# sanweiliti/EgoHMR

Measured on AMD Instinct MI355X. Metric: sampled bodies/sec (100-step DDPM, batch 256), higher is better.
Workload: dtype f32 results: denoiser GEMMs as 3x f16 MFMA on hi/lo-split operands (f32 accumulate) on the last 100 of 100 steps, plain f16 operands on the first 0; k = 100 is~; 1 GPU; B256 S1 DDPM-100 N4096 ResNet50+PointNet cond, diffuse_fuse(2 GCN passes), LBS every step, unguided; items_per_gpu=256, samples_per_item=1, denoising_steps=100, scene_points=4096, lbs_every_step=True, collision_guided=False, gcn_precision=f16x3, f16x3_last_steps=100, parallelism=items sharded x1, one RCCL all-gather of [B,226] at the end

## Files before the change

### egohmr_amd/_lib.py

```python
from __future__ import annotations

import ctypes as C
import glob
import itertools
import os
import subprocess
import sys
from types import SimpleNamespace

import torch

_HERE = os.path.dirname(os.path.abspath(__file__))
LIB_PATH = os.environ.get("EHM_LIB_PATH") or os.path.join(_HERE, "libegohmr_hip.so")
CSRC = os.path.join(_HERE, "csrc")
INCLUDE = os.path.join(os.path.dirname(_HERE), "include")
SOURCES = ["gcn.hip", "gcn_tile.hip", "linear.hip", "conv.hip", "stem.hip", "metrics.hip", "smpl.hip", "sampler.hip", "guidance.hip", "prep.hip", "step.hip", "eval.hip", "stage1.hip", "scene.hip", "loss.hip", "gcn_bwd.hip"]


class EgoHMRHipError(RuntimeError):
    def __init__(self, msg="", rc=None, function=None):
        super().__init__(msg)
        self.rc, self.function = rc, function


class EgoHMRRangeError(EgoHMRHipError):
    """rc = -34: an activation of the denoiser reached the f16 range and was clamped in its X2 / f16 store (ehm_gcn_stack_status).  The results are finite
    but not parity grade; the remedy is float32 activations for that checkpoint: EgoHMR.gcn_precision = 'f32' (EgoHMR.on_saturation = 'f32' does it
    and re-runs the call)."""


def build(verbose: bool = False, force: bool = False) -> str:
    import hashlib
    from concurrent.futures import ThreadPoolExecutor
    hipcc = os.environ.get("HIPCC", "/opt/rocm/bin/hipcc")
    extra = os.environ.get("EHM_HIPCC_FLAGS", "").split()
    flags = ["--offload-arch=gfx950", "-O3", "-std=c++17", "-fPIC", f"-I{INCLUDE}", f"-I{CSRC}", *extra]
    hdrs = glob.glob(os.path.join(CSRC, "*.h")) + [os.path.join(INCLUDE, "egohmr_hip.h")]
    hdr_time = max(os.path.getmtime(h) for h in hdrs)
    tag = hashlib.sha1(" ".join([hipcc] + flags).encode()).hexdigest()[:10]
    objdir = os.path.join(_HERE, "build", os.path.basename(LIB_PATH) + "." + tag)
    os.makedirs(objdir, exist_ok=True)
    jobs = []
    sources = SOURCES
    for s in sources:
        src, obj = os.path.join(CSRC, s), os.path.join(objdir, s.replace(".hip", ".o"))
        if force or not os.path.exists(obj) or os.path.getmtime(obj) < max(os.path.getmtime(src), hdr_time):
            jobs.append((src, obj))
    objs = [os.path.join(objdir, s.replace(".hip", ".o")) for s in sources]
    tag_path = LIB_PATH + ".tag"
    linked_tag = open(tag_path).read().strip() if os.path.exists(tag_path) else None
    if not jobs and os.path.exists(LIB_PATH) and linked_tag == tag and all(os.path.getmtime(LIB_PATH) >= os.path.getmtime(o) for o in objs):
        return LIB_PATH

    def compile_one(job):
        cmd = [hipcc, *flags, "-c", job[0], "-o", job[1]]
        if verbose:
            print(" ".join(cmd), file=sys.stderr)
        return subprocess.run(cmd, capture_output=True, text=True)

    with ThreadPoolExecutor(max_workers=int(os.environ.get("EHM_BUILD_JOBS", min(len(jobs) or 1, os.cpu_count() or 1)))) as ex:
        for (src, _), r in zip(jobs, ex.map(compile_one, jobs)):
            if r.returncode != 0:
                raise EgoHMRHipError(f"hipcc failed on {src}:\n{r.stdout}\n{r.stderr}")
            if "failed to meet occupancy target" in r.stderr:
                os.remove(os.path.join(objdir, os.path.basename(src).replace(".hip", ".o")))
                raise EgoHMRHipError(f"hipcc: a kernel of {src} missed its occupancy target:\n{r.stderr}")
    cmd = [hipcc, "--offload-arch=gfx950", "-fPIC", "-shared", *objs, "-o", LIB_PATH]
    if verbose:
        print(" ".join(cmd), file=sys.stderr)
    r = subprocess.run(cmd, capture_output=True, text=True)
    if r.returncode != 0:
        raise EgoHMRHipError(f"hipcc (link) failed:\n{r.stdout}\n{r.stderr}")
    with open(tag_path, "w") as f:
        f.write(tag + "\n")
    return LIB_PATH


def build_features() -> set:
    return set(lib().ehm_build_features().decode().split())


class GConvParams(C.Structure):
    _fields_ = [("W", C.c_void_p), ("M", C.c_void_p), ("adj2", C.c_void_p), ("bias", C.c_void_p),
                ("bn_weight", C.c_void_p), ("bn_bias", C.c_void_p), ("bn_mean", C.c_void_p), ("bn_var", C.c_void_p),
                ("in_dim", C.c_int), ("out_dim", C.c_int)]


class LinearDesc(C.Structure):
    _fields_ = [("A0", C.c_void_p), ("A1", C.c_void_p), ("W", C.c_void_p), ("bias", C.c_void_p), ("group_bias", C.c_void_p),
                ("Y", C.c_void_p), ("colmax", C.c_void_p), ("M", C.c_int64), ("N", C.c_int), ("K0", C.c_int), ("K1", C.c_int),
                ("rows_per_group", C.c_int), ("valid_rows_per_group", C.c_int), ("relu_in0", C.c_int), ("relu_out", C.c_int),
                ("w_scale", C.c_float), ("lift_points", C.c_void_p), ("lift_W4", C.c_void_p), ("hi_only", C.c_int), ("group_bias_stride", C.c_int)]


class ConvDesc(C.Structure):
    _fields_ = [("x", C.c_void_p), ("W", C.c_void_p), ("bias", C.c_void_p), ("residual", C.c_void_p), ("y", C.c_void_p),
                ("N", C.c_int), ("H", C.c_int), ("Wd", C.c_int), ("Ci", C.c_int), ("Co", C.c_int),
                ("KH", C.c_int), ("KW", C.c_int), ("stride", C.c_int), ("pad", C.c_int), ("relu", C.c_int),
                ("w_scale", C.c_float)]


class ConvX2Desc(C.Structure):
    _fields_ = [("x", C.c_void_p), ("x_rows", C.c_int64), ("W", C.c_void_p), ("bias", C.c_void_p), ("residual", C.c_void_p), ("y", C.c_void_p),
                ("N", C.c_int), ("H", C.c_int), ("Wd", C.c_int), ("Ci", C.c_int), ("Co", C.c_int),
                ("KH", C.c_int), ("KW", C.c_int), ("stride", C.c_int), ("pad", C.c_int), ("relu", C.c_int),
                ("w_scale", C.c_float), ("workspace", C.c_void_p), ("workspace_bytes", C.c_int64),
                ("x2", C.c_void_p), ("x2_rows", C.c_int64), ("H2", C.c_int), ("W2", C.c_int), ("Ci2", C.c_int), ("stride2", C.c_int), ("hi_only", C.c_int),
                ("workspace_clean", C.c_int)]


class EvalPointsDesc(C.Structure):
    _fields_ = [("pred", C.c_void_p), ("gt", C.c_void_p), ("pred_origin", C.c_void_p), ("gt_origin", C.c_void_p), ("mask", C.c_void_p),
                ("per_point", C.c_void_p), ("mean", C.c_void_p), ("vis_sum", C.c_void_p), ("invis_sum", C.c_void_p),
                ("B", C.c_int), ("S", C.c_int), ("P", C.c_int), ("pred_points", C.c_int), ("gt_points", C.c_int), ("origin_point", C.c_int)]


class ItemPrepDesc(C.Structure):
    _fields_ = [("keypoints_2d", C.c_void_p), ("joint_map", C.c_void_p), ("NK", C.c_int), ("force_visible", C.c_int),
                ("fx", C.c_void_p), ("cx", C.c_void_p), ("cy", C.c_void_p), ("box_center", C.c_void_p), ("box_size", C.c_void_p), ("transl", C.c_void_p),
                ("fx_norm", C.c_float), ("with_bbox", C.c_int), ("with_cam_center", C.c_int),
                ("tW1", C.c_void_p), ("tb1", C.c_void_p), ("tW2", C.c_void_p), ("tb2", C.c_void_p), ("t_hidden", C.c_int), ("t_out", C.c_int),
                ("img_rowsum", C.c_void_p), ("scene_rowsum", C.c_void_p), ("other", C.c_void_p), ("other_ld", C.c_int), ("other_col0", C.c_int),
                ("vis", C.c_void_p), ("mask_slot", C.c_void_p), ("mask_items", C.c_void_p), ("count", C.c_void_p), ("finite", C.c_void_p),
                ("need_scratch", C.c_void_p), ("pass_group", C.c_int), ("B", C.c_int)]


class PackDesc(C.Structure):
    _fields_ = [("B", C.c_int), ("J", C.c_int), ("V", C.c_int), ("finite", C.c_void_p), ("chk", C.c_void_p), ("chk_rows", C.c_int),
                ("last_noise", C.c_void_p), ("x_final", C.c_void_p), ("x0", C.c_void_p), ("pose6d", C.c_void_p), ("R", C.c_void_p),
                ("verts", C.c_void_p), ("joints", C.c_void_p), ("betas_in", C.c_void_p), ("betas_out", C.c_void_p),
                ("transl", C.c_void_p), ("fx", C.c_void_p), ("cx", C.c_void_p), ("cy", C.c_void_p), ("fx_norm", C.c_float),
                ("global_orient", C.c_void_p), ("body_pose", C.c_void_p), ("kp3d_full", C.c_void_p), ("kp2d_full", C.c_void_p),
                ("focal", C.c_void_p), ("center", C.c_void_p), ("finite_out", C.c_void_p)]


class ValLossesDesc(C.Structure):
    _fields_ = ([(n, C.c_int) for n in ("B", "V", "pred_joints", "gt_joints", "kp3d_points", "kp3d_full_points", "kp2d_points")] +
                [(n, C.c_void_p) for n in ("pred_vertices", "pred_keypoints_3d", "pred_keypoints_3d_full", "pred_keypoints_2d_full",
                                           "pred_global_orient", "pred_body_pose", "pred_betas", "pred_pose_6d",
                                           "keypoints_2d", "keypoints_3d", "keypoints_3d_full",
                                           "gt_vertices_male", "gt_vertices_female", "gt_joints_male", "gt_joints_female", "gender",
                                           "gt_global_orient", "gt_body_pose", "gt_betas", "focal", "center", "penetration")] +
                [("weights", C.c_double * 9), ("workspace", C.c_void_p), ("workspace_bytes", C.c_int64)] +
                [(n, C.c_void_p) for n in ("losses", "joint_vis_num", "per_item", "per_item_vis", "vis_mask")])


LOSS_KEYS = ("loss", "loss_v2v", "loss_keypoints_3d", "loss_keypoints_3d_full", "loss_keypoints_2d_full", "loss_betas", "loss_body_pose",
             "loss_global_orient", "loss_pose_6d_ortho", "loss_coap_penetration", "loss_keypoints_3d_vis_batch_sum")


GCN_CONV_INPUT, GCN_CONV_OUTPUT = -1, -2


class StepCoefs(C.Structure):
    _fields_ = [(n, C.c_float) for n in ("coef1", "coef2", "log_variance", "variance", "sqrt_recip_ac", "sqrt_recipm1_ac",
                                         "sqrt_ac_prev", "dir_coef", "sigma", "nonzero", "grad_scale")]


class NonlocalParams(C.Structure):
    _fields_ = [("Wqkv", C.c_void_p), ("bqkv", C.c_void_p), ("qkv_scale", C.c_float), ("Wo", C.c_void_p), ("bo", C.c_void_p), ("o_scale", C.c_float),
                ("Ci", C.c_int)]


class SampleDesc(C.Structure):
    _fields_ = [("B", C.c_int), ("passes", C.c_int), ("num_steps", C.c_int), ("ddim", C.c_int), ("lbs_every_step", C.c_int),
                ("num_scene_points", C.c_int), ("guide_denom", C.c_float), ("tau", C.c_float), ("num_masked", C.c_int), ("guide_all_points", C.c_int), ("lowprec_steps", C.c_int), ("nonlocal_ci", C.c_int), ("per_step_launches", C.c_int)]


class Stage1Desc(C.Structure):
    _fields_ = [("img_feats", C.c_void_p), ("scene_feats", C.c_void_p), ("fx", C.c_void_p), ("cam_cx", C.c_void_p), ("cam_cy", C.c_void_p),
                ("box_center", C.c_void_p), ("box_size", C.c_void_p), ("W1t", C.c_void_p), ("b1", C.c_void_p), ("W2", C.c_void_p), ("b2", C.c_void_p),
                ("init_cam", C.c_void_p), ("init_betas", C.c_void_p), ("pred_cam", C.c_void_p), ("pred_cam_full", C.c_void_p), ("pred_betas", C.c_void_p),
                ("fx_norm", C.c_float), ("crop_res", C.c_float), ("with_cam_center", C.c_int), ("with_bbox_info", C.c_int), ("with_focal_length", C.c_int),
                ("img_dim", C.c_int), ("scene_dim", C.c_int), ("hidden", C.c_int), ("B", C.c_int)]


class SceneDesc(C.Structure):
    _fields_ = [("verts", C.c_void_p), ("total_verts", C.c_int64), ("mesh_offsets", C.c_void_p), ("num_meshes", C.c_int), ("max_mesh_verts", C.c_int64),
                ("groups", C.c_void_p), ("num_groups", C.c_int), ("params", C.c_void_p), ("mode", C.c_int), ("chain_len", C.c_int), ("B", C.c_int),
                ("target", C.c_int), ("stride", C.c_int), ("points", C.c_void_p), ("index", C.c_void_p), ("n_selected", C.c_void_p),
                ("status", C.c_void_p), ("workspace", C.c_void_p), ("workspace_bytes", C.c_int64)]


_P, _I, _L, _F = C.c_void_p, C.c_int, C.c_int64, C.c_float

PROTOTYPES = {
    "ehm_last_error": (C.c_char_p, []),
    "ehm_target_arch": (C.c_char_p, []),
    "ehm_build_features": (C.c_char_p, []),
    "ehm_rot6d_to_rotmat": (_I, [_P, _P, _L, _I, _P]),
    "ehm_rot6d_to_rotmat_bwd": (_I, [_P, _P, _P, _L, _I, _P]),
    "ehm_rotmat_to_angle_axis": (_I, [_P, _P, _L, _P]),
    "ehm_rotmat_to_angle_axis_bwd": (_I, [_P, _P, _P, _L, _P]),
    "ehm_smpl_create": (_I, [C.POINTER(_P), _P, _P, _P, _P, _P, C.POINTER(C.c_int32), C.POINTER(C.c_int32), _I, _I, _P]),
    "ehm_smpl_destroy": (None, [_P]),
    "ehm_smpl_forward": (_I, [_P, _P, _P, _P, _P, _P, _I, _P]),
    "ehm_smpl_forward_rot6d": (_I, [_P, _P, _P, _P, _P, _P, _P, _P, _P, _P, _I, _P]),
    "ehm_gcn_create": (_I, [C.POINTER(_P), _P, C.POINTER(GConvParams), C.POINTER(GConvParams), _I, C.POINTER(GConvParams), _I, _P]),
    "ehm_gcn_destroy": (None, [_P]),
    "ehm_gcn_row_tile": (_I, []),
    "ehm_gcn_set_precision": (_I, [_P, _I]),
    "ehm_gcn_get_precision": (_I, [_P]),
    "ehm_gcn_set_uncond_mode": (_I, [_P, _I]),
    "ehm_gcn_set_pass_map": (_I, [_P, _P, _P, _I]),
    "ehm_gcn_set_nonlocal": (_I, [_P, C.POINTER(NonlocalParams)]),
    "ehm_gcn_reserve": (_I, [_P, _I, _I]),
    "ehm_gcn_activation_group": (_I, [_P]),
    "ehm_gcn_pack_activations": (_I, [_P, _P, _L, _I, _I, _P]),
    "ehm_gcn_unpack_activations": (_I, [_P, _P, _L, _I, _I, _P]),
    "ehm_gcn_pack_activations_checked": (_I, [_P, _P, _P, _L, _P]),
    "ehm_gcn_input_layer": (_I, [_P, _P, _P, _P, _P, _P, _P, _P, _I, _I, _P]),
    "ehm_gcn_input_layer_rows": (_I, [_P, _P, _P, _I, _P]),
    "ehm_gcn_hidden_layer": (_I, [_P, _I, _P, _P, _P, _L, _P]),
    "ehm_gcn_hidden_stack": (_I, [_P, C.POINTER(C.c_void_p), _L, C.POINTER(C.c_int), _P]),
    "ehm_gcn_stack_status": (_I, [_P, _P]),
    "ehm_gcn_stack_status_async": (_I, [_P, _P, _P]),
    "ehm_gcn_output_layer": (_I, [_P, _P, _P, _P, _I, _I, _P]),
    "ehm_gcn_bwd_epilogue": (_I, [_P, _I, _P, _P, _P, _I, _I, _P]),
    "ehm_gcn_bwd_params_workspace_bytes": (_I, [_P, _I, _I, C.POINTER(C.c_int64)]),
    "ehm_gcn_bwd_params": (_I, [_P, _I, _P, _P, _P, _I, _I, _P, _P, _P, _P, _P, _P, _L, _P]),
    "ehm_linear_split": (_I, [C.POINTER(LinearDesc), _P]),
    "ehm_split_pack": (_I, [_P, _P, _L, _I, _I, _F, _P]),
    "ehm_skinny_gemm_f32": (_I, [_P, _P, _P, _P, _I, _I, _I, _I, _P]),
    "ehm_resnet_stem_scratch_bytes": (C.c_size_t, [_I, _I, _I]),
    "ehm_resnet_stem": (_I, [_P, _P, _P, _P, _P, _I, _I, _I, _I, _P]),
    "ehm_conv_x2_rows": (C.c_int64, [C.c_int64]),
    "ehm_conv_x2": (_I, [C.POINTER(ConvX2Desc), _P]),
    "ehm_conv_x2_workspace_bytes": (C.c_int64, [C.POINTER(ConvX2Desc)]),
    "ehm_conv_x2_workspace_status": (_I, [_P, _P, _P]),
    "ehm_x2_group_mean": (_I, [_P, _P, _I, _I, _I, _I, _P]),
    "ehm_conv_nhwc_split": (_I, [C.POINTER(ConvDesc), _P]),
    "ehm_nonlocal_attention": (_I, [_P, _P, _L, _I, _P]),
    "ehm_pointnet_lift": (_I, [_P, _P, _P, _P, _P, _I, _I, _I, _I, _P]),
    "ehm_ddpm_step": (_I, [_P, _P, _P, _P, _P, _F, _F, _F, _F, _F, _L, _P]),
    "ehm_ddim_step": (_I, [_P, _P, _P, _P, _F, _F, _F, _F, _F, _F, _L, _P]),
    "ehm_collision_proxy": (_I, [_P, _P, _P, _P, _I, _I, _I, _F, _P]),
    "ehm_collision_query": (_I, [_P, _P, _P, _P, _P, _I, _I, _I, _F, _I, _P]),
    "ehm_smpl_backward_rot6d": (_I, [_P, _P, _P, _P, _P, _P, _P, _I, _P]),
    "ehm_guidance_grad_finish": (_I, [_P, _P, _P, _I, _F, _P]),
    "ehm_smpl_backward": (_I, [_P, _P, _P, _P, _P, _P, _P, _I, _P, _L, _P]),
    "ehm_smpl_backward_workspace_bytes": (_I, [_P, _I, C.POINTER(C.c_int64)]),
    "ehm_nn_dist2": (_I, [_P, _P, _P, _P, _I, _I, _I, _P]),
    "ehm_eval_point_errors": (_I, [C.POINTER(EvalPointsDesc), _P]),
    "ehm_eval_procrustes": (_I, [_P, _P, _P, _P, _P, _P, _P, _P, _I, _I, _I, _P]),
    "ehm_eval_procrustes_vis": (_I, [_P, _P, _P, _P, _P, _P, _P, _P, _I, _I, _I, _P]),
    "ehm_eval_diversity": (_I, [_P, _P, _I, _P, _P, _I, _I, _I, _P]),
    "ehm_stage1_head": (_I, [C.POINTER(Stage1Desc), _P]),
    "ehm_scene_workspace_bytes": (_I, [C.POINTER(SceneDesc), C.POINTER(C.c_int64)]),
    "ehm_scene_select": (_I, [C.POINTER(SceneDesc), _P]),
    "ehm_sample_workspace_bytes": (_L, [C.POINTER(SampleDesc), _I, _I]),
    "ehm_sample_loop": (_I, [_P, _P, C.POINTER(SampleDesc), C.POINTER(StepCoefs)] + [_P] * 18 + [_L, _P]),
    "ehm_item_prep": (_I, [C.POINTER(ItemPrepDesc), _P]),
    "ehm_pack_outputs": (_I, [C.POINTER(PackDesc), _P]),
    "ehm_val_losses_workspace_bytes": (_I, [_I, _I, C.POINTER(C.c_int64)]),
    "ehm_val_losses": (_I, [C.POINTER(ValLossesDesc), _P]),
    "ehm_scene_cap_points": (_I, [_P, _P, _P, _P, _I, _I, _I, _I, _P]),
    "ehm_profile_begin": (_I, []),
    "ehm_profile_end": (_I, [C.POINTER(C.c_double), C.POINTER(C.c_int64), _I]),
}
PROF_CLASSES = ("input", "chain_f16x3", "chain_f16", "hidden_f32", "out_dot", "step_body", "skin_input", "guidance", "reserved_8", "reserved_9",
                "guid_nearest", "guid_skin_bwd", "guid_posefeat_bwd", "step_fused", "guid_nearest_evals")
VALUE_FUNCTIONS = frozenset({"ehm_gcn_row_tile", "ehm_gcn_get_precision", "ehm_gcn_activation_group", "ehm_conv_x2_rows", "ehm_conv_x2_workspace_bytes",
                             "ehm_sample_workspace_bytes", "ehm_resnet_stem_scratch_bytes"})

_lib = None
_api = None


def lib() -> C.CDLL:
    global _lib, _api
    if _lib is None:
        if not os.path.exists(LIB_PATH):
            raise EgoHMRHipError(
                f"{LIB_PATH} is missing: build it with `python -c 'import __graft_entry__ as g; g.build()'` "
                "(hipcc --offload-arch=gfx950).  egohmr_amd has no CPU/eager fallback.")
        try:
            handle = C.CDLL(LIB_PATH)
        except OSError as e:
            raise EgoHMRHipError(f"cannot load {LIB_PATH}: {e}") from e
        for name, (res, args) in PROTOTYPES.items():
            try:
                fn = getattr(handle, name)
            except AttributeError as e:
                raise EgoHMRHipError(f"{LIB_PATH} does not export {name}; rebuild it") from e
            fn.restype = res
            fn.argtypes = args
        if handle.ehm_target_arch() != b"gfx950":
            raise EgoHMRHipError("libegohmr_hip.so was not built for gfx950")
        _api = SimpleNamespace(**{name: _checked(name, getattr(handle, name)) for name in PROTOTYPES})
        _lib = handle
    return _lib


def api() -> SimpleNamespace:
    lib()
    return _api


def _error(rc: int, function: str) -> EgoHMRHipError:
    msg = lib().ehm_last_error()
    cls = EgoHMRRangeError if rc == -34 else EgoHMRHipError
    return cls(f"{function} failed (rc={rc}): {msg.decode() if msg else ''}", rc=rc, function=function)


def _checked(name, fn):
    unchecked, value = PROTOTYPES[name][0] in (None, C.c_char_p), name in VALUE_FUNCTIONS

    def call(*args):
        rc = fn(*[ptr(a) if isinstance(a, torch.Tensor) else a for a in args])
        if not unchecked and (rc < 0 if value else rc != 0):
            raise _error(rc, name)
        return rc
    call.__name__ = name
    return call


def check(rc: int, what: str = "") -> None:
    if rc != 0:
        raise _error(rc, what or "libegohmr_hip")


class Handle:
    _serials = itertools.count(1)

    def __init__(self, ptr, destroy, keep=()):
        self.ptr, self._destroy, self.keep = ptr, destroy, list(keep)
        self.serial = next(Handle._serials)

    @property
    def _as_parameter_(self):
        return self.ptr

    def close(self):
        p, self.ptr = self.ptr, None
        if p is not None:
            self._destroy(p)
        self.keep = []

    def __del__(self):
        try:
            self.close()
        except Exception:
            pass


def ptr(t) -> int:
    if t is None:
        return None
    if not t.is_cuda:
        raise EgoHMRHipError("egohmr_amd kernels need tensors on a HIP device (got a CPU tensor); there is no CPU path")
    if not t.is_contiguous():
        raise EgoHMRHipError("tensor handed to the C ABI must be contiguous")
    return t.data_ptr()


class TensorKey:

    def __init__(self, *modules):
        self.modules = modules
        self.refresh()

    def refresh(self):
        self.slots = []
        seen = set()
        for mod in self.modules:
            for m in mod.modules():
                if id(m) in seen:
                    continue
                seen.add(id(m))
                self.slots += [(m._parameters, n) for n in m._parameters] + [(m._buffers, n) for n in m._buffers]

    def __call__(self):
        out = []
        for d, n in self.slots:
            t = d.get(n)
            if t is not None:
                out.append((t.data_ptr(), t._version))
        return tuple(out)


def f32(t, device=None):
    t = t.detach()
    if device is not None and t.device != device:
        t = t.to(device)
    if t.dtype != torch.float32:
        t = t.float()
    return t.contiguous()


def stream_ptr() -> int:
    try:
        return torch.cuda.current_stream().cuda_stream
    except RuntimeError as e:
        raise EgoHMRHipError(f"egohmr_amd kernels need a HIP device; there is no CPU path ({e})") from e


def on_device(dev):
    import contextlib
    dev = torch.device(dev) if not isinstance(dev, torch.device) else dev
    return torch.cuda.device(dev) if dev.type == "cuda" else contextlib.nullcontext()
```

### egohmr_amd/csrc/gcn.hip

```cpp
#include <stdlib.h>

#include "common.h"
#include "egohmr_hip.h"
#include "gcn_dev.h"
#include "internal.h"

namespace {

__global__ void pack_w_kernel(const float* __restrict__ W, float* __restrict__ Wp, int K, int N) {
  __shared__ float tile[32][33];
  int u = blockIdx.z;
  int k0 = blockIdx.y * 32, n0 = blockIdx.x * 32;
  int tx = threadIdx.x & 31, ty = threadIdx.x >> 5;
  for (int r = ty; r < 32; r += 8) {
    int k = k0 + r, n = n0 + tx;
    tile[r][tx] = (k < K && n < N) ? W[((size_t)u * K + k) * N + n] : 0.f;
  }
  __syncthreads();
  for (int r = ty; r < 32; r += 8) {
    int n = n0 + r, k = k0 + tx;
    if (n < N && k < K) {
      int nt = n >> 6, c = n & 63;
      Wp[((size_t)nt * 128 + u * 64 + c) * K + k] = tile[tx][r];
    }
  }
}

__global__ void pack_epilogue_kernel(const float* __restrict__ adj, ehm_gconv_params p, float* D, float* M1, float* shift,
                                     float* Aoff) {
  int N = p.out_dim;
  int n = blockIdx.x * blockDim.x + threadIdx.x;
  if (blockIdx.x == 0 && threadIdx.x < kJ * kJ) {
    int i = threadIdx.x / kJ, j = threadIdx.x % kJ;
    float aij = adj[i * kJ + j] + p.adj2[i * kJ + j];
    float aji = adj[j * kJ + i] + p.adj2[j * kJ + i];
    Aoff[i * kJ + j] = (i == j) ? 0.f : (aji + aij) / 2;
  }
  if (n >= N) return;
  float scale = 1.f, sh = p.bias ? p.bias[n] : 0.f;
  if (p.bn_weight) {
    scale = p.bn_weight[n] / sqrtf(p.bn_var[n] + 1e-5f);
    sh = (sh - p.bn_mean[n]) * scale + p.bn_bias[n];
  }
  shift[n] = sh;
  for (int j = 0; j < kJ; ++j) {
    const float ajj = adj[j * kJ + j] + p.adj2[j * kJ + j];
    float m = p.M[j * N + n];
    D[j * N + n] = ajj * m * scale;
    M1[j * N + n] = m * scale;
  }
}

__global__ void pack_out_kernel(const float* __restrict__ adj, ehm_gconv_params p, float* Wt, float* M, float* A, float* bias) {
  int K = p.in_dim;
  int t = blockIdx.x * blockDim.x + threadIdx.x;
  if (t < 12 * K) {
    int r = t / K, k = t % K;
    int u = r / 6, c = r % 6;
    Wt[t] = p.W[((size_t)u * K + k) * 6 + c];
  }
  if (t < kJ * kJ) {
    int i = t / kJ, j = t % kJ;
    A[t] = ((adj[j * kJ + i] + p.adj2[j * kJ + i]) + (adj[i * kJ + j] + p.adj2[i * kJ + j])) / 2;
  }
  if (t < kJ * 6) M[t] = p.M[t];
  if (t < 6) bias[t] = p.bias ? p.bias[t] : 0.f;
}

__global__ void absmax_kernel(const float* __restrict__ w, size_t n, unsigned int* __restrict__ out) {
  float m = 0.f;
  for (size_t i = (size_t)blockIdx.x * blockDim.x + threadIdx.x; i < n; i += (size_t)gridDim.x * blockDim.x) m = fmaxf(m, fabsf(w[i]));
#pragma unroll
  for (int o = 32; o >= 1; o >>= 1) m = fmaxf(m, __shfl_xor(m, o));
  if ((threadIdx.x & 63) == 0) atomicMax(out, __float_as_uint(m));
}

template <int G>
__global__ void pack_ws_kernel(const float* __restrict__ Wp, half_t* __restrict__ Ws, size_t rows, int K, float scale) {
  size_t i = (size_t)blockIdx.x * blockDim.x + threadIdx.x;
  if (i >= rows * K) return;
  split_store<G>(Ws, i / K, (int)(i % K), K, Wp[i] * scale);
}
__global__ void scale_epilogue_kernel(const float* __restrict__ D, const float* __restrict__ M1, float* __restrict__ Ds,
                                      float* __restrict__ M1s, int N, float inv_scale) {
  int i = blockIdx.x * blockDim.x + threadIdx.x;
  if (i >= kJ * N) return;
  const int j = i / N, n = i % N;
  Ds[n * kJ + j] = D[i] * inv_scale;
  M1s[n * kJ + j] = M1[i] * inv_scale;
}

#define AS1 __attribute__((address_space(1)))
#define AS3 __attribute__((address_space(3)))

template <bool RES>
__global__ __launch_bounds__(256, 2) void gcn_hidden_kernel(const float* __restrict__ X, LayerDev L,
                                                             const float* __restrict__ Res, float* __restrict__ Y,
                                                             int m_tiles) {
  __shared__ __attribute__((aligned(16))) float lds[2 * STAGE];

  const int K = L.K, N = L.N;
  const int n_tiles = N / BNH;
  int bid = blockIdx.x;
  const int total = m_tiles * n_tiles;
  int lin = ((total & 7) == 0) ? (bid & 7) * (total >> 3) + (bid >> 3) : bid;
  const int m_tile = lin / n_tiles, n_tile = lin % n_tiles;
  const size_t m0 = (size_t)m_tile * BM;

  const int tid = threadIdx.x;
  const int lane = tid & 63;
  const int wave = __builtin_amdgcn_readfirstlane(tid >> 6);
  const int wm = wave >> 1, wn = wave & 1;

  const int ld_r = lane >> 3, ld_c = lane & 7;
  const float* gA[6];
  const float* gB[4];
#pragma unroll
  for (int i = 0; i < 6; ++i) {
    int r = 8 * (wave + 4 * i) + ld_r;
    gA[i] = X + (m0 + r) * K + ((ld_c ^ ((r >> 1) & 7)) << 2);
  }
#pragma unroll
  for (int i = 0; i < 4; ++i) {
    int r = 8 * (wave + 4 * i) + ld_r;
    gB[i] = L.Wp + ((size_t)n_tile * 128 + r) * K + ((ld_c ^ ((r >> 1) & 7)) << 2);
  }
  auto stage = [&](int buf, int kt) {
    float* base = lds + buf * STAGE;
#pragma unroll
    for (int i = 0; i < 6; ++i)
      __builtin_amdgcn_global_load_lds((const AS1 void*)(gA[i] + kt * BK), (AS3 void*)(base + (wave + 4 * i) * 256), 16, 0, 0);
#pragma unroll
    for (int i = 0; i < 4; ++i)
      __builtin_amdgcn_global_load_lds((const AS1 void*)(gB[i] + kt * BK),
                                       (AS3 void*)(base + A_TILE + (wave + 4 * i) * 256), 16, 0, 0);
  };

  const int mi = lane & 31, h = lane >> 5;
  const int rA = 96 * wm + 48 * ((mi >> 2) & 1) + (mi & 3) + 4 * (mi >> 3);
  const int rB = 32 * wn + mi;
  const int keyA = (rA >> 1) & 7, keyB = (rB >> 1) & 7;

  f32x16 acc0[3], acc1[3];
#pragma unroll
  for (int t = 0; t < 3; ++t) {
#pragma unroll
    for (int r = 0; r < 16; ++r) { acc0[t][r] = 0.f; acc1[t][r] = 0.f; }
  }

  const int KT = K / BK;
  stage(0, 0);
  for (int kt = 0; kt < KT; ++kt) {
    asm volatile("s_waitcnt vmcnt(0)" ::: "memory");
    __syncthreads();
    if (kt + 1 < KT) stage((kt + 1) & 1, kt + 1);
    const float* As = lds + (kt & 1) * STAGE;
    const float* Bs = As + A_TILE;
#pragma unroll
    for (int kk = 0; kk < 4; ++kk) {
      const int cA = ((2 * kk + h) ^ keyA) << 2, cB = ((2 * kk + h) ^ keyB) << 2;
      f32x4 a[3], b[2];
#pragma unroll
      for (int t = 0; t < 3; ++t) a[t] = *(const f32x4*)(As + (rA + 16 * t) * BK + cA);
#pragma unroll
      for (int u = 0; u < 2; ++u) b[u] = *(const f32x4*)(Bs + (rB + 64 * u) * BK + cB);
#pragma unroll
      for (int s = 0; s < 4; ++s) {
#pragma unroll
        for (int t = 0; t < 3; ++t) {
          acc0[t] = __builtin_amdgcn_mfma_f32_32x32x2f32(a[t][s], b[0][s], acc0[t], 0, 0, 0);
          acc1[t] = __builtin_amdgcn_mfma_f32_32x32x2f32(a[t][s], b[1][s], acc1[t], 0, 0, 0);
        }
      }
    }
  }

  const int n = n_tile * BNH + 32 * wn + mi;
  const size_t rowb = m0 + 96 * wm + 48 * h;
  float res0[kJ], res1[kJ];
#pragma unroll
  for (int j = 0; j < kJ; ++j) res0[j] = RES ? Res[(rowb + j) * (size_t)N + n] : 0.f;
  {
    float dj[kJ], mj[kJ];
    const float sh = L.shift[n];
#pragma unroll
    for (int j = 0; j < kJ; ++j) { dj[j] = L.D[j * N + n]; mj[j] = L.M1[j * N + n]; }
    __builtin_amdgcn_sched_barrier(0);
#pragma unroll
    for (int j = 0; j < kJ; ++j) {
#pragma unroll
      for (int beta = 0; beta < 2; ++beta) {
        const int q = 24 * beta + j;
        acc0[q >> 4][q & 15] = fmaf(dj[j], acc0[q >> 4][q & 15], sh);
        acc1[q >> 4][q & 15] *= mj[j];
      }
    }
  }
  __builtin_amdgcn_sched_barrier(0);
#pragma unroll
  for (int j = 0; j < kJ; ++j) res1[j] = RES ? Res[(rowb + 24 + j) * (size_t)N + n] : 0.f;
  __builtin_amdgcn_sched_barrier(0);
  {
    float d0[kJ], g1[kJ];
#pragma unroll
    for (int j = 0; j < kJ; ++j) { d0[j] = acc0[j >> 4][j & 15]; g1[j] = acc1[j >> 4][j & 15]; }
    gcn_mix_store<false>(d0, g1, res0, n, N, rowb, L.Aoff, Y, L.relu != 0);
  }
  __builtin_amdgcn_sched_barrier(0);
  {
    float d0[kJ], g1[kJ];
#pragma unroll
    for (int j = 0; j < kJ; ++j) { d0[j] = acc0[(24 + j) >> 4][(24 + j) & 15]; g1[j] = acc1[(24 + j) >> 4][(24 + j) & 15]; }
    gcn_mix_store<false>(d0, g1, res1, n, N, rowb + 24, L.Aoff, Y, L.relu != 0);
  }
}

template <int OUT>
__global__ __launch_bounds__(256) void gcn_input_kernel(GcnInputArgs a) {
  __shared__ __attribute__((aligned(16))) float T[kJ * 256];
  gcn_input_body<OUT>(T, blockIdx.x, blockIdx.y, a);
}

template <int OUT>
__global__ __launch_bounds__(256) void gcn_input_rows_kernel(GcnInputArgs a) {
  __shared__ __attribute__((aligned(16))) float T[kJ * 256];
  gcn_input_body<OUT, false, true>(T, (int)threadIdx.x, blockIdx.x, blockIdx.y, a, nullptr);
}


template <bool HALF_IN>
__global__ __launch_bounds__(256) void gcn_out_dot_kernel(const float* __restrict__ X, OutDev O, float* __restrict__ hs, int64_t rows) {
  __shared__ float part[4][16][16];
  gcn_out_dot_rows16<HALF_IN, 0>(X, O, hs, (int64_t)blockIdx.x * OUT_ROWS_PER_BLOCK, rows, part, (int)threadIdx.x);
}

__global__ __launch_bounds__(192) void gcn_out_mix_kernel(const float* __restrict__ hs, OutDev O, const uint8_t* __restrict__ vis,
                                                          float* __restrict__ x0, int B, int passes, const int32_t* __restrict__ mask_slot) {
  __shared__ float sh[2][kJ][12];
  __shared__ float outs[2][kJ][6];
  const int b = blockIdx.x, tid = threadIdx.x;
  const int slot = mask_slot ? mask_slot[b] : b;
  for (int i = tid; i < passes * kJ * 12; i += 192) {
    const int p = i / (kJ * 12), rem = i % (kJ * 12);
    sh[p][rem / 12][rem % 12] = (p == 1 && slot < 0) ? 0.f : hs[((size_t)(p ? B + slot : b) * kJ) * 12 + rem];
  }
  __syncthreads();
  for (int e = tid; e < passes * kJ * 6; e += 192) {
    const int p = e / (kJ * 6), j = (e / 6) % kJ, c = e % 6;
    const float s = O.A[j * kJ + j] * (O.M[j * 6 + c] * sh[p][j][c]);
    float t = 0.f;
    for (int jp = 0; jp < kJ; ++jp)
      if (jp != j) t = fmaf(O.A[j * kJ + jp], O.M[jp * 6 + c] * sh[p][jp][6 + c], t);
    outs[p][j][c] = s + t + O.bias[c];
  }
  __syncthreads();
  if (tid < kPoseDim) {
    const int j = tid / 6, c = tid % 6;
    float v = outs[0][j][c];
    if (passes == 2 && !vis[(size_t)b * kJ + j]) v = outs[1][j][c];
    x0[(size_t)b * kPoseDim + tid] = v;
  }
}

}

__global__ void pack_aoff_half_kernel(const float* __restrict__ Aoff, half8* __restrict__ out) {
  const int lane = threadIdx.x, i = lane & 31;
#pragma unroll
  for (int s = 0; s < 3; ++s) {
    half8 v;
#pragma unroll
    for (int c = 0; c < 8; ++c) {
      const int kk = 16 * s + 8 * (lane >> 5) + c;
      float x = 0.f;
      if (i < kJ) x = kk < kJ ? Aoff[i * kJ + kk] : (kk - kJ == i ? 1.f : 0.f);
      v[c] = (half_t)x;
    }
    out[s * 64 + lane] = v;
  }
}

static int pack_layer(const float* adj, const ehm_gconv_params& p, LayerDev& L, float*& cursor, bool with_w, hipStream_t st) {
  const int N = p.out_dim, K = p.in_dim;
  L.K = K;
  L.N = N;
  L.relu = p.bn_weight != nullptr;
  if (with_w) {
    L.Wp = cursor;
    cursor += (size_t)2 * K * N;
    L.Ws = (half_t*)cursor;
    cursor += (size_t)2 * K * N;
    L.Wh = (half_t*)cursor;
    cursor += (size_t)K * N;
    L.Ds = cursor;   cursor += (size_t)kJ * N;
    L.M1s = cursor;  cursor += (size_t)kJ * N;
  }
  if (!with_w) {
    L.Ds = cursor;   cursor += (size_t)kJ * N;
    L.M1s = cursor;  cursor += (size_t)kJ * N;
    L.w_scale = 1.f;
  }
  L.D = cursor;      cursor += (size_t)kJ * N;
  L.M1 = cursor;     cursor += (size_t)kJ * N;
  L.shift = cursor;  cursor += N;
  L.Aoff = cursor;   cursor += kJ * kJ;
  L.AoffH = (const half_t*)cursor;  cursor += 768;
  if (with_w) {
    dim3 grid((unsigned)ceil_div(N, 32), (unsigned)ceil_div(K, 32), 2);
    hipLaunchKernelGGL(pack_w_kernel, grid, dim3(256), 0, st, p.W, L.Wp, K, N);
  }
  const int threads = 1024;
  hipLaunchKernelGGL(pack_epilogue_kernel, dim3((unsigned)ceil_div(N, threads)), dim3(threads), 0, st, adj, p, L.D, L.M1,
                     L.shift, L.Aoff);
  hipLaunchKernelGGL(pack_aoff_half_kernel, dim3(1), dim3(64), 0, st, L.Aoff, (half8*)L.AoffH);
  if (!with_w) hipLaunchKernelGGL(scale_epilogue_kernel, dim3((unsigned)ceil_div(kJ * N, 256)), dim3(256), 0, st, L.D, L.M1, L.Ds, L.M1s, N, 1.f);
  EHM_LAUNCH_CHECK();
  if (with_w) {
    unsigned int* d_max = (unsigned int*)cursor;
    EHM_HIP(hipMemsetAsync(d_max, 0, sizeof(unsigned int), st));
    hipLaunchKernelGGL(absmax_kernel, dim3(256), dim3(256), 0, st, p.W, (size_t)2 * K * N, d_max);
    unsigned int bits = 0;
    EHM_HIP(hipMemcpyAsync(&bits, d_max, sizeof(bits), hipMemcpyDeviceToHost, st));
    EHM_HIP(hipStreamSynchronize(st));
    float wmax;
    memcpy(&wmax, &bits, sizeof(wmax));
    int e = 0;
    if (wmax > 0.f && wmax < 3.0e38f) {
      (void)frexpf(wmax, &e);
      e = 12 - e;
      if (e > 24) e = 24;
      if (e < -24) e = -24;
    }
    L.w_scale = ldexpf(1.f, e);
    hipLaunchKernelGGL(pack_ws_kernel<32>, dim3((unsigned)ceil_div((int64_t)2 * K * N, 256)), dim3(256), 0, st, L.Wp, L.Ws, (size_t)2 * N, K,
                       L.w_scale);
    ehm_pack_half(L.Wp, L.Wh, (size_t)2 * K * N, L.w_scale, st);
    hipLaunchKernelGGL(scale_epilogue_kernel, dim3((unsigned)ceil_div(kJ * N, 256)), dim3(256), 0, st, L.D, L.M1, L.Ds, L.M1s, N,
                       1.f / L.w_scale);
    EHM_LAUNCH_CHECK();
  }
  return 0;
}

extern "C" int ehm_gcn_row_tile(void) { return BM; }

extern "C" int ehm_gcn_create(ehm_gcn** out, const float* adj, const ehm_gconv_params* input_conv,
                              const ehm_gconv_params* hidden, int num_hidden, const ehm_gconv_params* output_conv,
                              int hid_dim, void* stream) {
  EHM_CHECK_ARG(out && adj && input_conv && hidden && output_conv);
  EHM_CHECK_ARG(num_hidden >= 0 && num_hidden <= 16);
  EHM_CHECK_ARG(hid_dim > 0 && hid_dim % 64 == 0 && hid_dim % BK == 0);
  EHM_CHECK_ARG(input_conv->out_dim == hid_dim && output_conv->in_dim == hid_dim && output_conv->out_dim == 6);
  for (int i = 0; i < num_hidden; ++i) EHM_CHECK_ARG(hidden[i].in_dim == hid_dim && hidden[i].out_dim == hid_dim && hidden[i].W);
  hipStream_t st = (hipStream_t)stream;
  auto* g = new ehm_gcn();
  if (const char* e = getenv("EHM_F16_CHAIN")) g->chain = atoi(e);
  g->hid = hid_dim;
  g->num_hidden = num_hidden;
  g->adj = adj;
  g->raw_input = *input_conv;
  for (int i = 0; i < num_hidden; ++i) g->raw_hidden[i] = hidden[i];
  g->raw_out = *output_conv;
  const size_t epi = (size_t)2 * kJ * hid_dim + hid_dim + kJ * kJ + 768;
  size_t floats = epi * (1 + num_hidden) + (size_t)num_hidden * (5 * (size_t)hid_dim * hid_dim + 2 * kJ * hid_dim) + 2 * (size_t)kJ * hid_dim +
                  12 * (size_t)hid_dim + kJ * 6 + kJ * kJ + 8 + 64;
  if (hipMalloc(&g->arena, floats * sizeof(float)) != hipSuccess) {
    delete g;
    ehm_set_error("ehm_gcn_create: hipMalloc of %zu bytes failed", floats * sizeof(float));
    return EHM_ENOMEM;
  }
  float* cur = g->arena;
  int rc = pack_layer(adj, *input_conv, g->input, cur, false, st);
  for (int i = 0; i < num_hidden && rc == 0; ++i) rc = pack_layer(adj, hidden[i], g->hidden[i], cur, true, st);
  if (rc == 0) {
    g->out.K = hid_dim;
    g->out.Wt = cur;   cur += 12 * (size_t)hid_dim;
    g->out.M = cur;    cur += kJ * 6;
    g->out.A = cur;    cur += kJ * kJ;
    g->out.bias = cur; cur += 8;
    hipLaunchKernelGGL(pack_out_kernel, dim3((unsigned)ceil_div(12 * hid_dim, 256)), dim3(256), 0, st, adj, *output_conv,
                       g->out.Wt, g->out.M, g->out.A, g->out.bias);
    if (hipGetLastError() != hipSuccess) rc = EHM_EIO;
  }
  if (rc == 0 && num_hidden > 0) {
    if (hipMalloc(&g->hidden_dev, sizeof(LayerDev) * num_hidden) != hipSuccess ||
        hipMemcpyAsync(g->hidden_dev, g->hidden, sizeof(LayerDev) * num_hidden, hipMemcpyHostToDevice, st) != hipSuccess)
      rc = EHM_ENOMEM;
  }
  if (rc == 0 && (hipMalloc(&g->chain_sticky, 64) != hipSuccess || hipMemsetAsync(g->chain_sticky, 0, 64, st) != hipSuccess)) rc = EHM_ENOMEM;
  if (rc == 0 && hipStreamSynchronize(st) != hipSuccess) rc = EHM_EIO;
  if (rc == 0) rc = ehm_gcn_reserve_rows(g, 2 * 256 * kJ);
  if (rc != 0) {
    if (g->hidden_dev) (void)hipFree(g->hidden_dev);
    if (g->chain_sticky) (void)hipFree(g->chain_sticky);
    if (g->chain_sync) (void)hipFree(g->chain_sync);
    if (g->hs) (void)hipFree(g->hs);
    (void)hipFree(g->arena);
    delete g;
    ehm_set_error("ehm_gcn_create: packing kernels failed");
    return rc;
  }
  *out = g;
  return 0;
}

extern "C" void ehm_gcn_destroy(ehm_gcn* h) {
  if (!h) return;
  (void)hipFree(h->arena);
  if (h->hs) (void)hipFree(h->hs);
  if (h->hidden_dev) (void)hipFree(h->hidden_dev);
  if (h->chain_sync) (void)hipFree(h->chain_sync);
  if (h->chain_sticky) (void)hipFree(h->chain_sticky);
  delete h;
}

int ehm_gcn_input_args(const ehm_gcn* h, const GcnRun& r, const float* h_img, const float* h_oth, const uint8_t* vis, const float* x, const float* Wx,
                       const float* tvec, float* out, int B, int passes, GcnInputArgs* a) {
  EHM_CHECK_ARG(h && h_img && h_oth && vis && x && Wx && tvec && out && a);
  EHM_CHECK_ARG(B > 0 && (passes == 1 || passes == 2));
  a->h_img = h_img; a->h_oth = h_oth; a->vis = vis; a->x = x; a->Wx = Wx; a->tvec = tvec;
  a->L = h->input;
  a->Y = out;
  a->B = B; a->passes = passes; a->mask_all = r.uncond_masks_all;
  a->mask_items = r.items(passes);
  a->sticky = h->chain_sticky;
  a->total_vb = r.virtual_bodies(B, passes);
  a->ny = (int)ceil_div(h->hid, 256);
  return 0;
}

template <bool PRE, int OUT>
static void launch_input_conv(const GcnInputArgs& a, hipStream_t st) {
  const dim3 grid((unsigned)a.total_vb, (unsigned)a.ny);
  if constexpr (PRE) hipLaunchKernelGGL(gcn_input_rows_kernel<OUT>, grid, dim3(256), 0, st, a);
  else hipLaunchKernelGGL(gcn_input_kernel<OUT>, grid, dim3(256), 0, st, a);
}
template <bool PRE>
static int input_conv(const GcnInputArgs& a, int fmt, hipStream_t st) {
  if (fmt == EHM_PREC_F32) launch_input_conv<PRE, 0>(a, st);
  else if (fmt == EHM_PREC_F16X3) launch_input_conv<PRE, 1>(a, st);
  else launch_input_conv<PRE, 2>(a, st);
  EHM_LAUNCH_CHECK();
  return 0;
}

int ehm_gcn_input_impl(const ehm_gcn* h, const GcnRun& r, const float* h_img, const float* h_oth, const uint8_t* vis, const float* x,
                       const float* Wx, const float* tvec, float* out, int B, int passes, hipStream_t st) {
  GcnInputArgs a;
  const int rc = ehm_gcn_input_args(h, r, h_img, h_oth, vis, x, Wx, tvec, out, B, passes, &a);
  return rc != 0 ? rc : input_conv<false>(a, gcn_input_format(h, r.precision), st);
}

extern "C" int ehm_gcn_input_layer(ehm_gcn* h, const float* h_img, const float* h_oth, const uint8_t* vis, const float* x,
                                   const float* Wx, const float* tvec, float* out, int B, int passes, void* stream) {
  EHM_CHECK_ARG(h);
  const int rc = ehm_gcn_input_impl(h, h->run, h_img, h_oth, vis, x, Wx, tvec, out, B, passes, (hipStream_t)stream);
  if (rc == 0) h->run.valid_rows = (int64_t)h->run.virtual_bodies(B, passes) * kJ;
  return rc;
}

extern "C" int ehm_gcn_input_layer_rows(ehm_gcn* h, const float* pre, float* out, int bodies, void* stream) {
  EHM_CHECK_ARG(h && pre && out && bodies > 0);
  GcnInputArgs a{};
  a.L = h->input;
  a.Y = out;
  a.B = bodies; a.passes = 1; a.mask_all = 0;
  a.mask_items = nullptr;
  a.total_vb = bodies;
  a.ny = (int)ceil_div(h->hid, 256);
  a.sticky = h->chain_sticky;
  h->run.valid_rows = (int64_t)bodies * kJ;
  a.pre = pre;
  return input_conv<true>(a, gcn_input_format(h, h->run.precision), (hipStream_t)stream);
}

static int hidden_layer(const ehm_gcn* h, const GcnRun& r, int layer, const float* X, const float* residual, float* out, int64_t rows_pad,
                        hipStream_t st) {
  EHM_CHECK_ARG(X && out);
  EHM_CHECK_ARG(layer >= 0 && layer < h->num_hidden);
  EHM_CHECK_ARG(rows_pad > 0 && rows_pad % BM == 0);
  EHM_CHECK_ARG(X != out);
  if (r.precision != EHM_PREC_F32)
    return ehm_gcn_tile_layer_impl(h, r, layer, X, residual, out, rows_pad, layer == h->num_hidden - 1, st);
  const int m_tiles = (int)(rows_pad / BM);
  const int blocks = m_tiles * (h->hid / BNH);
  if (residual)
    hipLaunchKernelGGL(gcn_hidden_kernel<true>, dim3(blocks), dim3(256), 0, st, X, h->hidden[layer], residual, out, m_tiles);
  else
    hipLaunchKernelGGL(gcn_hidden_kernel<false>, dim3(blocks), dim3(256), 0, st, X, h->hidden[layer], (const float*)nullptr, out, m_tiles);
  EHM_LAUNCH_CHECK();
  return 0;
}

extern "C" int ehm_gcn_hidden_layer(ehm_gcn* h, int layer, const float* X, const float* residual, float* out,
                                    int64_t rows_pad, void* stream) {
  EHM_CHECK_ARG(h);
  return hidden_layer(h, h->run, layer, X, residual, out, rows_pad, (hipStream_t)stream);
}

int ehm_gcn_hidden_stack_impl(ehm_gcn* h, const GcnRun& r, float* const bufs[3], int64_t rows_pad, int* result_index, hipStream_t st) {
  EHM_CHECK_ARG(h && bufs && bufs[0] && bufs[1] && bufs[2] && result_index && rows_pad > 0 && rows_pad % BM == 0);
  EHM_CHECK_ARG(h->num_hidden % 2 == 0);
  const int nblk = h->num_hidden / 2;
  *result_index = (nblk & 1) ? 2 : 0;
  if (nblk == 0) return 0;
  if (h->chain && r.precision != EHM_PREC_F32) return ehm_gcn_tile_chain_impl(h, r, (void* const*)bufs, rows_pad, st);
  int in = 0;
  for (int blk = 0; blk < nblk; ++blk) {
    const int y2 = in == 0 ? 2 : 0;
    int rc = hidden_layer(h, r, 2 * blk, bufs[in], nullptr, bufs[1], rows_pad, st);
    if (rc == 0) rc = hidden_layer(h, r, 2 * blk + 1, bufs[1], bufs[in], bufs[y2], rows_pad, st);
    if (rc != 0) return rc;
    in = y2;
  }
  return 0;
}

extern "C" int ehm_gcn_hidden_stack(ehm_gcn* h, float* const bufs[3], int64_t rows_pad, int* result_index, void* stream) {
  EHM_CHECK_ARG(h);
  return ehm_gcn_hidden_stack_impl(h, h->run, bufs, rows_pad, result_index, (hipStream_t)stream);
}

extern "C" int ehm_gcn_stack_status(ehm_gcn* h, void* stream) {
  EHM_CHECK_ARG(h);
  unsigned int flag = 0;
  if (h->chain_sticky) {
    EHM_HIP(hipMemcpyAsync(&flag, h->chain_sticky, sizeof(flag), hipMemcpyDeviceToHost, (hipStream_t)stream));
    EHM_HIP(hipStreamSynchronize((hipStream_t)stream));
    if (flag) {
      EHM_HIP(hipMemsetAsync(h->chain_sticky, 0, sizeof(flag), (hipStream_t)stream));
      h->chain_sync_clean = 0;
    }
  }
  if (flag & ~kStickySaturated) {
    ehm_set_error("ehm_gcn_hidden_stack: a chained launch since the last status call timed out waiting for a producer tile, or left tiles "
                  "unproduced (GPU shared / preempted / CU-masked?); the results of that sampling loop are invalid - re-run, or set EHM_F16_CHAIN=0");
    return EHM_EIO;
  }
  if (flag & kStickySaturated) {
    ehm_set_error("ehm_gcn: an activation of the denoiser reached the f16 range (|x| >= 65504) since the last status call and was CLAMPED in its X2 / f16 "
                  "store - the split format holds |x| <= 131008 and is f32-grade only below 65504 (nothing became inf / NaN, the results are finite but not "
                  "parity grade).  This checkpoint needs ehm_gcn_set_precision(h, 0) (EgoHMR.gcn_precision = 'f32': float32 activations, exact-f32 MFMA)");
    return EHM_ERANGE;
  }
  return 0;
}

extern "C" int ehm_gcn_stack_status_async(ehm_gcn* h, uint32_t* host_flag, void* stream) {
  EHM_CHECK_ARG(h && host_flag);
  if (h->chain_sticky) EHM_HIP(hipMemcpyAsync(host_flag, h->chain_sticky, sizeof(unsigned int), hipMemcpyDeviceToHost, (hipStream_t)stream));
  else *host_flag = 0u;
  return 0;
}

int ehm_gcn_reserve_rows(ehm_gcn* h, int64_t rows_pad) {
  if (rows_pad <= h->reserved_rows) return 0;
  const size_t need = 8 + (size_t)((h->num_hidden > 0 ? h->num_hidden : 1) + 3) * (size_t)ceil_div(rows_pad, BM) + 32;
  if (h->chain_sync) EHM_HIP(hipFree(h->chain_sync));
  h->chain_sync = nullptr;
  h->chain_sync_words = 0;
  EHM_HIP(hipMalloc(&h->chain_sync, need * sizeof(unsigned int)));
  h->chain_sync_words = need;
  h->chain_sync_clean = 0;
  if (h->hs) EHM_HIP(hipFree(h->hs));
  h->hs = nullptr;
  h->hs_rows = 0;
  EHM_HIP(hipMalloc(&h->hs, (size_t)round_up(rows_pad, 4096) * 12 * sizeof(float)));
  h->hs_rows = round_up(rows_pad, 4096);
  h->reserved_rows = rows_pad;
  return 0;
}

extern "C" int ehm_gcn_reserve(ehm_gcn* h, int max_bodies, int passes) {
  EHM_CHECK_ARG(h && max_bodies > 0 && (passes == 1 || passes == 2));
  return ehm_gcn_reserve_rows(h, round_up((int64_t)max_bodies * passes * kJ, BM));
}

int ehm_gcn_output_dot_impl(ehm_gcn* h, const GcnRun& r, const float* X, int B, int passes, const float** hs, hipStream_t st) {
  const int64_t rows = (int64_t)r.virtual_bodies(B, passes) * kJ;
  if (rows > h->hs_rows) {
    const int rc = ehm_gcn_reserve_rows(h, round_up(rows, BM));
    if (rc != 0) return rc;
  }
  if (r.precision == EHM_PREC_F16)
    hipLaunchKernelGGL(gcn_out_dot_kernel<true>, dim3((unsigned)ceil_div(rows, OUT_ROWS_PER_BLOCK)), dim3(256), 0, st, X, h->out, h->hs, rows);
  else
    hipLaunchKernelGGL(gcn_out_dot_kernel<false>, dim3((unsigned)ceil_div(rows, OUT_ROWS_PER_BLOCK)), dim3(256), 0, st, X, h->out, h->hs, rows);
  EHM_LAUNCH_CHECK();
  *hs = h->hs;
  return 0;
}

extern "C" int ehm_gcn_output_layer(ehm_gcn* h, const float* X, const uint8_t* vis, float* x0, int B, int passes,
                                    void* stream) {
  EHM_CHECK_ARG(h && X && x0);
  EHM_CHECK_ARG(B > 0 && (passes == 1 || (passes == 2 && vis)));
  const float* hs;
  const int rc = ehm_gcn_output_dot_impl(h, h->run, X, B, passes, &hs, (hipStream_t)stream);
  if (rc != 0) return rc;
  hipLaunchKernelGGL(gcn_out_mix_kernel, dim3(B), dim3(192), 0, (hipStream_t)stream, hs, h->out, vis, x0, B, passes, h->run.slots(passes));
  EHM_LAUNCH_CHECK();
  return 0;
}

extern "C" int ehm_gcn_set_pass_map(ehm_gcn* h, const int32_t* mask_items, const int32_t* mask_slot, int num_masked) {
  EHM_CHECK_ARG(h && (num_masked < 0 || (mask_slot && (num_masked == 0 || mask_items))));
  h->run.mask_items = num_masked >= 0 ? mask_items : nullptr;
  h->run.mask_slot = num_masked >= 0 ? mask_slot : nullptr;
  h->run.num_masked = num_masked < 0 ? -1 : num_masked;
  return 0;
}

extern "C" int ehm_gcn_set_nonlocal(ehm_gcn* h, const ehm_nonlocal_params* p) {
  EHM_CHECK_ARG(h);
  if (!p) { h->nonlocal = ehm_nonlocal_params{}; return 0; }
  EHM_CHECK_ARG(p->Wqkv && p->bqkv && p->Wo && p->bo && p->Ci > 0 && p->Ci % 8 == 0 && p->qkv_scale > 0.f && p->o_scale > 0.f);
  h->nonlocal = *p;
  return 0;
}

extern "C" int ehm_gcn_set_precision(ehm_gcn* h, int mode) {
  EHM_CHECK_ARG(h && (mode == EHM_PREC_F32 || mode == EHM_PREC_F16X3 || mode == EHM_PREC_F16));
  h->run.precision = mode;
  return 0;
}
extern "C" int ehm_gcn_get_precision(const ehm_gcn* h) { return h ? h->run.precision : EHM_EINVAL; }
extern "C" int ehm_gcn_set_uncond_mode(ehm_gcn* h, int masks_whole_condition) {
  EHM_CHECK_ARG(h && (masks_whole_condition == 0 || masks_whole_condition == 1));
  h->run.uncond_masks_all = masks_whole_condition;
  return 0;
}
extern "C" int ehm_gcn_activation_group(const ehm_gcn* h) { return h ? (h->run.precision == EHM_PREC_F16 ? 0 : 32) : EHM_EINVAL; }
```

### egohmr_amd/csrc/gcn_dev.h

```cpp
#pragma once
#include "common.h"
#include "egohmr_hip.h"

typedef _Float16 half_t;
typedef _Float16 half8 __attribute__((ext_vector_type(8)));

constexpr int BM = 192;
constexpr int BNH = 64;
constexpr int BK = 32;
constexpr int A_TILE = BM * BK;
constexpr int B_TILE = 2 * BNH * BK;
constexpr int STAGE = A_TILE + B_TILE;

struct LayerDev {
  float* Wp;
  half_t* Ws;
  half_t* Wh;
  float* Ds;
  float* M1s;
  float w_scale;
  float* D;
  float* M1;
  float* shift;
  float* Aoff;
  const half_t* AoffH;
  int K, N;
  int relu;
};

struct OutDev {
  float* Wt;
  float* M;
  float* A;
  float* bias;
  int K;
};


enum { EHM_PREC_F32 = 0, EHM_PREC_F16X3 = 1, EHM_PREC_F16 = 2 };

struct GcnRun {
  int precision = EHM_PREC_F32;
  const int32_t* mask_items = nullptr;
  const int32_t* mask_slot = nullptr;
  int num_masked = -1;
  int uncond_masks_all = 0;
  int64_t valid_rows = 0;
  int virtual_bodies(int B, int passes) const { return passes == 2 ? B + (num_masked >= 0 ? num_masked : B) : B; }
  const int32_t* items(int passes) const { return (passes == 2 && num_masked >= 0) ? mask_items : nullptr; }
  const int32_t* slots(int passes) const { return (passes == 2 && num_masked >= 0) ? mask_slot : nullptr; }
  unsigned int guarded_rows(int64_t rows_pad) const { return (unsigned int)(valid_rows > 0 && valid_rows < rows_pad ? valid_rows : rows_pad); }
};

struct ehm_gcn {
  int hid = 0;
  int num_hidden = 0;
  GcnRun run{};
  LayerDev input{};
  LayerDev hidden[16]{};
  LayerDev* hidden_dev = nullptr;
  unsigned int* chain_sync = nullptr;
  unsigned int* chain_sticky = nullptr;
  size_t chain_sync_words = 0;
  int chain_sync_clean = 0;
  int64_t chain_sync_shape = 0;
  size_t chain_err_off = 0;
  int chain = 1;
  OutDev out{};
  float* arena = nullptr;
  float* hs = nullptr;
  int64_t hs_rows = 0;
  int64_t reserved_rows = 0;
  ehm_nonlocal_params nonlocal{};
  const float* adj = nullptr;
  ehm_gconv_params raw_input{}, raw_hidden[16]{}, raw_out{};
};

static inline int gcn_input_format(const ehm_gcn* h, int prec) {
  return (prec == EHM_PREC_F16X3 && h->num_hidden == 0) ? (int)EHM_PREC_F32 : prec;
}

template <int G = 32>
static __device__ __forceinline__ size_t split_off(size_t row, int n, int N) {
  return row * (size_t)N * 2 + (size_t)(n / G) * (2 * G) + (n % G);
}
template <int G = 32>
static __device__ __forceinline__ void split_store(half_t* base, size_t row, int n, int N, float v) {
  const float c = fminf(fmaxf(v, -65504.f), 65504.f);
  const half_t hi = (half_t)c;
  const half_t lo = (half_t)fminf(fmaxf(v - (float)hi, -65504.f), 65504.f);
  half_t* p = base + split_off<G>(row, n, N);
  p[0] = hi;
  p[G] = lo;
}
template <int G = 32>
static __device__ __forceinline__ float split_load(const half_t* base, size_t row, int n, int N) {
  const half_t* p = base + split_off<G>(row, n, N);
  return (float)p[0] + (float)p[G];
}

static __device__ __forceinline__ unsigned int split_pack_bits(float v) {
  const float c = fminf(fmaxf(v, -65504.f), 65504.f);
  const half_t hi = (half_t)c;
  const half_t lo = (half_t)fminf(fmaxf(v - (float)hi, -65504.f), 65504.f);
  return (unsigned int)__builtin_bit_cast(unsigned short, hi) | ((unsigned int)__builtin_bit_cast(unsigned short, lo) << 16);
}
static __device__ __forceinline__ unsigned int split_pair_word(float v, bool odd) {
  const unsigned int own = split_pack_bits(v);
  const unsigned int nbr = dpp_xor1_u32(own);
  return odd ? ((nbr >> 16) | (own & 0xffff0000u)) : ((own & 0xffffu) | (nbr << 16));
}
template <int G = 32>
static __device__ __forceinline__ void split_store_pair(half_t* base, size_t row, int n, int N, float v) {
  const unsigned int own = split_pack_bits(v);
  const unsigned int nbr = dpp_xor1_u32(own);
  const bool odd = n & 1;
  const unsigned int word = odd ? ((nbr >> 16) | (own & 0xffff0000u)) : ((own & 0xffffu) | (nbr << 16));
  half_t* p = base + split_off<G>(row, n & ~1, N) + (odd ? G : 0);
  *(unsigned int*)p = word;
}
template <int G = 32>
static __device__ __forceinline__ unsigned int split_load_pair_raw(const half_t* base, size_t row, int n, int N) {
  const half_t* p = base + split_off<G>(row, n & ~1, N) + ((n & 1) ? G : 0);
  return *(const unsigned int*)p;
}
static __device__ __forceinline__ float split_pair_decode(unsigned int own, int n) {
  const bool odd = n & 1;
  const unsigned int nbr = dpp_xor1_u32(own);
  const unsigned short hb = odd ? (unsigned short)(nbr >> 16) : (unsigned short)(own & 0xffffu);
  const unsigned short lb = odd ? (unsigned short)(own >> 16) : (unsigned short)(nbr & 0xffffu);
  return (float)__builtin_bit_cast(half_t, hb) + (float)__builtin_bit_cast(half_t, lb);
}
template <int G = 32>
static __device__ __forceinline__ float split_load_pair(const half_t* base, size_t row, int n, int N) {
  const bool odd = n & 1;
  const half_t* p = base + split_off<G>(row, n & ~1, N) + (odd ? G : 0);
  const unsigned int own = *(const unsigned int*)p;
  const unsigned int nbr = dpp_xor1_u32(own);
  const unsigned short hb = odd ? (unsigned short)(nbr >> 16) : (unsigned short)(own & 0xffffu);
  const unsigned short lb = odd ? (unsigned short)(own >> 16) : (unsigned short)(nbr & 0xffffu);
  return (float)__builtin_bit_cast(half_t, hb) + (float)__builtin_bit_cast(half_t, lb);
}

template <bool SPLIT_OUT, int G = 32>
static __device__ __forceinline__ void gcn_mix_store(const float (&d0)[kJ], const float (&g1)[kJ], const float (&res)[kJ], int n, int N,
                                              size_t row0, const float* __restrict__ Aoff, float* __restrict__ Y, bool relu) {
  typedef const float __attribute__((address_space(4))) cfloat;
  const cfloat* Ac = (const cfloat*)(uintptr_t)Aoff;
#pragma unroll
  for (int j = 0; j < kJ; ++j) {
    float s = d0[j];
#pragma unroll
    for (int jp = 0; jp < kJ; ++jp) s = fmaf(Ac[j * kJ + jp], g1[jp], s);
    if (relu) s = fmaxf(s, 0.f);
    if (SPLIT_OUT) split_store_pair<G>((half_t*)Y, row0 + j, n, N, s + res[j]);
    else Y[(row0 + j) * (size_t)N + n] = s + res[j];
  }
}

typedef float f32x2 __attribute__((ext_vector_type(2)));
template <class Store>
static __device__ __forceinline__ void gcn_mix2(const f32x2 (&dp)[kJ], const f32x2 (&gp)[kJ], const float* __restrict__ Aoff, bool relu,
                                                Store store) {
  typedef const float __attribute__((address_space(4))) cfloat;
  const cfloat* Ac = (const cfloat*)(uintptr_t)Aoff;
#pragma unroll
  for (int j0 = 0; j0 < kJ; j0 += 4) {
    __builtin_amdgcn_sched_barrier(0);
#pragma unroll
    for (int i = 0; i < 4; ++i) {
      const int j = j0 + i;
      float s0 = dp[j][0], s1 = dp[j][1];
#pragma unroll
      for (int jp = 0; jp < kJ; ++jp) {
        const float a = Ac[j * kJ + jp];
        s0 = fmaf(a, gp[jp][0], s0);
        s1 = fmaf(a, gp[jp][1], s1);
      }
      if (relu) { s0 = fmaxf(s0, 0.f); s1 = fmaxf(s1, 0.f); }
      store(j, s0, s1);
    }
  }
}

constexpr unsigned int kStickySaturated = 4u;

struct GcnInputArgs {
  const float* h_img; const float* h_oth; const uint8_t* vis; const float* x; const float* Wx; const float* tvec;
  LayerDev L;
  float* Y;
  int B, passes, mask_all;
  const int32_t* mask_items;
  int total_vb, ny;
  unsigned int* sticky = nullptr;
  const float* pre = nullptr;
};

template <int OUT, bool X_LDS = false, bool PRE = false>
__device__ __forceinline__ void gcn_input_body(float* T, int tid, int bx, int by, const GcnInputArgs& a, const float* xb_in) {
  const float* __restrict__ h_img = a.h_img; const float* __restrict__ h_oth = a.h_oth; const uint8_t* __restrict__ vis = a.vis;
  const float* __restrict__ x = a.x; const float* __restrict__ Wx = a.Wx; const float* __restrict__ tvec = a.tvec;
  const LayerDev& L = a.L;
  float* __restrict__ Y = a.Y;
  const int B = a.B, passes = a.passes, mask_all = a.mask_all;
  const int32_t* __restrict__ mask_items = a.mask_items;
  (void)passes;
  const int N = L.N;
  const int vb = bx;
  const int p = vb >= B ? 1 : 0, b = p ? (mask_items ? mask_items[vb - B] : vb - B) : vb;
  const int n_raw = by * 256 + tid;
  const int n = n_raw < N ? n_raw : N - 1;
  float base[2] = {0.f, 0.f}, img[2] = {0.f, 0.f}, wx[2][6] = {{0.f, 0.f, 0.f, 0.f, 0.f, 0.f}, {0.f, 0.f, 0.f, 0.f, 0.f, 0.f}};
  if constexpr (!PRE)
#pragma unroll
  for (int k = 0; k < 2; ++k) {
    base[k] = ((p == 1 && mask_all) ? 0.f : h_oth[((size_t)b * 2 + k) * N + n]) + tvec[k * N + n];
    img[k] = (p == 0) ? h_img[((size_t)b * 2 + k) * N + n] : 0.f;
#pragma unroll
    for (int c = 0; c < 6; ++c) wx[k][c] = Wx[(k * 6 + c) * N + n];
  }
  const float* xb = xb_in ? xb_in : (PRE ? nullptr : x + (size_t)b * kPoseDim);
  float xr[X_LDS ? kPoseDim : 1];
  if constexpr (X_LDS) {
    typedef const f32x4 __attribute__((address_space(3))) lf32x4;
    lf32x4* xl = (lf32x4*)xb_in;
#pragma unroll
    for (int i = 0; i < kPoseDim / 4; ++i) {
      const f32x4 v = xl[i];
      xr[4 * i] = v[0]; xr[4 * i + 1] = v[1]; xr[4 * i + 2] = v[2]; xr[4 * i + 3] = v[3];
    }
  }
  const uint8_t* vb_ = PRE ? nullptr : vis + (size_t)b * kJ;
  float h0[kJ], h1[kJ];
  const float sh = L.shift[n];
  float dj[kJ], mj[kJ];
  {
    typedef unsigned int u32x4_tb __attribute__((ext_vector_type(4)));
    const __amdgpu_buffer_rsrc_t dsB = ehm_buffer_rsrc(L.Ds), m1B = ehm_buffer_rsrc(L.M1s);
    const unsigned int nrow = (unsigned int)n * (unsigned int)(kJ * 4);
#pragma unroll
    for (int q4 = 0; q4 < kJ / 4; ++q4) {
      const u32x4_tb d4 = __builtin_amdgcn_raw_buffer_load_b128(dsB, nrow, 16 * q4, 0);
      const u32x4_tb m4 = __builtin_amdgcn_raw_buffer_load_b128(m1B, nrow, 16 * q4, 0);
#pragma unroll
      for (int i = 0; i < 4; ++i) {
        const unsigned int du = d4[i], mu = m4[i];
        dj[4 * q4 + i] = __builtin_bit_cast(float, du);
        mj[4 * q4 + i] = __builtin_bit_cast(float, mu);
      }
    }
  }
  const f32x2 img2 = {img[0], img[1]}, base2 = {base[0], base[1]};
  f32x2 wx2[6];
#pragma unroll
  for (int c = 0; c < 6; ++c) wx2[c] = f32x2{wx[0][c], wx[1][c]};
#pragma unroll
  for (int j = 0; j < kJ; ++j) {
    f32x2 s;
    if constexpr (PRE) {
      const float* pr = a.pre + ((size_t)vb * kJ + j) * 2 * (size_t)N + n;
      s = f32x2{pr[0], pr[N]};
    } else {
    const float v = vb_[j] ? 1.f : 0.f;
    s = __builtin_elementwise_fma(f32x2{v, v}, img2, base2);
#pragma unroll
    for (int c = 0; c < 6; ++c) {
      const float xv = X_LDS ? xr[X_LDS ? j * 6 + c : 0] : xb[j * 6 + c];
      s = __builtin_elementwise_fma(f32x2{xv, xv}, wx2[c], s);
    }
    }
    h0[j] = fmaf(dj[j], s[0], sh);
    h1[j] = mj[j] * s[1];
  }
  if constexpr (OUT == 2) {
    typedef unsigned int u32x4_t __attribute__((ext_vector_type(4)));
    typedef _Float16 half2_t __attribute__((ext_vector_type(2)));
    const int lane = tid & 63, wv = tid >> 6;
    f32x16 DA, DB;
#pragma unroll
    for (int r = 0; r < 16; ++r) { DA[r] = 0.f; DB[r] = 0.f; }
#pragma unroll
    for (int s3 = 0; s3 < 3; ++s3) {
      const half8 af = ((const half8*)L.AoffH)[s3 * 64 + lane];
      u32x4_t Pw, Qw;
#pragma unroll
      for (int e = 0; e < 4; ++e) {
        const int kp = 16 * s3 + 2 * e, kq = kp + 8;
        const float p0 = kp < kJ ? h1[kp] : h0[kp - kJ], p1 = kp + 1 < kJ ? h1[kp + 1] : h0[kp + 1 - kJ];
        const float q0 = kq < kJ ? h1[kq] : h0[kq - kJ], q1 = kq + 1 < kJ ? h1[kq + 1] : h0[kq + 1 - kJ];
        const half2_t hp = {(half_t)fmaf(p0, 0.f, fminf(fmaxf(p0, -65504.f), 65504.f)), (half_t)fmaf(p1, 0.f, fminf(fmaxf(p1, -65504.f), 65504.f))};
        const half2_t hq = {(half_t)fmaf(q0, 0.f, fminf(fmaxf(q0, -65504.f), 65504.f)), (half_t)fmaf(q1, 0.f, fminf(fmaxf(q1, -65504.f), 65504.f))};
        const auto sw = __builtin_amdgcn_permlane32_swap(__builtin_bit_cast(unsigned int, hp), __builtin_bit_cast(unsigned int, hq), false, false);
        Pw[e] = sw[0];
        Qw[e] = sw[1];
      }
      DA = __builtin_amdgcn_mfma_f32_32x32x16_f16(af, __builtin_bit_cast(half8, Pw), DA, 0, 0, 0);
      DB = __builtin_amdgcn_mfma_f32_32x32x16_f16(af, __builtin_bit_cast(half8, Qw), DB, 0, 0, 0);
    }
    const bool relu = L.relu != 0;
    const int cA = 64 * wv + (lane & 31), half = lane >> 5;
#pragma unroll
    for (int r = 0; r < 12; ++r) {
      const int j = (r & 3) + 8 * (r >> 2) + 4 * half;
      const float va = relu ? fmaxf(DA[r], 0.f) : DA[r], vb = relu ? fmaxf(DB[r], 0.f) : DB[r];
      T[j * 256 + cA] = fmaf(DA[r], 0.f, va);
      T[j * 256 + cA + 32] = fmaf(DB[r], 0.f, vb);
    }
  } else {
    typedef const float __attribute__((address_space(4))) cfloat;
    const cfloat* Ac = (const cfloat*)(uintptr_t)L.Aoff;
    const bool relu = L.relu != 0;
    f32x2 sacc[kJ / 2];
#pragma unroll
    for (int jj = 0; jj < kJ / 2; ++jj) sacc[jj] = f32x2{h0[2 * jj], h0[2 * jj + 1]};
#pragma unroll
    for (int jp = 0; jp < kJ; ++jp) {
      const f32x2 hh = {h1[jp], h1[jp]};
#pragma unroll
      for (int jj = 0; jj < kJ / 2; ++jj) sacc[jj] = __builtin_elementwise_fma(f32x2{Ac[jp * kJ + 2 * jj], Ac[jp * kJ + 2 * jj + 1]}, hh, sacc[jj]);
    }
#pragma unroll
    for (int jj = 0; jj < kJ / 2; ++jj) {
      f32x2 o = sacc[jj];
      if (relu) { o[0] = fmaxf(o[0], 0.f); o[1] = fmaxf(o[1], 0.f); }
      if constexpr (OUT != 0) o = __builtin_elementwise_fma(sacc[jj], f32x2{0.f, 0.f}, o);
      T[(2 * jj) * 256 + tid] = o[0];
      T[(2 * jj + 1) * 256 + tid] = o[1];
    }
  }
  __syncthreads();
  typedef unsigned int u32x4 __attribute__((ext_vector_type(4)));
  const int nb = by * 256;
#pragma unroll
  for (int i = 0; i < 3; ++i) {
    const int u = tid + 256 * i, j = u >> 5, c8 = (u & 31) * 8;
    if (nb + c8 >= N) continue;

    const f32x4 v0 = *(const f32x4*)(T + j * 256 + c8), v1 = *(const f32x4*)(T + j * 256 + c8 + 4);
    const float v[8] = {v0[0], v0[1], v0[2], v0[3], v1[0], v1[1], v1[2], v1[3]};
    const size_t row = (size_t)vb * kJ + j;
    if (OUT != 0) {
      if (a.sticky) {
        float vm = 0.f;
#pragma unroll
        for (int k = 0; k < 8; k += 2) vm = fmaxf(vm, fmaxf(fabsf(v[k]), fabsf(v[k + 1])));
        if (vm >= 65504.f && vm <= 3.0e38f) __hip_atomic_fetch_or(a.sticky, kStickySaturated, __ATOMIC_RELAXED, __HIP_MEMORY_SCOPE_AGENT);
      }
      half8 hh, ll;
#pragma unroll
      for (int k = 0; k < 8; ++k) {
        const float c = fmaf(v[k], 0.f, fminf(fmaxf(v[k], -65504.f), 65504.f));
        hh[k] = (half_t)c;
        ll[k] = (half_t)fminf(fmaxf(v[k] - (float)hh[k], -65504.f), 65504.f);
      }
      if (OUT == 1) {
        half_t* p = (half_t*)Y + split_off<32>(row, nb + c8, N);
        *(u32x4*)p = __builtin_bit_cast(u32x4, hh);
        *(u32x4*)(p + 32) = __builtin_bit_cast(u32x4, ll);
      } else {
        *(u32x4*)((half_t*)Y + row * (size_t)N + nb + c8) = __builtin_bit_cast(u32x4, hh);
      }
    } else {
      float* p = Y + row * (size_t)N + nb + c8;
      *(f32x4*)p = v0;
      *(f32x4*)(p + 4) = v1;
    }
  }
}
template <int OUT>
__device__ __forceinline__ void gcn_input_body(float* T, int bx, int by, const GcnInputArgs& a) {
  gcn_input_body<OUT>(T, (int)threadIdx.x, bx, by, a, nullptr);
}

constexpr int OUT_ROWS_PER_BLOCK = 16;
template <bool HALF_IN, int AUX>
__device__ __forceinline__ f32x4 gcn_out_dot_quarter(const float* __restrict__ X, const OutDev& O, int64_t r, int wave, int lane) {
  const int K = O.K;
  const int row = lane & 15, q = lane >> 4;
  const int kq = K / 4;
  typedef unsigned int u32x4_od __attribute__((ext_vector_type(4)));
  typedef unsigned int u32x2_od __attribute__((ext_vector_type(2)));
  const __amdgpu_buffer_rsrc_t rsX = ehm_buffer_rsrc_4g(X), rsW = ehm_buffer_rsrc(O.Wt);
  const unsigned int vox = (unsigned int)((r * K + (size_t)wave * kq + 8 * q) * (HALF_IN ? 2 : 4));
  const unsigned int vow = (unsigned int)(((size_t)(row < 12 ? row : 0) * K + (size_t)wave * kq + 8 * q) * 4);
  f32x4 acc = {0.f, 0.f, 0.f, 0.f}, acc2 = {0.f, 0.f, 0.f, 0.f};
#pragma unroll 4
  for (int k = 0; k + 32 <= kq; k += 32) {
    float xv[8];
    if (HALF_IN) {
      const half8 hv = __builtin_bit_cast(half8, (u32x4_od)__builtin_amdgcn_raw_buffer_load_b128(rsX, vox, k * 2, AUX));
#pragma unroll
      for (int c = 0; c < 8; ++c) xv[c] = (float)hv[c];
    } else {
      const f32x4 x0 = __builtin_bit_cast(f32x4, (u32x4_od)__builtin_amdgcn_raw_buffer_load_b128(rsX, vox, k * 4, AUX));
      const f32x4 x1 = __builtin_bit_cast(f32x4, (u32x4_od)__builtin_amdgcn_raw_buffer_load_b128(rsX, vox, k * 4 + 16, AUX));
#pragma unroll
      for (int c = 0; c < 4; ++c) { xv[c] = x0[c]; xv[4 + c] = x1[c]; }
    }
    f32x4 w0 = __builtin_bit_cast(f32x4, (u32x4_od)__builtin_amdgcn_raw_buffer_load_b128(rsW, vow, k * 4, 0));
    f32x4 w1 = __builtin_bit_cast(f32x4, (u32x4_od)__builtin_amdgcn_raw_buffer_load_b128(rsW, vow, k * 4 + 16, 0));
    if (row >= 12) { w0 = f32x4{0.f, 0.f, 0.f, 0.f}; w1 = w0; }
#pragma unroll
    for (int c = 0; c < 4; c += 2) {
      acc = __builtin_amdgcn_mfma_f32_16x16x4f32(xv[c], w0[c], acc, 0, 0, 0);
      acc2 = __builtin_amdgcn_mfma_f32_16x16x4f32(xv[c + 1], w0[c + 1], acc2, 0, 0, 0);
    }
#pragma unroll
    for (int c = 0; c < 4; c += 2) {
      acc = __builtin_amdgcn_mfma_f32_16x16x4f32(xv[4 + c], w1[c], acc, 0, 0, 0);
      acc2 = __builtin_amdgcn_mfma_f32_16x16x4f32(xv[5 + c], w1[c + 1], acc2, 0, 0, 0);
    }
  }
  if (kq & 16) {
    const int k = kq - 16 - 4 * q;
    f32x4 xv;
    if (HALF_IN) {
      typedef _Float16 half4_t __attribute__((ext_vector_type(4)));
      const half4_t hv = __builtin_bit_cast(half4_t, (u32x2_od)__builtin_amdgcn_raw_buffer_load_b64(rsX, vox + (unsigned int)(k * 2), 0, AUX));
      xv = f32x4{(float)hv[0], (float)hv[1], (float)hv[2], (float)hv[3]};
    } else {
      xv = __builtin_bit_cast(f32x4, (u32x4_od)__builtin_amdgcn_raw_buffer_load_b128(rsX, vox + (unsigned int)(k * 4), 0, AUX));
    }
    f32x4 wv = __builtin_bit_cast(f32x4, (u32x4_od)__builtin_amdgcn_raw_buffer_load_b128(rsW, vow + (unsigned int)(k * 4), 0, 0));
    if (row >= 12) wv = f32x4{0.f, 0.f, 0.f, 0.f};
#pragma unroll
    for (int c = 0; c < 4; c += 2) {
      acc = __builtin_amdgcn_mfma_f32_16x16x4f32(xv[c], wv[c], acc, 0, 0, 0);
      acc2 = __builtin_amdgcn_mfma_f32_16x16x4f32(xv[c + 1], wv[c + 1], acc2, 0, 0, 0);
    }
  }
  acc += acc2;
  return acc;
}

template <bool HALF_IN, int AUX>
__device__ __forceinline__ void gcn_out_dot_rows16(const float* __restrict__ X, const OutDev& O, float* __restrict__ hs, int64_t r0, int64_t rows,
                                                   float (*part)[16][16], int tid) {
  const int lane = tid & 63, wave = tid >> 6;
  const int row = lane & 15, q = lane >> 4;
  const int64_t r = r0 + row < rows ? r0 + row : rows - 1;
  const float* Xb = (const float*)((const char*)X + (size_t)r0 * O.K * (HALF_IN ? 2 : 4));
  const f32x4 acc = gcn_out_dot_quarter<HALF_IN, AUX>(Xb, O, r - r0, wave, lane);
#pragma unroll
  for (int c = 0; c < 4; ++c) part[wave][4 * q + c][row] = acc[c];
  __syncthreads();
  if (tid < 16 * 12) {
    const int rr = tid / 12, cc = tid % 12;
    if (r0 + rr < rows) hs[(r0 + rr) * 12 + cc] = (part[0][rr][cc] + part[1][rr][cc]) + (part[2][rr][cc] + part[3][rr][cc]);
  }
}
```

### egohmr_amd/csrc/internal.h

```cpp
#pragma once
#include "common.h"
#include "egohmr_hip.h"

int ehm_smpl_forward_impl(ehm_smpl* h, const float* betas, const float* rot_or_x, bool from_rot6d, const float* mean,
                          const float* std_, float* verts, float* joints, float* Rws, float* Aws, float* pose6d_out, int B,
                          hipStream_t st, float* vposed = nullptr);
int ehm_smpl_writes_vposed(const ehm_smpl* h, int B);
int ehm_smpl_pose_impl(ehm_smpl* h, const float* betas, const float* x, const float* mean, const float* std_, float* Rws, float* Aws,
                       float* jws, int B, hipStream_t st);
int ehm_smpl_pose_rotmat_impl(ehm_smpl* h, const float* betas, const float* rotmats, float* Rws, float* Aws, float* jws, int B, hipStream_t st);
int ehm_step_body_impl(ehm_smpl* h, const float* hs, const void* out_dev, const uint8_t* vis, const float* x, const float* noise,
                       const float* grad, float* x_next, float* x0, const ehm_step_coefs* c, int ddim, int passes, const int32_t* mask_slot, int do_pose,
                       const float* betas, const float* mean, const float* std_, float* verts, float* joints, float* Rws, float* Aws,
                       float* pose6d, int B, hipStream_t st, const struct GcnInputArgs* next_input = nullptr, int next_prec = 0,
                       int* fused = nullptr, void* defer_pf = nullptr);
int ehm_skin_steps_impl(ehm_smpl* h, const float* A_steps, const void* pf_steps, int nsteps, int final_step, int B, float* verts, float* joints,
                        float* scratch_verts, float* scratch_joints, hipStream_t st);
int ehm_step_fused_impl(const void* out_dev, const float* X, int prec, const uint8_t* vis, const float* x, const float* noise, const float* grad,
                        float* x_next, float* x0, const ehm_step_coefs* c, int ddim, int passes, const int32_t* mask_slot, int B,
                        const struct GcnInputArgs* next_input, int next_prec, hipStream_t st);
int ehm_pose_steps_impl(ehm_smpl* smpl, const float* x0_steps, int nsteps, int final_step, int B, const float* betas, const float* mean,
                        const float* std_, float* A_steps, void* pf_steps, float* R, float* joints, float* pose6d, float* x0_final,
                        float* scratch_joints, hipStream_t st);
int ehm_skin_min_bodies();
int ehm_smpl_has_mfma_skin(const ehm_smpl* h);
int64_t ehm_skin_pf_bytes_per_step(int B);
void ehm_smpl_dev(const ehm_smpl* h, void* out);
size_t ehm_smpl_dev_size();
int ehm_smpl_num_verts(const ehm_smpl* h);
int ehm_smpl_num_extra(const ehm_smpl* h);
struct GcnInputArgs;
struct GcnRun;
int ehm_gcn_input_args(const ehm_gcn* h, const GcnRun& r, const float* h_img, const float* h_oth, const uint8_t* vis, const float* x, const float* Wx,
                       const float* tvec, float* out, int B, int passes, GcnInputArgs* a);
int ehm_gcn_input_impl(const ehm_gcn* h, const GcnRun& r, const float* h_img, const float* h_oth, const uint8_t* vis, const float* x,
                       const float* Wx, const float* tvec, float* out, int B, int passes, hipStream_t st);
int ehm_gcn_hidden_stack_impl(ehm_gcn* h, const GcnRun& r, float* const bufs[3], int64_t rows_pad, int* result_index, hipStream_t st);
int ehm_gcn_output_dot_impl(ehm_gcn* h, const GcnRun& r, const float* X, int B, int passes, const float** hs, hipStream_t st);
int ehm_num_cus();
int ehm_gcn_tile_layer_impl(const ehm_gcn* h, const GcnRun& r, int layer, const void* X, const void* residual, void* out, int64_t rows_pad,
                            bool out_f32, hipStream_t st);
int ehm_gcn_tile_chain_impl(ehm_gcn* h, const GcnRun& r, void* const bufs[3], int64_t rows_pad, hipStream_t st);
void ehm_pack_half(const float* X, void* Y, size_t n, float scale, hipStream_t st);
int ehm_gcn_reserve_rows(ehm_gcn* h, int64_t rows_pad);
int64_t ehm_guidance_scratch_bytes(int B, int N);
int ehm_guidance_impl(ehm_smpl* smpl, const float* betas, const float* x, const float* mean, const float* std_,
                      const float* scene, int B, int N, float tau, float denom, float margin, float* verts_ws, float* joints_ws, float* R_ws,
                      float* A_ws, float* gverts, float* loss, float* gpose, float* grad, void* scratch, hipStream_t st,
                      float* vposed_ws = nullptr);
unsigned long long* ehm_prof_evals_ptr();
struct EhmProfScope {
  int cls;
  hipStream_t st;
  void* rec;
  EhmProfScope(int cls_, hipStream_t st_);
  ~EhmProfScope();
};
```

### egohmr_amd/csrc/sampler.hip

```cpp
#include <stdarg.h>

#include "common.h"
#include "egohmr_hip.h"
#include "gcn_dev.h"
#include "internal.h"
#include "smpl_dev.h"
#include "step_dev.h"

static thread_local char g_err[512] = "";
void ehm_set_error(const char* fmt, ...) {
  va_list ap;
  va_start(ap, fmt);
  vsnprintf(g_err, sizeof(g_err), fmt, ap);
  va_end(ap);
}
extern "C" const char* ehm_last_error(void) { return g_err; }
extern "C" const char* ehm_target_arch(void) { return "gfx950"; }
extern "C" const char* ehm_build_features(void) {
  return ""
#ifdef EHM_STAMPS
         "stamps "
#endif
      ;
}

int ehm_num_cus() {
  static int n[16] = {};
  int dev = 0;
  if (hipGetDevice(&dev) != hipSuccess || dev < 0 || dev >= 16) return 256;
  if (n[dev] == 0) {
    hipDeviceProp_t prop;
    n[dev] = (hipGetDeviceProperties(&prop, dev) == hipSuccess && prop.multiProcessorCount > 0) ? prop.multiProcessorCount : 256;
  }
  return n[dev];
}

#include <vector>
namespace {
struct ProfRec { int cls; hipEvent_t a, b; };
bool g_prof_on = false;
std::vector<ProfRec*> g_prof;
unsigned long long* g_prof_evals = nullptr;
}
unsigned long long* ehm_prof_evals_ptr() { return g_prof_on ? g_prof_evals : nullptr; }
EhmProfScope::EhmProfScope(int cls_, hipStream_t st_) : cls(cls_), st(st_), rec(nullptr) {
  if (!g_prof_on) return;
  ProfRec* r = new ProfRec{cls, nullptr, nullptr};
  if (hipEventCreate(&r->a) != hipSuccess || hipEventCreate(&r->b) != hipSuccess || hipEventRecord(r->a, st) != hipSuccess) {
    delete r;
    return;
  }
  rec = r;
}
EhmProfScope::~EhmProfScope() {
  if (!rec) return;
  ProfRec* r = (ProfRec*)rec;
  (void)hipEventRecord(r->b, st);
  g_prof.push_back(r);
}
extern "C" int ehm_profile_begin(void) {
  for (ProfRec* r : g_prof) { (void)hipEventDestroy(r->a); (void)hipEventDestroy(r->b); delete r; }
  g_prof.clear();
  if (!g_prof_evals && hipMalloc(&g_prof_evals, sizeof(unsigned long long)) != hipSuccess) g_prof_evals = nullptr;
  if (g_prof_evals) (void)hipMemset(g_prof_evals, 0, sizeof(unsigned long long));
  g_prof_on = true;
  return 0;
}
extern "C" int ehm_profile_end(double* ms, int64_t* launches, int n) {
  EHM_CHECK_ARG(ms && launches && n > 0 && n <= EHM_PROF_N);
  g_prof_on = false;
  for (int i = 0; i < n; ++i) { ms[i] = 0.0; launches[i] = 0; }
  int rc = 0;
  for (ProfRec* r : g_prof) {
    float t = 0.f;
    if (hipEventSynchronize(r->b) != hipSuccess || hipEventElapsedTime(&t, r->a, r->b) != hipSuccess) rc = EHM_EIO;
    else if (r->cls >= 0 && r->cls < n) { ms[r->cls] += t; launches[r->cls] += 1; }
    (void)hipEventDestroy(r->a);
    (void)hipEventDestroy(r->b);
    delete r;
  }
  g_prof.clear();
  if (n > EHM_PROF_G_NEAREST_EVALS && g_prof_evals) {
    unsigned long long ev = 0;
    if (hipMemcpy(&ev, g_prof_evals, sizeof(ev), hipMemcpyDeviceToHost) == hipSuccess) launches[EHM_PROF_G_NEAREST_EVALS] = (int64_t)ev;
  }
  if (rc) ehm_set_error("ehm_profile_end: an event of the profile could not be read");
  return rc;
}

namespace {

__global__ void ddpm_step_kernel(const float* __restrict__ x, const float* __restrict__ x0, const float* __restrict__ noise,
                                 const float* __restrict__ grad, float* __restrict__ out, float c1, float c2, float logvar,
                                 float nz, float gscale, int64_t n) {
  int64_t i = (int64_t)blockIdx.x * blockDim.x + threadIdx.x;
  if (i >= n) return;
  float mean = __fadd_rn(__fmul_rn(c1, x0[i]), __fmul_rn(c2, x[i]));
  if (grad) mean = __fadd_rn(mean, __fmul_rn(gscale, grad[i]));
  const float sd = expf(__fmul_rn(0.5f, logvar));
  out[i] = __fadd_rn(mean, __fmul_rn(__fmul_rn(nz, sd), noise[i]));
}

__global__ void ddim_step_kernel(const float* __restrict__ x, const float* __restrict__ x0, const float* __restrict__ noise,
                                 float* __restrict__ out, float sr, float srm1, float sap, float dir, float sigma, float nz,
                                 int64_t n) {
  int64_t i = (int64_t)blockIdx.x * blockDim.x + threadIdx.x;
  if (i >= n) return;
  const float eps = __fdiv_rn(__fsub_rn(__fmul_rn(sr, x[i]), x0[i]), srm1);
  const float mean = __fadd_rn(__fmul_rn(x0[i], sap), __fmul_rn(dir, eps));
  out[i] = __fadd_rn(mean, __fmul_rn(__fmul_rn(nz, sigma), noise[i]));
}

}

extern "C" int ehm_ddpm_step(const float* x, const float* x0, const float* noise, const float* grad, float* x_next, float coef1,
                             float coef2, float log_variance, float nonzero, float grad_scale, int64_t n, void* stream) {
  EHM_CHECK_ARG(x && x0 && noise && x_next && n >= 0);
  if (n == 0) return 0;
  hipLaunchKernelGGL(ddpm_step_kernel, dim3((unsigned)ceil_div(n, 256)), dim3(256), 0, (hipStream_t)stream, x, x0, noise, grad,
                     x_next, coef1, coef2, log_variance, nonzero, grad_scale, n);
  EHM_LAUNCH_CHECK();
  return 0;
}

extern "C" int ehm_ddim_step(const float* x, const float* x0, const float* noise, float* x_next, float sqrt_recip_ac,
                             float sqrt_recipm1_ac, float sqrt_ac_prev, float dir_coef, float sigma, float nonzero, int64_t n,
                             void* stream) {
  EHM_CHECK_ARG(x && x0 && noise && x_next && n >= 0);
  if (n == 0) return 0;
  hipLaunchKernelGGL(ddim_step_kernel, dim3((unsigned)ceil_div(n, 256)), dim3(256), 0, (hipStream_t)stream, x, x0, noise, x_next,
                     sqrt_recip_ac, sqrt_recipm1_ac, sqrt_ac_prev, dir_coef, sigma, nonzero, n);
  EHM_LAUNCH_CHECK();
  return 0;
}

namespace {
constexpr int kSkinSegment = 128;
struct Workspace {
  float* X[3];
  float* x_cur;
  float* A;
  float* g_verts_in;
  float* g_joints;
  float* g_R;
  float* g_A;
  float* g_gverts;
  float* g_vposed;
  float* g_loss;
  float* g_gpose;
  float* g_grad;
  void* g_scratch;
  float* nl_qkv;
  float* nl_y;
  float* loop_A;
  void* loop_pf;
  float* loop_verts;
  float* loop_joints;
  float* loop_x0;
  int skin_seg;
  int64_t rows, rows_pad;
  int64_t total_bytes;
};

Workspace carve(const ehm_sample_desc* d, int hid, int V, int n_joints, char* base) {
  Workspace w{};
  w.rows = (int64_t)(d->B + (d->passes == 2 ? (d->num_masked >= 0 ? d->num_masked : d->B) : 0)) * kJ;
  w.rows_pad = round_up(w.rows, ehm_gcn_row_tile());
  int64_t off = 0;
  auto take = [&](int64_t floats) {
    float* p = base ? (float*)(base + off) : nullptr;
    off += round_up(floats * 4, 256);
    return p;
  };
  for (int i = 0; i < 3; ++i) w.X[i] = take(w.rows_pad * hid);
  w.x_cur = take((int64_t)d->B * kPoseDim);
  w.A = take((int64_t)d->B * kJ * 12);
  const bool guided = d->num_scene_points > 0;
  if (guided) {
    w.g_verts_in = take((int64_t)d->B * V * 3);
    w.g_joints = take((int64_t)d->B * n_joints * 3);
    w.g_R = take((int64_t)d->B * kJ * 9);
    w.g_A = take((int64_t)d->B * kJ * 12);
    w.g_gverts = take((int64_t)d->B * V * 3);
    w.g_vposed = take((int64_t)d->B * V * 3);
    w.g_loss = take(d->B);
    w.g_gpose = take((int64_t)d->B * kPoseDim);
    w.g_grad = take((int64_t)d->B * kPoseDim);
    w.g_scratch = take(ehm_guidance_scratch_bytes(d->B, d->num_scene_points) / 4 + 64);
  }
  if (d->nonlocal_ci > 0) {
    w.nl_qkv = take(w.rows * 3 * d->nonlocal_ci);
    w.nl_y = take(w.rows * d->nonlocal_ci);
  }
  if (d->B >= ehm_skin_min_bodies() && d->lbs_every_step) {
    w.skin_seg = d->num_steps < kSkinSegment ? d->num_steps : kSkinSegment;
    w.loop_A = take((int64_t)w.skin_seg * d->B * kJ * 12);
    w.loop_pf = take((int64_t)w.skin_seg * (ehm_skin_pf_bytes_per_step(d->B) / 4));
    w.loop_verts = take((int64_t)d->B * V * 3);
    w.loop_joints = take((int64_t)d->B * n_joints * 3);
    w.loop_x0 = take((int64_t)w.skin_seg * d->B * kPoseDim);
  }
  w.total_bytes = off;
  return w;
}
}

extern "C" int64_t ehm_sample_workspace_bytes(const ehm_sample_desc* d, int hid_dim, int num_verts) {
  EHM_CHECK_ARG(d && d->B > 0 && (d->passes == 1 || d->passes == 2) && hid_dim > 0 && num_verts > 0);
  return carve(d, hid_dim, num_verts, 64 + kJ, nullptr).total_bytes;
}

extern "C" int ehm_sample_loop(ehm_gcn* gcn, ehm_smpl* smpl, const ehm_sample_desc* d, const ehm_step_coefs* steps,
                               const float* h_img, const float* h_oth, const uint8_t* vis, const float* Wx, const float* tvecs,
                               const float* noise, const float* scene, const float* betas, const float* mean, const float* std_,
                               float* x_final, float* x0_final, float* verts, float* joints, float* R, float* pose6d,
                               float* trace, void* workspace, int64_t workspace_bytes, void* stream) {
  EHM_CHECK_ARG(gcn && smpl && d && steps && h_img && h_oth && vis && Wx && tvecs && noise && betas && mean && std_);
  EHM_CHECK_ARG(x_final && x0_final && verts && joints && R && pose6d && workspace);
  EHM_CHECK_ARG(d->B > 0 && d->num_steps > 0 && (d->passes == 1 || d->passes == 2));
  GcnRun base = gcn->run;
  EHM_CHECK_ARG(d->passes == 1 || base.virtual_bodies(d->B, 2) == d->B + (d->num_masked >= 0 ? d->num_masked : d->B));
  const int hid = gcn->hid, nh = gcn->num_hidden, V = ehm_smpl_num_verts(smpl);
  EHM_CHECK_ARG(nh % 2 == 0);
  bool any_guided = false;
  for (int k = 0; k < d->num_steps; ++k) any_guided |= steps[k].grad_scale != 0.f;
  EHM_CHECK_ARG(!any_guided || (scene && d->num_scene_points > 0));
  const ehm_nonlocal_params* nlp = &gcn->nonlocal;
  EHM_CHECK_ARG(d->nonlocal_ci == nlp->Ci);
  EHM_CHECK_ARG(nlp->Ci == 0 || (base.precision != EHM_PREC_F16 && d->lowprec_steps == 0));
  Workspace w = carve(d, hid, V, 64 + kJ, (char*)workspace);
  EHM_CHECK_ARG(workspace_bytes >= w.total_bytes);
  hipStream_t st = (hipStream_t)stream;
  const int B = d->B;
  const int64_t n = (int64_t)B * kPoseDim;

  for (int i = 0; i < 3; ++i)
    if (w.rows_pad > w.rows)
      EHM_HIP(hipMemsetAsync(w.X[i] + w.rows * hid, 0, (size_t)(w.rows_pad - w.rows) * hid * sizeof(float), st));
  EHM_HIP(hipMemcpyAsync(w.x_cur, noise, n * sizeof(float), hipMemcpyDeviceToDevice, st));

  int rc = 0;
  base.valid_rows = w.rows;
  const int lowprec = base.precision == EHM_PREC_F16X3 ? d->lowprec_steps : 0;
  auto prec_of = [&](int k) { return (lowprec > 0 && k < lowprec) ? (int)EHM_PREC_F16 : base.precision; };
  const bool defer_skin = w.skin_seg > 0 && d->lbs_every_step && ehm_smpl_has_mfma_skin(smpl);
  const int64_t pf_bytes_step = ehm_skin_pf_bytes_per_step(B);
  int pending = 0;
  bool pending_poses = false;
  const bool fused_steps = !d->per_step_launches && hid % 64 == 0 && (defer_skin || !d->lbs_every_step) &&
                           w.rows_pad * hid * 4 < ((int64_t)1 << 32);
  if (defer_skin && B % 32 != 0) EHM_HIP(hipMemsetAsync(w.loop_pf, 0, (size_t)w.skin_seg * pf_bytes_step, st));
  auto flush_skin = [&](bool final_step_inside) -> int {
    if (pending == 0) return 0;
    int r = 0;
    if (pending_poses)
      r = ehm_pose_steps_impl(smpl, w.loop_x0, pending, final_step_inside ? pending - 1 : -1, B, betas, mean, std_, w.loop_A, w.loop_pf, R, joints, pose6d,
                              x0_final, w.loop_joints, st);
    if (r == 0)
      r = ehm_skin_steps_impl(smpl, w.loop_A, w.loop_pf, pending, final_step_inside ? pending - 1 : -1, B, verts, joints, w.loop_verts, w.loop_joints, st);
    pending = 0;
    pending_poses = false;
    return r;
  };
  bool input_done = false;
  for (int k = 0; k < d->num_steps && rc == 0; ++k) {
    const ehm_step_coefs& c = steps[k];
    GcnRun run = base;
    run.precision = prec_of(k);
    const bool last = k == d->num_steps - 1;
    if (trace) EHM_HIP(hipMemcpyAsync(trace + (int64_t)k * n, w.x_cur, n * sizeof(float), hipMemcpyDeviceToDevice, st));
    const float* grad = nullptr;
    if (c.grad_scale != 0.f) {
      EhmProfScope ps(EHM_PROF_GUIDANCE, st);
      rc = ehm_guidance_impl(smpl, betas, w.x_cur, mean, std_, scene, B, d->num_scene_points, d->tau, d->guide_denom, d->guide_all_points ? d->tau : 0.f,
                             w.g_verts_in, w.g_joints, w.g_R, w.g_A, w.g_gverts, w.g_loss, w.g_gpose, w.g_grad, w.g_scratch, st, w.g_vposed);
      grad = w.g_grad;
    }
    if (rc == 0 && !input_done) {
      EhmProfScope ps(EHM_PROF_INPUT, st);
      rc = ehm_gcn_input_impl(gcn, run, h_img, h_oth, vis, w.x_cur, Wx, tvecs + (int64_t)k * 2 * hid, w.X[0], B, d->passes, st);
    }
    input_done = false;
    int in = 0;
    if (rc == 0) {
      const int p = run.precision;
      EhmProfScope ps(p == EHM_PREC_F16X3 ? EHM_PROF_CHAIN_F16X3 : p == EHM_PREC_F16 ? EHM_PROF_CHAIN_F16 : EHM_PROF_HIDDEN_F32, st);
      rc = ehm_gcn_hidden_stack_impl(gcn, run, w.X, w.rows_pad, &in, st);
    }
    const float* hs = nullptr;
    const void* out_dev = &gcn->out;
    const float* feat = w.X[in];
    if (rc == 0 && nlp->Ci > 0) {
      const int ci = nlp->Ci, nrows = (int)w.rows;
      ehm_conv_desc c1{feat, nlp->Wqkv, nlp->bqkv, nullptr, w.nl_qkv, nrows, 1, 1, hid, 3 * ci, 1, 1, 1, 0, 0, nlp->qkv_scale};
      rc = ehm_conv_nhwc_split(&c1, st);
      if (rc == 0) rc = ehm_nonlocal_attention(w.nl_qkv, w.nl_y, w.rows / kJ, ci, st);
      ehm_conv_desc c2{w.nl_y, nlp->Wo, nlp->bo, feat, w.X[1], nrows, 1, 1, ci, hid, 1, 1, 1, 0, 0, nlp->o_scale};
      if (rc == 0) rc = ehm_conv_nhwc_split(&c2, st);
      feat = w.X[1];
    }
    if (rc == 0 && fused_steps && (last ? defer_skin : run.precision == prec_of(k + 1))) {
      if (defer_skin && pending > 0 && !pending_poses) rc = flush_skin(false);
      const float* eps = noise + (int64_t)(1 + k) * n;
      float* dst = last ? x_final : w.x_cur;
      GcnInputArgs nin;
      if (rc == 0 && !last) rc = ehm_gcn_input_args(gcn, run, h_img, h_oth, vis, dst, Wx, tvecs + (int64_t)(k + 1) * 2 * hid, w.X[0], B, d->passes, &nin);
      if (rc == 0)
        rc = ehm_step_fused_impl(out_dev, feat, run.precision, vis, w.x_cur, eps, grad, dst, defer_skin ? w.loop_x0 + (int64_t)pending * n : x0_final,
                                 &c, d->ddim, d->passes, run.slots(d->passes), B, last ? nullptr : &nin, gcn_input_format(gcn, prec_of(k + 1)), st);
      input_done = !last;
      if (rc == 0 && defer_skin) {
        pending_poses = true;
        ++pending;
        if (pending == w.skin_seg || last) rc = flush_skin(last);
      }
      continue;
    }
    if (rc == 0 && pending_poses) rc = flush_skin(false);
    if (rc == 0) {
      EhmProfScope ps(EHM_PROF_OUT_DOT, st);
      rc = ehm_gcn_output_dot_impl(gcn, run, feat, B, d->passes, &hs, st);
    }
    if (rc == 0) {
      const float* eps = noise + (int64_t)(1 + k) * n;
      float* dst = last ? x_final : w.x_cur;
      GcnInputArgs nin;
      const GcnInputArgs* pnin = nullptr;
      if (!last && d->lbs_every_step && !defer_skin) {
        rc = ehm_gcn_input_args(gcn, run, h_img, h_oth, vis, dst, Wx, tvecs + (int64_t)(k + 1) * 2 * hid, w.X[0], B, d->passes, &nin);
        pnin = &nin;
      }
      int fused = 0;
      if (rc == 0 && defer_skin) {
        rc = ehm_step_body_impl(smpl, hs, out_dev, vis, w.x_cur, eps, grad, dst, x0_final, &c, d->ddim, d->passes, run.slots(d->passes), 1,
                                betas, mean, std_, verts, joints, R, w.loop_A + (int64_t)pending * B * kJ * 12, pose6d, B, st, nullptr, 0, nullptr,
                                (char*)w.loop_pf + (int64_t)pending * pf_bytes_step);
        ++pending;
        if (rc == 0 && (pending == w.skin_seg || last)) rc = flush_skin(last);
      } else if (rc == 0) {
        rc = ehm_step_body_impl(smpl, hs, out_dev, vis, w.x_cur, eps, grad, dst, x0_final, &c, d->ddim, d->passes, run.slots(d->passes),
                                (d->lbs_every_step || last) ? 1 : 0,
                                betas, mean, std_, verts, joints, R, w.A, pose6d, B, st, pnin, gcn_input_format(gcn, prec_of(k + 1)), &fused);
      }
      input_done = fused != 0;
    }
  }
  return rc;
}
```

### egohmr_amd/csrc/step.hip

```cpp
#include "common.h"
#include "egohmr_hip.h"
#include "gcn_dev.h"
#include "internal.h"
#include "smpl_dev.h"
#include "step_dev.h"

namespace {

struct StepFusedArgs {
  const float* X;
  StepBodyArgs sb;
  GcnInputArgs in;
  int do_input;
};

constexpr int kFusedT = kJ * 256;

template <bool HALF_IN, int OUT, int NT>
__global__ __launch_bounds__(NT, 4) void step_fused_kernel(StepFusedArgs a) {
  constexpr int G = NT / 256, NWV = NT / 64;
  __shared__ __attribute__((aligned(16))) float T[G * kFusedT];
  __shared__ __attribute__((aligned(16))) StepBodyLds L;
  const int tid = threadIdx.x, lane = tid & 63, wave = tid >> 6;
  const int b = blockIdx.x, B = a.sb.B;
  const int slot = a.sb.passes == 2 ? (a.sb.mask_slot ? a.sb.mask_slot[b] : b) : -1;
  const int nrows = slot >= 0 ? 2 * kJ : kJ;

  float (*part)[4][16][16] = (float (*)[4][16][16])T;
  for (int task = wave; task < 12; task += NWV) {
    const int tile = task >> 2, wq = task & 3;
    if (16 * tile < nrows) {
      int rr = 16 * tile + (lane & 15);
      if (rr >= nrows) rr = nrows - 1;
      const int64_t r = (int64_t)(rr >= kJ ? B + slot : b) * kJ + (rr % kJ);
      const f32x4 acc = gcn_out_dot_quarter<HALF_IN, 0>(a.X, a.sb.O, r, wq, lane);
#pragma unroll
      for (int c = 0; c < 4; ++c) part[tile][wq][4 * (lane >> 4) + c][lane & 15] = acc[c];
    }
  }
  if (wave == NWV - 1) step_stage_tables<true>(b, lane, a.sb, L);
  __syncthreads();
  for (int i = tid; i < 2 * kJ * 12; i += NT) {
    const int rr = i / 12, cc12 = i % 12, tile = rr >> 4, tr = rr & 15;
    (&L.sh[0][0][0])[i] = rr < nrows ? (part[tile][0][tr][cc12] + part[tile][1][tr][cc12]) + (part[tile][2][tr][cc12] + part[tile][3][tr][cc12]) : 0.f;
  }
  __syncthreads();
  if (wave < 3) {
    SmplDev unused;
    step_body_one<true, false, true>(b, lane, a.sb, unused, L, [] {}, wave, 3);
  }
  if (!a.do_input) return;
  __syncthreads();
  const int ny = a.in.ny, np = slot >= 0 ? 2 : 1, grp = tid >> 8;
  const int rounds = np * ((ny + G - 1) / G);
  for (int k = 0; k < rounds; ++k) {
    const int cb = grp + G * (k / np), p = k % np;
    if (cb < ny) gcn_input_body<OUT, true>(T + grp * kFusedT, tid & 255, p ? B + slot : b, cb, a.in, L.xn);
    else __syncthreads();
    __syncthreads();
  }
}

struct PoseStepsArgs {
  const float* x0_steps;
  const float *betas, *mean, *std_;
  float* A_steps; char* pf_steps; int64_t pf_bytes;
  float *R, *joints, *pose6d, *x0_final, *scratch_joints;
  int B, final_step, jstride;
};

__global__ __launch_bounds__(64) void pose_steps_kernel(PoseStepsArgs p, SmplDev S) {
  __shared__ StepBodyLds L;
  const int b = blockIdx.x, s = blockIdx.y, lane = threadIdx.x;
  const bool fin = s == p.final_step;
  StepBodyArgs a{};
  a.betas = p.betas; a.mean = p.mean; a.std_ = p.std_; a.B = p.B; a.jstride = p.jstride;
  a.Rws = fin ? p.R : nullptr;
  a.joints = fin ? p.joints : p.scratch_joints;
  a.pose6d = fin ? p.pose6d : nullptr;
  a.Aws = p.A_steps + (size_t)s * p.B * kJ * 12;
  a.pf = (sk_half8*)(p.pf_steps + (size_t)s * p.pf_bytes);
  const float* x0row = p.x0_steps + ((size_t)s * p.B + b) * kPoseDim;
  for (int e = lane; e < kPoseDim; e += 64) {
    const float v = x0row[e];
    L.x0s[e] = v;
    if (fin) p.x0_final[(size_t)b * kPoseDim + e] = v;
  }
  __syncthreads();
  step_pose_part(b, lane, a, S, L, [] { __syncthreads(); }, L.x0s);
}

template <bool HALF_IN, int NT>
void launch_fused2(int next_prec, int B, hipStream_t st, const StepFusedArgs& a) {
  const dim3 grid((unsigned)B), blk(NT);
  if (next_prec == EHM_PREC_F32) hipLaunchKernelGGL((step_fused_kernel<HALF_IN, 0, NT>), grid, blk, 0, st, a);
  else if (next_prec == EHM_PREC_F16X3) hipLaunchKernelGGL((step_fused_kernel<HALF_IN, 1, NT>), grid, blk, 0, st, a);
  else hipLaunchKernelGGL((step_fused_kernel<HALF_IN, 2, NT>), grid, blk, 0, st, a);
}
template <bool HALF_IN>
void launch_fused(int next_prec, int B, hipStream_t st, const StepFusedArgs& a) {
  if (B <= ehm_num_cus()) launch_fused2<HALF_IN, 1024>(next_prec, B, st, a);
  else if (B > 2 * ehm_num_cus()) launch_fused2<HALF_IN, 256>(next_prec, B, st, a);
  else launch_fused2<HALF_IN, 512>(next_prec, B, st, a);
}

}

int ehm_step_fused_impl(const void* out_dev, const float* X, int prec, const uint8_t* vis, const float* x, const float* noise, const float* grad,
                        float* x_next, float* x0, const ehm_step_coefs* c, int ddim, int passes, const int32_t* mask_slot, int B,
                        const GcnInputArgs* next_input, int next_prec, hipStream_t st) {
  StepFusedArgs a{};
  a.X = X;
  a.sb.hs = nullptr; a.sb.O = *(const OutDev*)out_dev; a.sb.vis = vis; a.sb.x = x; a.sb.noise = noise; a.sb.grad = grad; a.sb.x_next = x_next;
  a.sb.x0 = x0; a.sb.c = *c; a.sb.ddim = ddim; a.sb.passes = passes; a.sb.B = B; a.sb.do_pose = 0; a.sb.mask_slot = mask_slot;
  a.sb.trace = nullptr; a.sb.pf = nullptr;
  if (a.sb.O.K % 64 != 0) {
    ehm_set_error("ehm_step_fused_impl: hidden width %d is not a multiple of 64", a.sb.O.K);
    return EHM_EINVAL;
  }
  a.do_input = next_input ? 1 : 0;
  if (next_input) a.in = *next_input;
  EhmProfScope ps(EHM_PROF_STEP_FUSED, st);
  if (prec == EHM_PREC_F16) launch_fused<true>(next_prec, B, st, a);
  else launch_fused<false>(next_prec, B, st, a);
  EHM_LAUNCH_CHECK();
  return 0;
}

int ehm_pose_steps_impl(ehm_smpl* smpl, const float* x0_steps, int nsteps, int final_step, int B, const float* betas, const float* mean,
                        const float* std_, float* A_steps, void* pf_steps, float* R, float* joints, float* pose6d, float* x0_final,
                        float* scratch_joints, hipStream_t st) {
  SmplDev sd;
  ehm_smpl_dev(smpl, &sd);
  PoseStepsArgs p{x0_steps, betas, mean, std_, A_steps, (char*)pf_steps, ehm_skin_pf_bytes_per_step(B), R, joints, pose6d, x0_final, scratch_joints,
                  B, final_step, (kJ + ehm_smpl_num_extra(smpl)) * 3};
  EhmProfScope ps(EHM_PROF_STEP_BODY, st);
  hipLaunchKernelGGL(pose_steps_kernel, dim3(B, nsteps), dim3(64), 0, st, p, sd);
  EHM_LAUNCH_CHECK();
  return 0;
}
```

### egohmr_amd/fused.py

```python
from __future__ import annotations

import ctypes as C
import dataclasses
from functools import partial
from types import SimpleNamespace

import torch

from . import _lib
from . import smpl as smpl_mod

PRECISIONS = {"f32": 0, "f16x3": 1, "f16": 2}

def pass_map(need):
    need = need.reshape(-1).bool()
    rank = torch.cumsum(need, 0, dtype=torch.int32) - 1
    mask_slot = torch.where(need, rank, torch.full_like(rank, -1)).contiguous()
    mask_items = torch.nonzero(need).reshape(-1).to(torch.int32).contiguous()
    return mask_items, mask_slot, int(mask_items.numel())


@dataclasses.dataclass
class _Prepared:
    B: int
    h_img: torch.Tensor
    h_oth: torch.Tensor
    vis: torch.Tensor
    vis_bool: torch.Tensor
    betas: torch.Tensor
    scene: torch.Tensor
    transl: torch.Tensor
    fx: torch.Tensor
    cam_cx: torch.Tensor
    cam_cy: torch.Tensor
    img_feats: torch.Tensor
    scene_feats: torch.Tensor
    finite: torch.Tensor
    mask_items: torch.Tensor
    mask_slot: torch.Tensor
    num_masked: int
    inputs: list = None

    PER_ITEM = ("h_img", "h_oth", "vis", "vis_bool", "betas", "scene", "transl", "fx", "cam_cx", "cam_cy", "img_feats", "scene_feats", "finite")

    def take(self, index):
        if isinstance(index, int):
            if index >= self.B:
                return self
            index = torch.arange(index, device=self.vis.device)
        index = index.to(self.vis.device, torch.long)
        picked = {k: getattr(self, k).index_select(0, index).contiguous() for k in self.PER_ITEM}
        mask_items, mask_slot, num_masked = pass_map(~picked["vis_bool"].all(dim=1))
        return dataclasses.replace(self, B=int(index.numel()), mask_items=mask_items, mask_slot=mask_slot, num_masked=num_masked, **picked)

    def tile(self, S):
        B, nm = self.B, max(self.num_masked, 0)
        off = torch.arange(S, device=self.mask_slot.device, dtype=torch.int32).view(-1, 1)
        slot = self.mask_slot.view(1, -1)
        tiled = {k: getattr(self, k).repeat(S, *([1] * (getattr(self, k).dim() - 1))).contiguous() for k in self.PER_ITEM}
        return dataclasses.replace(
            self, B=S * B, mask_items=(self.mask_items.view(1, -1) + off * B).reshape(-1).contiguous(),
            mask_slot=torch.where(slot >= 0, slot + off * nm, torch.full_like(slot, -1)).reshape(-1).contiguous(),
            num_masked=S * self.num_masked if self.num_masked >= 0 else self.num_masked, **tiled)


class FusedSampler:

    def __init__(self, model):
        self._model_ref = [model]
        self._gcn = self._gcn_key = self._folded = None
        self._nl_set = None
        self._pk = self._ck = None
        self._prep = self._prep_key = None
        self._joint_map = self._count_host = None
        self._beta_key = self._beta_w = None
        self._tv_cache = None
        self._ws, self._graphs = None, {}
        self._status_host = self._status_event = None
        self._sched_cache = {}
        self.schedule_info = None
        self.last_lowprec = 0
        self.last_trace = None

    @property
    def model(self):
        return self._model_ref[0]

    def _param_key(self):
        self._pk = self._pk or _lib.TensorKey(self.model.diffusion_model, self.model.input_process)
        return self._pk()

    def gcn(self):
        key = self._param_key()
        if self._gcn is None or key != self._gcn_key:
            if self._gcn is not None:
                self._gcn.close()
            m = self.model
            dm = m.diffusion_model
            gi = dm.gconv_input[0]
            h, keep = dm.create_native_handle(m.device)
            self._gcn, self._gcn_key = _lib.Handle(h, _lib.api().ehm_gcn_destroy, keep), key
            W = gi.gconv.W.detach().double()
            Wp, bp = m.input_process.poseEmbedding.weight.detach().double(), m.input_process.poseEmbedding.bias.detach().double()
            a, b, c, d = m.cond_split
            Wx = torch.einsum("ec,kef->kcf", Wp, W[:, b:c, :])
            bx = torch.einsum("e,kef->kf", bp, W[:, b:c, :])
            hid = dm.hid_dim
            Wd = gi.gconv.W.detach().float()
            k_oth = (b - a + 31) // 32 * 32
            W_img_cat = Wd[:, :a, :].permute(1, 0, 2).reshape(a, 2 * hid).contiguous()
            W_oth_cat = torch.zeros(k_oth, 2 * hid, device=m.device)
            W_oth_cat[:b - a] = Wd[:, a:b, :].permute(1, 0, 2).reshape(b - a, 2 * hid)
            self._folded = SimpleNamespace(Wx=Wx.float().contiguous(), bx=bx, W_t=W[:, c:d, :], W_img_cat=W_img_cat, W_oth_cat=W_oth_cat, k_oth=k_oth)
        A = _lib.api()
        A.ehm_gcn_set_uncond_mode(self._gcn, 0 if self.model.only_mask_img_cond else 1)
        mode = PRECISIONS[self.model.gcn_precision]
        if A.ehm_gcn_get_precision(self._gcn) != mode:
            A.ehm_gcn_set_precision(self._gcn, mode)
        if self.model.diffusion_model.nonlocal_layer:
            ((wq, sq, bq), (wo, so, bo)), nl_key = self.model.diffusion_model.nonlocal_packed()
            if self._nl_set != (nl_key, self._gcn.serial):
                p = _lib.NonlocalParams(_lib.ptr(wq), _lib.ptr(bq), sq, _lib.ptr(wo), _lib.ptr(bo), so, self.model.diffusion_model.non_local.inter_channels)
                A.ehm_gcn_set_nonlocal(self._gcn, C.byref(p))
                self._nl_set = (nl_key, self._gcn.serial)
        return self._gcn

    def _backbone_fn(self):
        return self.model.backbone.current()

    @torch.no_grad()
    def prepare(self, batch) -> _Prepared:
        with _lib.on_device(self.model.device):
            return self._prepare_on_device(batch)

    def _prepare_on_device(self, batch) -> _Prepared:
        m = self.model
        ins = [batch["img"], batch["scene_pcd_verts_full"], batch["orig_keypoints_2d"], batch["fx"], batch["cam_cx"], batch["cam_cy"],
               batch["box_center"], batch["box_size"], batch["smpl_params"]["transl"]]
        if ins[0].shape[0] == 0:
            raise ValueError("empty batch (the reference fails on it too: egohmr.py:233 reshapes x_t [0, 144] to [0, 24, -1])")
        if m.encoder_precision not in ("f16x3", "f16"):
            raise ValueError(f"EgoHMR.encoder_precision must be 'f16x3' or 'f16', not {m.encoder_precision!r}")
        m.backbone.hi_only = m.scene_enc.hi_only = m.encoder_precision == "f16"
        switches = (bool(m.with_bbox_info), bool(m.with_cam_center), bool(m.scene_cano), tuple(m.openpose_to_smpl), m.encoder_precision)
        key = tuple((id(t), t._version, t.data_ptr()) for t in ins) + self._param_key() + self._cond_param_key() + (switches,)
        if self._prep is not None and self._prep_key == key:
            return self._prep
        self.gcn()
        dev = m.device
        g = lambda k: _lib.f32(batch[k], dev)
        transl = _lib.f32(batch["smpl_params"]["transl"], dev)
        scene = g("scene_pcd_verts_full")
        if m.scene_cano:
            scene = scene - transl.unsqueeze(1)
        scene = scene.contiguous()
        img = g("img")
        B, f, st = img.shape[0], self._folded, _lib.stream_ptr()
        kp = g("orig_keypoints_2d")
        fx, cx, cy, bc, bs = g("fx"), g("cam_cx"), g("cam_cy"), g("box_center"), g("box_size")
        te = m.transl_enc.layers
        tw = [_lib.f32(te[0].weight, dev), _lib.f32(te[0].bias, dev), _lib.f32(te[2].weight, dev), _lib.f32(te[2].bias, dev)]
        n_scene, n_tr = m.scene_enc.fc_c.out_features, te[2].out_features
        n_other = n_scene + n_tr + 1 + (3 if m.with_bbox_info else 0) + (2 if m.with_cam_center else 0)
        jm = self._joint_map
        if kp.dim() != 3 or kp.shape[2] != 3 or not all(0 <= int(k) < kp.shape[1] for k in m.openpose_to_smpl):
            raise ValueError(f"orig_keypoints_2d must be [B, NK, 3] with NK > max(openpose_to_smpl) = {max(m.openpose_to_smpl)}; got {tuple(kp.shape)}")
        if jm is None or jm[0] != (tuple(m.openpose_to_smpl), str(dev)):
            jm = self._joint_map = ((tuple(m.openpose_to_smpl), str(dev)), torch.tensor(m.openpose_to_smpl, dtype=torch.int32, device=dev))
        oth = torch.empty(B, f.k_oth, device=dev)
        vis = torch.empty(B, 24, dtype=torch.uint8, device=dev)
        flags = torch.empty(2, B, dtype=torch.uint8, device=dev)
        maps = torch.empty(2 * B + 1, dtype=torch.int32, device=dev)
        sums = (img.reshape(B, -1).sum(dim=1), scene.reshape(B, -1).sum(dim=1))
        P = _lib.ptr
        d = _lib.ItemPrepDesc(keypoints_2d=P(kp), joint_map=P(jm[1]), NK=kp.shape[1], force_visible=8, fx=P(fx), cx=P(cx),
                              cy=P(cy), box_center=P(bc), box_size=P(bs), transl=P(transl), fx_norm=m.cfg.CAM.FX_NORM_COEFF,
                              with_bbox=int(m.with_bbox_info), with_cam_center=int(m.with_cam_center), tW1=P(tw[0]), tb1=P(tw[1]),
                              tW2=P(tw[2]), tb2=P(tw[3]), t_hidden=te[0].out_features, t_out=n_tr, img_rowsum=P(sums[0]),
                              scene_rowsum=P(sums[1]), other=P(oth), other_ld=f.k_oth, other_col0=n_scene, vis=P(vis),
                              mask_slot=P(maps), mask_items=P(maps[B:]), count=P(maps[2 * B:]), finite=P(flags),
                              need_scratch=P(flags[1]), pass_group=1, B=B)
        _lib.api().ehm_item_prep(C.byref(d), st)
        if self._count_host is None:
            self._count_host = torch.zeros(1, dtype=torch.int32).pin_memory()
        self._count_host.copy_(maps[2 * B:], non_blocking=True)
        count_ready = torch.cuda.Event()
        count_ready.record(torch.cuda.current_stream(dev))
        img_feats = self._backbone_fn()(img)
        scene_feats = m.scene_enc(scene)
        oth[:, :n_scene].copy_(scene_feats)
        h_img, h_oth, betas = self._project(img_feats.contiguous(), oth, n_other)
        bad = (flags[0] == 0).view(B, 1, 1)
        h_img.masked_fill_(bad, 0.0)
        h_oth.masked_fill_(bad, 0.0)
        count_ready.synchronize()
        num_masked = int(self._count_host[0])
        self._prep = _Prepared(B=B, h_img=h_img, h_oth=h_oth, vis=vis, vis_bool=vis.view(torch.bool),
                               betas=betas, scene=scene, transl=transl, fx=fx, cam_cx=cx, cam_cy=cy, img_feats=img_feats,
                               scene_feats=scene_feats, finite=flags[0].view(torch.bool), mask_items=maps[B:B + num_masked],
                               mask_slot=maps[:B], num_masked=num_masked, inputs=ins)
        self._prep_key = key
        return self._prep

    def _project(self, img_feats, oth, n_other):
        m, f, A = self.model, self._folded, _lib.api()
        B, dev, hid = img_feats.shape[0], img_feats.device, m.diffusion_model.hid_dim
        st = _lib.stream_ptr()
        a = img_feats.shape[1]
        l1, l2 = m.beta_layer.layers[0], m.beta_layer.layers[2]
        if a % 32 or l1.out_features % 32 or l1.in_features != a + n_other or l2.out_features > 32:
            raise _lib.EgoHMRHipError(f"conditioning widths the projection kernels are not built for: image features {a}, beta head "
                                      f"{l1.in_features} -> {l1.out_features} -> {l2.out_features}, other features {n_other}")
        h_img = torch.empty(B, 2, hid, device=dev)
        h_oth = torch.empty(B, 2, hid, device=dev)
        A.ehm_skinny_gemm_f32(img_feats, f.W_img_cat, None, h_img, B, a, 2 * hid, 0, st)
        A.ehm_skinny_gemm_f32(oth, f.W_oth_cat, None, h_oth, B, f.k_oth, 2 * hid, 0, st)
        ib = m.beta_layer.init_betas
        key = tuple((t.data_ptr(), t._version) for t in (l1.weight, l1.bias, l2.weight, l2.bias, ib)) + (str(dev),)
        if self._beta_key != key:
            Wt = torch.zeros(a + f.k_oth, l1.out_features, device=dev)
            w = l1.weight.detach().float().to(dev)
            Wt[:a] = w[:, :a].t()
            Wt[a:a + n_other] = w[:, a:].t()
            W2 = torch.zeros(l1.out_features, 32, device=dev)
            W2[:, :l2.out_features] = l2.weight.detach().float().to(dev).t()
            b2 = torch.zeros(32, device=dev)
            b2[:l2.out_features] = (l2.bias.detach().float().to(dev) + ib.detach().float().to(dev).reshape(-1))
            self._beta_w = (Wt.contiguous(), l1.bias.detach().float().to(dev).contiguous(), W2.contiguous(), b2)
            self._beta_key = key
        W1, b1, W2, b2 = self._beta_w
        xb = torch.cat([img_feats, oth], dim=1)
        hb = torch.empty(B, l1.out_features, device=dev)
        A.ehm_skinny_gemm_f32(xb, W1, b1, hb, B, xb.shape[1], l1.out_features, 1, st)
        b32 = torch.empty(B, 32, device=dev)
        A.ehm_skinny_gemm_f32(hb, W2, b2, b32, B, l1.out_features, 32, 0, st)
        return h_img, h_oth, b32[:, :l2.out_features].contiguous()

    def _cond_param_key(self):
        m = self.model
        self._ck = self._ck or _lib.TensorKey(m.backbone, m.scene_enc, m.transl_enc, m.beta_layer, m.embed_timestep)
        return self._ck()

    def _apply_pass_map(self, st, passes):
        m, A = self.model, _lib.api()
        h = self.gcn()
        if passes == 2 and m.prune_passes:
            A.ehm_gcn_set_pass_map(h, st.mask_items if st.num_masked else None, st.mask_slot, st.num_masked)
            return st.B + st.num_masked, st.num_masked
        A.ehm_gcn_set_pass_map(h, None, None, -1)
        return passes * st.B, -1

    def invalidate(self, structure: bool = False):
        self._prep, self._prep_key = None, None
        if structure:
            self._pk = self._ck = None

    @torch.no_grad()
    def timestep_vectors(self, t_orig) -> torch.Tensor:
        m = self.model
        self.gcn()
        ckey = None
        if not torch.is_tensor(t_orig):
            ckey = (self._param_key(), self._cond_param_key(), tuple(int(t) for t in t_orig))
            if self._tv_cache is not None and self._tv_cache[0] == ckey:
                return self._tv_cache[1]
            t_orig = torch.tensor(ckey[2], device=m.device, dtype=torch.long)
        temb = m.embed_timestep.time_embed(m.sequence_pos_encoder.pe[t_orig][:, 0])
        tv = torch.einsum("ne,kef->nkf", temb.double(), self._folded.W_t) + self._folded.bx[None]
        tv = tv.float().contiguous()
        if ckey is not None:
            self._tv_cache = (ckey, tv)
        return tv

    @staticmethod
    def step_table(diffusion, ddim, cond_grad_weight, guided):
        cache = diffusion.__dict__.setdefault("_ehm_step_tables", {})
        fp = hash((diffusion.betas.tobytes(), tuple(getattr(diffusion, "timestep_map", ()))))
        key = (bool(ddim), float(cond_grad_weight), bool(guided), fp)
        if key not in cache:
            T = diffusion.num_timesteps
            rows = [diffusion.step_coefs(i, ddim, 0.0, cond_grad_weight, guided) for i in range(T - 1, -1, -1)]
            first_guided = next((i for i, r in enumerate(rows) if r.grad_scale != 0.0), T)
            cache[key] = ((_lib.StepCoefs * T)(*rows), first_guided)
        return cache[key]

    @staticmethod
    def guided_steps(diffusion, ddim, cond_grad_weight, guided) -> int:
        return diffusion.num_timesteps - FusedSampler.step_table(diffusion, ddim, cond_grad_weight, guided)[1]

    def _workspace(self, nbytes, device):
        if self._ws is None or self._ws.numel() < nbytes or self._ws.device != device:
            self._ws = torch.empty(int(nbytes), dtype=torch.uint8, device=device)
        return self._ws

    @torch.no_grad()
    def denoise_once(self, st, x_t, tvec, passes):
        m, A = self.model, _lib.api()
        rows = self._apply_pass_map(st, passes)[0] * 24
        h = self.gcn()
        fill = lambda X0: A.ehm_gcn_input_layer(h, st.h_img, st.h_oth, st.vis, x_t, self._folded.Wx, tvec, X0, st.B, passes, _lib.stream_ptr())
        return m.diffusion_model.denoiser_tail(h, fill, rows=rows, B=st.B, passes=passes, vis=st.vis, precision=m.gcn_precision, device=m.device)

    @torch.no_grad()
    def collision(self, verts, scene, want_grad=True, want_hits=False, all_points=None):
        m = self.model
        verts, scene = _lib.f32(verts, m.device), _lib.f32(scene, m.device)
        B, V, N = verts.shape[0], verts.shape[1], scene.shape[1]
        loss = torch.empty(B, device=m.device)
        gverts = torch.empty_like(verts) if want_grad else None
        hits = torch.empty(B, device=m.device, dtype=torch.int32) if want_hits else None
        allp = m.guide_all_points if all_points is None else all_points
        with torch.cuda.device(m.device):
            _lib.api().ehm_collision_query(verts, scene, loss, gverts, hits, B, V, N, m.collision_tau, int(bool(allp)), _lib.stream_ptr())
        return loss, gverts, hits

    @torch.no_grad()
    def guidance_gradient(self, st, x, betas):
        m, A = self.model, _lib.api()
        B = x.shape[0]
        mean, std = m._std_mean()
        verts = torch.empty(B, m.smpl.num_verts, 3, device=m.device)
        joints = torch.empty(B, m.smpl.num_joints_out, 3, device=m.device)
        s = _lib.stream_ptr()
        A.ehm_smpl_forward_rot6d(m.smpl.handle(), betas, x, mean, std, verts, joints, None, None, None, B, s)
        loss, gverts, _ = self.collision(verts, st.scene)
        gpose = torch.empty(B, 144, device=m.device)
        A.ehm_smpl_backward_rot6d(m.smpl.handle(), betas, x, mean, std, gverts, gpose, B, s)
        grad = torch.empty(B, 144, device=m.device)
        denom = self.guide_denom(B)
        A.ehm_guidance_grad_finish(gpose, loss, grad, B, denom, s)
        return grad

    def guide_denom(self, B: int) -> float:
        m = self.model
        if m.guide_reduction != "mean":
            return 1.0
        return float(m.guide_denom_override) if m.guide_denom_override else float(B)

    def schedule_key(self, diffusion, ddim: bool, n_guided: int, cond_grad_weight: float = 0.0, guide_denom: float = 1.0):
        m = self.model
        return (self._param_key(), self._cond_param_key(), tuple(diffusion.timestep_map), int(getattr(diffusion, "original_num_steps", diffusion.num_timesteps)),
                bool(ddim), int(n_guided), (float(cond_grad_weight), str(m.guide_reduction)) if n_guided else None, bool(m.guide_all_points) if n_guided else False,
                bool(m.diffuse_fuse),
                float(m.schedule_tol))

    def lowprec_steps(self, T: int, guided=False, ddim: bool = True, key=None) -> int:
        k = self.model.f16x3_last_steps
        if k is None or self.model.gcn_precision != "f16x3":
            return 0
        if k == "auto":
            info = self._sched_cache.get(key) if key is not None else None
            if info is None:
                return 0
            k = info["k"]
        return max(0, T - int(k))

    @staticmethod
    def _k_ladder(T: int, floor: int = 2):
        ks, x = [], float(max(floor, 2))
        while x < T:
            if not ks or int(round(x)) > ks[-1]:
                ks.append(int(round(x)))
            x *= 4.0 / 3.0
        return [k for k in ks if k < T] + [T]

    @staticmethod
    def pick_k(ladder, err_a, err_b, bar):
        lo, hi = 0, len(ladder) - 1
        while lo < hi:
            mid = (lo + hi) // 2
            if err_a(ladder[mid]) <= bar:
                hi = mid
            else:
                lo = mid + 1
        idx = lo
        while idx < len(ladder) - 1 and err_b(ladder[idx]) > bar:
            idx += 1
        return idx

    @torch.no_grad()
    def calibrate_schedule(self, diffusion, batch=None, ddim=False, guided=False, cond_grad_weight=1.0, tol=None, bodies=64, prepared=None,
                           seeds=(20260929, 20260930), force=False, denom_items=None, n_guided=None):
        m = self.model
        if m.gcn_precision != "f16x3":
            raise _lib.EgoHMRHipError("calibrate_schedule: the precision schedule only exists for gcn_precision='f16x3'")
        tol = float(m.schedule_tol if tol is None else tol)
        st_full = prepared if prepared is not None else self.prepare(batch)
        T = diffusion.num_timesteps
        if n_guided is None:
            n_guided = self.guided_steps(diffusion, ddim, cond_grad_weight, guided)
        denom_items = int(denom_items or st_full.B)
        old_tol, m.schedule_tol = m.schedule_tol, tol
        try:
            key = self.schedule_key(diffusion, ddim, n_guided, cond_grad_weight, self.guide_denom(denom_items))
        finally:
            m.schedule_tol = old_tol
        if not force and key in self._sched_cache:
            return self._sched_cache[key]
        good = torch.nonzero(st_full.finite).reshape(-1)
        if good.numel() == 0:
            return {"k": int(T), "T": int(T), "f16_steps": 0, "tol_m": tol, "criterion": "no item with finite inputs in the batch: not calibrated, not cached",
                    "bodies": 0, "ddim": bool(ddim), "guided_steps": int(n_guided), "trials": []}
        st = st_full.take(good[torch.arange(int(bodies), device=good.device) % good.numel()])
        nb, dev = st.B, m.device
        sub_batch = dict(batch) if batch is not None else {}

        def loop(noise, lowprec):
            r = self.run(diffusion, sub_batch, noise, ddim=ddim, guided=guided, cond_grad_weight=cond_grad_weight, prepared=st,
                         denom_items=denom_items, lowprec=lowprec)
            o = r["other_outputs"]
            return o["pred_vertices"].clone(), o["pred_keypoints_3d"].clone()

        def dist(a, b):
            return max(float((a[0] - b[0]).norm(dim=-1).max()), float((a[1] - b[1]).norm(dim=-1).max()))

        draws, refs, tried = [], [], {}
        for sd_ in seeds:
            g = torch.Generator(device=dev).manual_seed(int(sd_))
            draws.append(torch.randn(T + 1, nb, 144, device=dev, generator=g))
        refs.append(loop(draws[0], 0))
        ladder = self._k_ladder(T, floor=(n_guided + 8) if n_guided else 2)

        def err(k, d):
            if (k, d) not in tried:
                tried[(k, d)] = 0.0 if k >= T else dist(loop(draws[d], T - k), refs[d])
            return tried[(k, d)]

        def err1(k):
            if ladder[-1] > k and len(refs) < 2:
                refs.append(loop(draws[1], 0))
            return err(k, 1)

        idx = self.pick_k(ladder, lambda k: err(k, 0), err1, 0.5 * tol)
        k = ladder[idx]
        info = {"k": int(k), "T": int(T), "f16_steps": int(T - k), "tol_m": tol, "criterion": "max vertex/joint distance to the all-f16x3 loop <= tol/2 on two noise draws",
                "bodies": int(nb), "ddim": bool(ddim), "guided_steps": int(n_guided),
                "trials": sorted([{"k": kk, "draw": d, "max_dist_m": e} for (kk, d), e in tried.items()], key=lambda r: (r["k"], r["draw"]))}
        self._sched_cache[key] = info
        self.schedule_info = info
        return info

    def install_schedule(self, diffusion, info, ddim=False, guided=False, cond_grad_weight=1.0, denom_items=1):
        T = diffusion.num_timesteps
        n_guided = self.guided_steps(diffusion, ddim, cond_grad_weight, guided)
        assert int(info["T"]) == T, (info["T"], T)
        self._sched_cache[self.schedule_key(diffusion, ddim, n_guided, cond_grad_weight, self.guide_denom(int(denom_items)))] = dict(info)
        self.schedule_info = dict(info)

    @torch.no_grad()
    def measure_gain(self, batch=None, timesteps=(0,), prepared=None, bodies=16, delta=1e-2, seed=7):
        m = self.model
        st = (prepared if prepared is not None else self.prepare(batch)).take(bodies)
        g = torch.Generator(device=m.device).manual_seed(seed)
        x = torch.randn(st.B, 144, device=m.device, generator=g)
        d = torch.randn(st.B, 144, device=m.device, generator=g)
        d = d / d.norm(dim=1, keepdim=True) * delta
        passes = 2 if m.diffuse_fuse else 1
        out = {}
        for t in timesteps:
            tv = self.timestep_vectors(torch.tensor([int(t)], device=m.device))[0]
            a = self.denoise_once(st, x, tv, passes).clone()
            b = self.denoise_once(st, (x + d).contiguous(), tv, passes)
            out[int(t)] = float(((b - a).norm(dim=1) / delta).mean())
        return out

    @torch.no_grad()
    def run_samples(self, diffusion, batch, noise_stacks, ddim=False, guided=False, cond_grad_weight=1.0, defer_status=False):
        S = len(noise_stacks)
        st = self.prepare(batch)
        if S == 1:
            return [self.run(diffusion, batch, noise_stacks[0], ddim=ddim, guided=guided, cond_grad_weight=cond_grad_weight, prepared=st,
                             defer_status=defer_status)]
        B = st.B
        width = int(getattr(self.model, "loop_bodies", 0) or 0)
        g = S if width <= 0 else max(1, min(S, width // max(B, 1)))
        outs = []
        for s0 in range(0, S, g):
            outs += self._run_sample_group(diffusion, batch, st, noise_stacks[s0:s0 + g], ddim, guided, cond_grad_weight, defer_status)
        m = self.model
        m.scene_pcd_verts, m.input_transl = st.scene, st.transl
        m.focal_length, m.camera_center_full = m.focal_length[:B], m.camera_center_full[:B]
        last = outs[-1]["other_outputs"]
        m.smpl_output = smpl_mod.SMPLOutput(vertices=last["pred_vertices"], joints=last["pred_keypoints_3d"],
                                            full_pose=torch.cat([last["pred_smpl_params"]["global_orient"], last["pred_smpl_params"]["body_pose"]], dim=1))
        return outs

    def _run_sample_group(self, diffusion, batch, st, noise_stacks, ddim, guided, cond_grad_weight, defer_status):
        S, B, T = len(noise_stacks), st.B, diffusion.num_timesteps
        run = partial(self.run, diffusion, dict(batch), ddim=ddim, guided=guided, cond_grad_weight=cond_grad_weight, denom_items=B, defer_status=defer_status)
        if S == 1:
            return [run(noise_stack=noise_stacks[0], prepared=st)]
        res = run(noise_stack=torch.cat([_lib.f32(n, self.model.device)[: T + 1] for n in noise_stacks], dim=1), prepared=st.tile(S))

        def split(x):
            if torch.is_tensor(x):
                return list(x.reshape(S, B, *x.shape[1:]).unbind(0)) if x.dim() >= 1 and x.shape[0] == S * B else [x] * S
            if isinstance(x, dict):
                parts = {k: split(v) for k, v in x.items()}
                return [{k: parts[k][i] for k in x} for i in range(S)]
            return [x] * S
        return split(res)

    @torch.no_grad()
    def run(self, diffusion, batch, noise_stack, ddim=False, guided=False, cond_grad_weight=1.0, trace=False, prepared=None, denom_items=None,
            defer_status=False, lowprec=None):
        m = self.model
        if guided and getattr(m, "collision_model", None) is not None:
            raise _lib.EgoHMRHipError("FusedSampler.run(guided=True): the one-call loop cannot call the attached collision_model between steps and will "
                                      "not fall back to the build's proxy; sample through diffusion.p_sample_loop / ddim_sample_loop / val_losses")
        call = dict(diffusion=diffusion, batch=batch, noise_stack=noise_stack, ddim=ddim, guided=guided, cond_grad_weight=cond_grad_weight, trace=trace,
                    prepared=prepared, denom_items=denom_items)
        with _lib.on_device(m.device):
            try:
                return self._run_on_device(**call, defer_status=defer_status, lowprec=lowprec)
            except _lib.EgoHMRRangeError:
                if m.on_saturation != "f32" or m.gcn_precision == "f32":
                    raise
                import warnings
                warnings.warn("egohmr_amd: a denoiser activation reached the f16 range (|x| >= 65504) and was clamped in the split-f16 / f16 path; "
                              "EgoHMR.on_saturation = 'f32': switching this model to gcn_precision = 'f32' and re-running the call", RuntimeWarning)
                m.gcn_precision = "f32"
                return self._run_on_device(**call, defer_status=False, lowprec=None)

    def _run_on_device(self, *, diffusion, batch, noise_stack, ddim, guided, cond_grad_weight, trace, prepared, denom_items, defer_status, lowprec):
        m = self.model
        nonlocal_ci = m.diffusion_model.non_local.inter_channels if m.diffusion_model.nonlocal_layer else 0
        if nonlocal_ci and m.gcn_precision == "f16":
            raise _lib.EgoHMRHipError(m.diffusion_model.NONLOCAL_F16)
        if self._status_event is not None and self._status_event.query():
            self.check_status()
        st = prepared if prepared is not None else self.prepare(batch)
        B, T = st.B, diffusion.num_timesteps
        noise = _lib.f32(noise_stack, m.device)
        assert noise.shape[0] >= T + 1 and noise.shape[1] == B and noise.shape[2] == 144, noise.shape
        steps, first_guided = self.step_table(diffusion, ddim, cond_grad_weight, guided)
        any_guided = first_guided < T
        tvecs = self.timestep_vectors([diffusion.timestep_map[i] for i in range(T - 1, -1, -1)])
        if nonlocal_ci:
            lowprec = 0
        elif lowprec is None:
            lowprec = self._scheduled_lowprec(diffusion=diffusion, batch=batch, st=st, ddim=ddim, guided=guided, cond_grad_weight=cond_grad_weight,
                                              n_guided=T - first_guided, denom_items=denom_items or B)
        self.last_lowprec = int(lowprec)
        desc, nbytes = self._describe(st=st, T=T, ddim=ddim, any_guided=any_guided, denom_items=denom_items or B, lowprec=lowprec, nonlocal_ci=nonlocal_ci)
        gcn, smpl_h = self.gcn(), m.smpl.handle()
        launch = partial(self._launch, gcn=gcn, smpl_h=smpl_h, desc=desc, steps=steps, nbytes=nbytes, any_guided=any_guided)
        ins = dict(h_img=st.h_img, h_oth=st.h_oth, vis=st.vis, tvecs=tvecs, noise=noise[: T + 1].contiguous(), betas=st.betas, scene=st.scene)
        graph = m.use_hip_graph is True or (m.use_hip_graph == "auto" and desc.passes * B <= 64)
        tr = torch.empty(T, B, 144, device=m.device) if trace else None
        with torch.cuda.device(m.device):
            if graph and not any_guided and not trace:
                o = self._replay(launch=launch, gcn=gcn, smpl_h=smpl_h, desc=desc, steps=steps, nbytes=nbytes, st=st, ins=ins)
            else:
                o = SimpleNamespace(**ins, **self._out_bufs(B))
                launch(bufs=o, ws=self._workspace(nbytes, m.device), tr=tr)
        return self._finish(batch=batch, st=st, o=o, tr=tr, noise=noise, T=T, guided_ddim=ddim and any_guided, gcn=gcn, defer_status=defer_status)

    def _scheduled_lowprec(self, *, diffusion, batch, st, ddim, guided, cond_grad_weight, n_guided, denom_items):
        m, skey = self.model, None
        if m.f16x3_last_steps == "auto" and m.gcn_precision == "f16x3":
            skey = self.schedule_key(diffusion, ddim, n_guided, cond_grad_weight, self.guide_denom(denom_items))
            if skey not in self._sched_cache and m.auto_calibrate:
                self.calibrate_schedule(diffusion, batch, ddim=ddim, guided=guided, cond_grad_weight=cond_grad_weight, prepared=st,
                                        denom_items=denom_items, n_guided=n_guided)
            self.schedule_info = self._sched_cache.get(skey)
        return self.lowprec_steps(diffusion.num_timesteps, n_guided, ddim, key=skey)

    def _describe(self, *, st, T, ddim, any_guided, denom_items, lowprec, nonlocal_ci):
        m = self.model
        passes = 2 if m.diffuse_fuse else 1
        _, num_masked = self._apply_pass_map(st, passes)
        desc = _lib.SampleDesc(B=st.B, passes=passes, num_steps=T, ddim=int(ddim), per_step_launches=int(bool(m.per_step_launches)),
                               lbs_every_step=int(m.lbs_every_step), num_scene_points=st.scene.shape[1] if any_guided else 0,
                               guide_denom=self.guide_denom(denom_items), tau=m.collision_tau, num_masked=num_masked,
                               guide_all_points=int(bool(m.guide_all_points)), lowprec_steps=int(lowprec), nonlocal_ci=int(nonlocal_ci))
        return desc, _lib.api().ehm_sample_workspace_bytes(C.byref(desc), m.diffusion_model.hid_dim, m.smpl.num_verts)

    def _out_bufs(self, B):
        smpl = self.model.smpl
        shapes = dict(x_final=(144,), x0=(144,), verts=(smpl.num_verts, 3), joints=(smpl.num_joints_out, 3), R=(24, 3, 3), pose6d=(144,))
        return {k: torch.empty(B, *shape, device=self.model.device) for k, shape in shapes.items()}

    def _launch(self, *, gcn, smpl_h, desc, steps, nbytes, any_guided, bufs, ws, tr):
        mean, std = self.model._std_mean()
        _lib.api().ehm_sample_loop(gcn, smpl_h, C.byref(desc), steps, bufs.h_img, bufs.h_oth, bufs.vis, self._folded.Wx, bufs.tvecs, bufs.noise,
                                   bufs.scene if any_guided else None, bufs.betas, mean, std, bufs.x_final, bufs.x0, bufs.verts, bufs.joints, bufs.R,
                                   bufs.pose6d, tr, ws, nbytes, _lib.stream_ptr())

    def _replay(self, *, launch, gcn, smpl_h, desc, steps, nbytes, st, ins):
        m, dev = self.model, self.model.device
        ins = dict(ins, mask_items=st.mask_items, mask_slot=st.mask_slot)
        mean, std = m._std_mean()
        key = (st.B, desc.num_steps, desc.ddim, desc.passes, desc.lbs_every_step, desc.lowprec_steps, m.gcn_precision, gcn.serial,
               bytes(steps), st.scene.shape[1], desc.num_masked, smpl_h.serial,
               mean.data_ptr(), std.data_ptr(), self._folded.Wx.data_ptr(), self._nl_set)
        ent = self._graphs.get(key)
        if ent is None:
            if len(self._graphs) >= 8:
                self._graphs.clear()
            bufs = SimpleNamespace(**{k: torch.empty_like(v) for k, v in ins.items()}, **self._out_bufs(st.B))
            ws = torch.empty(int(nbytes), dtype=torch.uint8, device=dev)
            for k, v in ins.items():
                getattr(bufs, k).copy_(v)
            if desc.num_masked >= 0:
                _lib.api().ehm_gcn_set_pass_map(gcn, bufs.mask_items if desc.num_masked else None, bufs.mask_slot, desc.num_masked)
            launch(bufs=bufs, ws=ws, tr=None)
            torch.cuda.synchronize(dev)
            g = torch.cuda.CUDAGraph()
            with torch.cuda.graph(g):
                launch(bufs=bufs, ws=ws, tr=None)
            ent = self._graphs[key] = SimpleNamespace(graph=g, bufs=bufs, ws=ws)
        for k, v in ins.items():
            getattr(ent.bufs, k).copy_(v)
        ent.graph.replay()
        return SimpleNamespace(**{k: getattr(ent.bufs, k).clone() for k in ("x_final", "x0", "verts", "joints", "R", "pose6d")})

    def _finish(self, *, batch, st, o, tr, noise, T, guided_ddim, gcn, defer_status):
        m, A = self.model, _lib.api()
        self.last_trace = tr
        if tr is not None:
            batch["x_t"] = tr[-1]
        batch["vis_mask_smpl"] = st.vis_bool
        out = m._pack_output(batch, st, o.x0, o.pose6d, o.R, o.verts, o.joints, chk=noise, chk_rows=T, last_noise=noise[T], x_final=o.x_final)
        with torch.cuda.device(m.device):
            if defer_status:
                if self._status_host is None:
                    self._status_host = torch.zeros(1, dtype=torch.int32).pin_memory()
                A.ehm_gcn_stack_status_async(gcn, self._status_host.data_ptr(), _lib.stream_ptr())
                self._status_event = torch.cuda.Event()
                self._status_event.record()
            else:
                A.ehm_gcn_stack_status(gcn, _lib.stream_ptr())
                m.backbone.check_status()
        return {"sample": o.x_final, "pred_xstart": o.x_final if guided_ddim else o.x0, "other_outputs": out}

    def check_status(self):
        self.model.backbone.check_status()
        if self._status_event is None:
            return
        self._status_event.synchronize()
        self._status_event = None
        if int(self._status_host[0]) != 0:
            self._status_host.zero_()
            with torch.cuda.device(self.model.device):
                _lib.api().ehm_gcn_stack_status(self.gcn(), _lib.stream_ptr())
```

### include/egohmr_hip.h

```cpp
#ifndef EGOHMR_HIP_H
#define EGOHMR_HIP_H

#include <stddef.h>
#include <stdint.h>

#ifdef __cplusplus
extern "C" {
#endif

#define EHM_NUM_JOINTS 24
#define EHM_NUM_BETAS 10
#define EHM_POSE_DIM 144

const char* ehm_last_error(void);
const char* ehm_target_arch(void);
const char* ehm_build_features(void);

int ehm_rot6d_to_rotmat(const float* x6d, float* R, int64_t n, int mode, void* stream);
int ehm_rot6d_to_rotmat_bwd(const float* x6d, const float* gR, float* gx, int64_t n, int mode, void* stream);
int ehm_rotmat_to_angle_axis(const float* R, float* aa, int64_t n, void* stream);
int ehm_rotmat_to_angle_axis_bwd(const float* R, const float* gaa, float* gR, int64_t n, void* stream);

typedef struct ehm_smpl ehm_smpl;

int ehm_smpl_create(ehm_smpl** out, const float* v_template, const float* shapedirs, const float* posedirs,
                    const float* J_regressor, const float* lbs_weights, const int32_t* parents,
                    const int32_t* extra_joint_vertex_ids, int num_verts, int n_extra, void* stream);
void ehm_smpl_destroy(ehm_smpl* h);

int ehm_smpl_forward(ehm_smpl* h, const float* betas, const float* rotmats, float* verts, float* joints,
                     float* A_out, int B, void* stream);

int ehm_smpl_forward_rot6d(ehm_smpl* h, const float* betas, const float* x, const float* mean, const float* std,
                           float* verts, float* joints, float* R_out, float* pose6d_out, float* A_out, int B,
                           void* stream);

typedef struct {
  const float* W;
  const float* M;
  const float* adj2;
  const float* bias;
  const float* bn_weight;
  const float* bn_bias;
  const float* bn_mean;
  const float* bn_var;
  int in_dim;
  int out_dim;
} ehm_gconv_params;

typedef struct ehm_gcn ehm_gcn;

int ehm_gcn_create(ehm_gcn** out, const float* adj, const ehm_gconv_params* input_conv,
                   const ehm_gconv_params* hidden, int num_hidden, const ehm_gconv_params* output_conv,
                   int hid_dim, void* stream);
void ehm_gcn_destroy(ehm_gcn* h);

int ehm_gcn_set_precision(ehm_gcn* h, int mode);
int ehm_gcn_get_precision(const ehm_gcn* h);
int ehm_gcn_activation_group(const ehm_gcn* h);
int ehm_gcn_reserve(ehm_gcn* h, int max_bodies, int passes);
int ehm_gcn_pack_activations(const float* X, void* X2, int64_t rows, int K, int group, void* stream);
int ehm_gcn_unpack_activations(const void* X2, float* X, int64_t rows, int K, int group, void* stream);
int ehm_gcn_pack_activations_checked(ehm_gcn* h, const float* X, void* X2, int64_t rows, void* stream);

int ehm_gcn_row_tile(void);

int ehm_gcn_set_uncond_mode(ehm_gcn* h, int masks_whole_condition);
int ehm_gcn_set_pass_map(ehm_gcn* h, const int32_t* mask_items, const int32_t* mask_slot, int num_masked);
typedef struct {
  const void* Wqkv; const float* bqkv; float qkv_scale;
  const void* Wo; const float* bo; float o_scale;
  int Ci;
} ehm_nonlocal_params;
int ehm_gcn_set_nonlocal(ehm_gcn* h, const ehm_nonlocal_params* p);
int ehm_gcn_input_layer(ehm_gcn* h, const float* h_img, const float* h_oth, const uint8_t* vis, const float* x,
                        const float* Wx, const float* tvec, float* out, int B, int passes, void* stream);
int ehm_gcn_input_layer_rows(ehm_gcn* h, const float* pre, float* out, int bodies, void* stream);

int ehm_gcn_hidden_layer(ehm_gcn* h, int layer, const float* X, const float* residual, float* out,
                         int64_t rows_pad, void* stream);

int ehm_gcn_hidden_stack(ehm_gcn* h, float* const bufs[3], int64_t rows_pad, int* result_index, void* stream);
int ehm_gcn_stack_status(ehm_gcn* h, void* stream);
int ehm_gcn_stack_status_async(ehm_gcn* h, uint32_t* host_flag, void* stream);

int ehm_gcn_output_layer(ehm_gcn* h, const float* X, const uint8_t* vis, float* x0, int B, int passes,
                         void* stream);

#define EHM_GCN_CONV_INPUT (-1)
#define EHM_GCN_CONV_OUTPUT (-2)
int ehm_gcn_bwd_epilogue(const ehm_gcn* h, int conv, const float* gout, const float* gate, float* G, int ldg, int bodies, void* stream);
int ehm_gcn_bwd_params_workspace_bytes(const ehm_gcn* h, int conv, int bodies, int64_t* bytes);
int ehm_gcn_bwd_params(const ehm_gcn* h, int conv, const float* gout, const float* gate, const float* pre, int ld_pre, int bodies,
                       float* gM, float* gadj2, float* gbias, float* gbn_weight, float* gbn_bias, void* workspace, int64_t workspace_bytes,
                       void* stream);

typedef struct {
  const void* A0;
  const void* A1;
  const void* W;
  const float* bias;
  const float* group_bias;
  void* Y;
  float* colmax;
  int64_t M;
  int N, K0, K1;
  int rows_per_group;
  int valid_rows_per_group;
  int relu_in0;
  int relu_out;
  float w_scale;
  const float* lift_points;
  const float* lift_W4;
  int hi_only;
  int group_bias_stride;
} ehm_linear_desc;
int ehm_linear_split(const ehm_linear_desc* d, void* stream);
int ehm_split_pack(const float* X, void* X2, int64_t rows, int K, int K_padded, float scale, void* stream);
int ehm_pointnet_lift(const float* pts, const float* Wpos, const float* bpos, void* R0, void* P32, int B, int N, int N_padded,
                      int C, void* stream);

int ehm_skinny_gemm_f32(const float* X, const float* W, const float* bias, float* Y, int M, int K, int N, int relu, void* stream);


size_t ehm_resnet_stem_scratch_bytes(int N, int H, int W);
int ehm_resnet_stem(const float* img, const float* Wt, const float* bias, float* scratch, float* y, int N, int H, int W,
                    int out_x2, void* stream);

typedef struct ehm_conv_desc {
  const float* x; const void* W; const float* bias; const float* residual; float* y;
  int N, H, Wd, Ci, Co;
  int KH, KW, stride, pad, relu;
  float w_scale;
} ehm_conv_desc;
int ehm_conv_nhwc_split(const ehm_conv_desc* d, void* stream);

typedef struct ehm_conv_x2_desc {
  const void* x; int64_t x_rows; const void* W; const float* bias; const void* residual; void* y;
  int N, H, Wd, Ci, Co;
  int KH, KW, stride, pad, relu;
  float w_scale;
  void* workspace;
  int64_t workspace_bytes;
  const void* x2; int64_t x2_rows;
  int H2, W2, Ci2, stride2;
  int hi_only;
  int workspace_clean;
} ehm_conv_x2_desc;
int64_t ehm_conv_x2_rows(int64_t pixels);
int64_t ehm_conv_x2_workspace_bytes(const ehm_conv_x2_desc* d);
int ehm_conv_x2(const ehm_conv_x2_desc* d, void* stream);
int ehm_conv_x2_workspace_status(void* workspace, uint32_t* host_flag, void* stream);
int ehm_x2_group_mean(const void* X, float* Y, int groups, int rows_per_group, int C, int hi_only , void* stream);

int ehm_nonlocal_attention(const float* qkv, float* y, int64_t bodies, int Ci, void* stream);

int ehm_ddpm_step(const float* x, const float* x0, const float* noise, const float* grad, float* x_next,
                  float coef1, float coef2, float log_variance, float nonzero, float grad_scale, int64_t n,
                  void* stream);
int ehm_ddim_step(const float* x, const float* x0, const float* noise, float* x_next, float sqrt_recip_ac,
                  float sqrt_recipm1_ac, float sqrt_ac_prev, float dir_coef, float sigma, float nonzero,
                  int64_t n, void* stream);

int ehm_collision_proxy(const float* verts, const float* scene, float* loss, float* gverts, int B, int V, int N,
                        float tau, void* stream);

int ehm_collision_query(const float* verts, const float* scene, float* loss, float* gverts, int32_t* hits, int B, int V, int N,
                        float tau, int all_points, void* stream);

int ehm_smpl_backward_rot6d(ehm_smpl* h, const float* betas, const float* x, const float* mean, const float* std,
                            const float* gverts, float* gpose6d, int B, void* stream);

int ehm_smpl_backward(ehm_smpl* h, const float* betas, const float* rotmats, const float* gverts, const float* gjoints, float* gbetas,
                      float* grotmats, int B, void* workspace, int64_t workspace_bytes, void* stream);
int ehm_smpl_backward_workspace_bytes(const ehm_smpl* h, int B, int64_t* bytes);

int ehm_guidance_grad_finish(const float* gpose6d, const float* loss, float* grad, int B, float denom, void* stream);

int ehm_nn_dist2(const float* x, const float* y, float* dist2, int32_t* idx, int B, int P1, int P2, void* stream);

typedef struct ehm_eval_points_desc {
  const float* pred; const float* gt; const float* pred_origin; const float* gt_origin; const uint8_t* mask;
  float* per_point; float* mean; float* vis_sum; float* invis_sum;
  int B, S, P, pred_points, gt_points, origin_point;
} ehm_eval_points_desc;
int ehm_eval_point_errors(const ehm_eval_points_desc* d, void* stream);
int ehm_eval_procrustes(const float* pred, const float* gt, const uint8_t* mask, float* aligned, float* per_joint, float* mean, float* vis_sum,
                        float* invis_sum, int B, int S, int J, void* stream);
int ehm_eval_procrustes_vis(const float* pred, const float* gt, const uint8_t* align_mask, float* aligned, float* per_joint, float* mean, float* vis_sum,
                            float* invis_sum, int B, int S, int J, void* stream);
int ehm_eval_diversity(const float* joints, const uint8_t* mask, int invert, float* std_out, float* apd_out, int B, int S, int J, void* stream);

typedef struct ehm_stage1_desc {
  const float* img_feats;
  const float* scene_feats;
  const float* fx; const float* cam_cx; const float* cam_cy; const float* box_center ; const float* box_size;
  const float* W1t; const float* b1; const float* W2; const float* b2; const float* init_cam; const float* init_betas;
  float* pred_cam;
  float* pred_cam_full;
  float* pred_betas;
  float fx_norm, crop_res;
  int with_cam_center, with_bbox_info, with_focal_length;
  int img_dim, scene_dim, hidden, B;
} ehm_stage1_desc;
int ehm_stage1_head(const ehm_stage1_desc* d, void* stream);

#define EHM_SCENE_GROUP 8
#define EHM_SCENE_PARAMS 64
#define EHM_SCENE_MAX_CHAIN 4
#define EHM_SCENE_P_CHAIN 0
#define EHM_SCENE_P_COS 0
#define EHM_SCENE_P_SIN 1
#define EHM_SCENE_P_CX 2
#define EHM_SCENE_P_CZ 3
#define EHM_SCENE_P_XMIN 4
#define EHM_SCENE_P_XMAX 5
#define EHM_SCENE_P_ZMIN 6
#define EHM_SCENE_P_ZMAX 7
#define EHM_SCENE_P_CUBE 8
#define EHM_SCENE_P_OUT 48
enum { EHM_SCENE_WHOLE = 0, EHM_SCENE_CUBE = 1 };
enum { EHM_SCENE_OK = 0, EHM_SCENE_TOO_FEW = 1, EHM_SCENE_EMPTY_CROP = 2 };
typedef struct ehm_scene_desc {
  const double* verts;
  int64_t total_verts;
  const int64_t* mesh_offsets;
  int num_meshes;
  int64_t max_mesh_verts;
  const int32_t* groups;
  int num_groups;
  const double* params;
  int mode, chain_len, B, target, stride;
  float* points;
  int64_t* index;
  int64_t* n_selected;
  int32_t* status;
  void* workspace;
  int64_t workspace_bytes;
} ehm_scene_desc;
int ehm_scene_workspace_bytes(const ehm_scene_desc* d, int64_t* bytes);
int ehm_scene_select(const ehm_scene_desc* d, void* stream);

typedef struct ehm_item_prep_desc {
  const float* keypoints_2d;
  const int32_t* joint_map;
  int NK, force_visible;
  const float *fx, *cx, *cy, *box_center, *box_size, *transl;
  float fx_norm;
  int with_bbox, with_cam_center;
  const float *tW1, *tb1, *tW2, *tb2;
  int t_hidden, t_out;
  const float *img_rowsum, *scene_rowsum;
  float* other;
  int other_ld, other_col0;
  uint8_t* vis;
  int32_t *mask_slot, *mask_items, *count;
  uint8_t* finite;
  uint8_t* need_scratch;
  int pass_group;
  int B;
} ehm_item_prep_desc;
int ehm_item_prep(const ehm_item_prep_desc* d, void* stream);

typedef struct ehm_pack_desc {
  int B, J, V;
  const uint8_t* finite;
  const float* chk;
  int chk_rows;
  const float* last_noise;
  float* x_final;
  float *x0, *pose6d, *R, *verts, *joints;
  const float* betas_in;
  float* betas_out;
  const float *transl, *fx, *cx, *cy;
  float fx_norm;
  float *global_orient, *body_pose, *kp3d_full, *kp2d_full, *focal, *center;
  uint8_t* finite_out;
} ehm_pack_desc;
int ehm_pack_outputs(const ehm_pack_desc* d, void* stream);

enum {
  EHM_LOSS_TOTAL = 0, EHM_LOSS_V2V = 1, EHM_LOSS_KP3D = 2, EHM_LOSS_KP3D_FULL = 3, EHM_LOSS_KP2D_FULL = 4, EHM_LOSS_BETAS = 5, EHM_LOSS_BODY_POSE = 6,
  EHM_LOSS_GLOBAL_ORIENT = 7, EHM_LOSS_POSE_6D_ORTHO = 8, EHM_LOSS_PENETRATION = 9, EHM_LOSS_KP3D_VIS_SUM = 10, EHM_LOSS_TERMS = 11
};
typedef struct ehm_val_losses_desc {
  int B, V, pred_joints, gt_joints, kp3d_points, kp3d_full_points, kp2d_points;
  const float *pred_vertices, *pred_keypoints_3d, *pred_keypoints_3d_full, *pred_keypoints_2d_full;
  const float *pred_global_orient, *pred_body_pose, *pred_betas, *pred_pose_6d;
  const float *keypoints_2d, *keypoints_3d, *keypoints_3d_full;
  const float *gt_vertices_male, *gt_vertices_female, *gt_joints_male, *gt_joints_female;
  const int64_t* gender;
  const float *gt_global_orient, *gt_body_pose, *gt_betas;
  const float *focal, *center;
  const float* penetration;
  double weights[9];
  void* workspace;
  int64_t workspace_bytes;
  float* losses;
  int64_t* joint_vis_num;
  float* per_item;
  int64_t* per_item_vis;
  uint8_t* vis_mask;
} ehm_val_losses_desc;
int ehm_val_losses_workspace_bytes(int B, int V, int64_t* bytes);
int ehm_val_losses(const ehm_val_losses_desc* d, void* stream);

int ehm_scene_cap_points(const float* verts, const float* scene, float* scene_out, int32_t* count, int B, int V, int N, int cap, void* stream);

typedef struct {
  float coef1, coef2, log_variance, variance;
  float sqrt_recip_ac, sqrt_recipm1_ac, sqrt_ac_prev, dir_coef, sigma;
  float nonzero;
  float grad_scale;
} ehm_step_coefs;

typedef struct {
  int B;
  int passes;
  int num_steps;
  int ddim;
  int lbs_every_step;
  int num_scene_points;
  float guide_denom;
  float tau;
  int num_masked;
  int guide_all_points;
  int lowprec_steps;
  int nonlocal_ci;
  int per_step_launches;
} ehm_sample_desc;

int64_t ehm_sample_workspace_bytes(const ehm_sample_desc* d, int hid_dim, int num_verts);
int ehm_sample_loop(ehm_gcn* gcn, ehm_smpl* smpl, const ehm_sample_desc* d, const ehm_step_coefs* steps,
                    const float* h_img, const float* h_oth, const uint8_t* vis, const float* Wx, const float* tvecs,
                    const float* noise, const float* scene, const float* betas, const float* mean, const float* std,
                    float* x_final, float* x0_final, float* verts, float* joints, float* R, float* pose6d,
                    float* trace, void* workspace, int64_t workspace_bytes, void* stream);

enum {
  EHM_PROF_INPUT = 0,
  EHM_PROF_CHAIN_F16X3 = 1,
  EHM_PROF_CHAIN_F16 = 2,
  EHM_PROF_HIDDEN_F32 = 3,
  EHM_PROF_OUT_DOT = 4,
  EHM_PROF_STEP_BODY = 5,
  EHM_PROF_SKIN_INPUT = 6,
  EHM_PROF_GUIDANCE = 7,
  EHM_PROF_RESERVED_8 = 8,
  EHM_PROF_RESERVED_9 = 9,
  EHM_PROF_G_NEAREST = 10,
  EHM_PROF_G_SKIN_BWD = 11,
  EHM_PROF_G_POSEFEAT_BWD = 12,
  EHM_PROF_STEP_FUSED = 13,
  EHM_PROF_G_NEAREST_EVALS = 14,
  EHM_PROF_N = 15
};
int ehm_profile_begin(void);
int ehm_profile_end(double* ms, int64_t* launches, int n);

#ifdef __cplusplus
}
#endif
#endif
```

Before: 2278 bodies/s.

## Precompute step-invariant condition contribution table for GCN input layer

Splits the GCN input-layer graph convolution by linearity. The image and other-condition terms, which do not change across denoising steps, are precomputed once per sampling run into a [B,24,hid] table E. Each step then convolves only the x/time part and adds E for the conditioned pass. The fused step kernel now emits both the conditioned and masked virtual bodies from one convolution instead of two, halving input-conv rounds per body. The cost is reading a sizeable table every step, plus extra memory and a cache key in the Python path, and relu is applied after the sum, which may slightly change rounding.

```diff
diff --git a/egohmr_amd/_lib.py b/egohmr_amd/_lib.py
--- a/egohmr_amd/_lib.py
+++ b/egohmr_amd/_lib.py
@@ -210,6 +210,8 @@
     "ehm_gcn_unpack_activations": (_I, [_P, _P, _L, _I, _I, _P]),
     "ehm_gcn_pack_activations_checked": (_I, [_P, _P, _P, _L, _P]),
     "ehm_gcn_input_layer": (_I, [_P, _P, _P, _P, _P, _P, _P, _P, _I, _I, _P]),
+    "ehm_gcn_cond_table": (_I, [_P, _P, _P, _P, _I, _P, _P]),
+    "ehm_gcn_input_layer_cond": (_I, [_P, _P, _P, _P, _P, _P, _P, _P, _P, _I, _I, _P]),
     "ehm_gcn_input_layer_rows": (_I, [_P, _P, _P, _I, _P]),
     "ehm_gcn_hidden_layer": (_I, [_P, _I, _P, _P, _P, _L, _P]),
     "ehm_gcn_hidden_stack": (_I, [_P, C.POINTER(C.c_void_p), _L, C.POINTER(C.c_int), _P]),
diff --git a/egohmr_amd/csrc/gcn.hip b/egohmr_amd/csrc/gcn.hip
--- a/egohmr_amd/csrc/gcn.hip
+++ b/egohmr_amd/csrc/gcn.hip
@@ -224,7 +224,13 @@
 template <int OUT>
 __global__ __launch_bounds__(256) void gcn_input_rows_kernel(GcnInputArgs a) {
   __shared__ __attribute__((aligned(16))) float T[kJ * 256];
-  gcn_input_body<OUT, false, true>(T, (int)threadIdx.x, blockIdx.x, blockIdx.y, a, nullptr);
+  gcn_input_body<OUT, false, true>(T, (int)threadIdx.x, (int)blockIdx.x, -1, (int)blockIdx.x, (int)blockIdx.y, a, nullptr);
+}
+
+__global__ __launch_bounds__(256) void gcn_cond_table_kernel(const float* __restrict__ h_img, const float* __restrict__ h_oth, const uint8_t* __restrict__ vis,
+                                                             LayerDev L, int mask_all, float* __restrict__ E) {
+  const int n = blockIdx.x * 256 + threadIdx.x;
+  if (n < L.N) gcn_cond_table_body(h_img, h_oth, vis, L, mask_all, (int)blockIdx.y, n, E);
 }
 
 
@@ -407,6 +413,7 @@
 extern "C" void ehm_gcn_destroy(ehm_gcn* h) {
   if (!h) return;
   (void)hipFree(h->arena);
+  if (h->cond_E) (void)hipFree(h->cond_E);
   if (h->hs) (void)hipFree(h->hs);
   if (h->hidden_dev) (void)hipFree(h->hidden_dev);
   if (h->chain_sync) (void)hipFree(h->chain_sync);
@@ -414,11 +421,11 @@
   delete h;
 }
 
-int ehm_gcn_input_args(const ehm_gcn* h, const GcnRun& r, const float* h_img, const float* h_oth, const uint8_t* vis, const float* x, const float* Wx,
-                       const float* tvec, float* out, int B, int passes, GcnInputArgs* a) {
-  EHM_CHECK_ARG(h && h_img && h_oth && vis && x && Wx && tvec && out && a);
+int ehm_gcn_input_args(const ehm_gcn* h, const GcnRun& r, const float* h_img, const float* h_oth, const uint8_t* vis, const float* E, const float* x,
+                       const float* Wx, const float* tvec, float* out, int B, int passes, GcnInputArgs* a) {
+  EHM_CHECK_ARG(h && h_img && h_oth && vis && E && x && Wx && tvec && out && a);
   EHM_CHECK_ARG(B > 0 && (passes == 1 || passes == 2));
-  a->h_img = h_img; a->h_oth = h_oth; a->vis = vis; a->x = x; a->Wx = Wx; a->tvec = tvec;
+  a->h_img = h_img; a->h_oth = h_oth; a->vis = vis; a->E = E; a->x = x; a->Wx = Wx; a->tvec = tvec;
   a->L = h->input;
   a->Y = out;
   a->B = B; a->passes = passes; a->mask_all = r.uncond_masks_all;
@@ -444,19 +451,54 @@
   return 0;
 }
 
-int ehm_gcn_input_impl(const ehm_gcn* h, const GcnRun& r, const float* h_img, const float* h_oth, const uint8_t* vis, const float* x,
+int ehm_gcn_input_impl(const ehm_gcn* h, const GcnRun& r, const float* h_img, const float* h_oth, const uint8_t* vis, const float* E, const float* x,
                        const float* Wx, const float* tvec, float* out, int B, int passes, hipStream_t st) {
   GcnInputArgs a;
-  const int rc = ehm_gcn_input_args(h, r, h_img, h_oth, vis, x, Wx, tvec, out, B, passes, &a);
+  const int rc = ehm_gcn_input_args(h, r, h_img, h_oth, vis, E, x, Wx, tvec, out, B, passes, &a);
   return rc != 0 ? rc : input_conv<false>(a, gcn_input_format(h, r.precision), st);
+}
+
+int ehm_gcn_cond_table_impl(const ehm_gcn* h, const GcnRun& r, const float* h_img, const float* h_oth, const uint8_t* vis, int B, float* E, hipStream_t st) {
+  EHM_CHECK_ARG(h && h_img && h_oth && vis && E && B > 0);
+  hipLaunchKernelGGL(gcn_cond_table_kernel, dim3((unsigned)ceil_div(h->hid, 256), (unsigned)B), dim3(256), 0, st, h_img, h_oth, vis, h->input,
+                     r.uncond_masks_all, E);
+  EHM_LAUNCH_CHECK();
+  return 0;
+}
+
+extern "C" int ehm_gcn_cond_table(ehm_gcn* h, const float* h_img, const float* h_oth, const uint8_t* vis, int B, float* E, void* stream) {
+  EHM_CHECK_ARG(h);
+  return ehm_gcn_cond_table_impl(h, h->run, h_img, h_oth, vis, B, E, (hipStream_t)stream);
+}
+
+extern "C" int ehm_gcn_input_layer_cond(ehm_gcn* h, const float* h_img, const float* h_oth, const uint8_t* vis, const float* E, const float* x,
+                                        const float* Wx, const float* tvec, float* out, int B, int passes, void* stream) {
+  EHM_CHECK_ARG(h);
+  const int rc = ehm_gcn_input_impl(h, h->run, h_img, h_oth, vis, E, x, Wx, tvec, out, B, passes, (hipStream_t)stream);
+  if (rc == 0) h->run.valid_rows = (int64_t)h->run.virtual_bodies(B, passes) * kJ;
+  return rc;
 }
 
 extern "C" int ehm_gcn_input_layer(ehm_gcn* h, const float* h_img, const float* h_oth, const uint8_t* vis, const float* x,
                                    const float* Wx, const float* tvec, float* out, int B, int passes, void* stream) {
-  EHM_CHECK_ARG(h);
-  const int rc = ehm_gcn_input_impl(h, h->run, h_img, h_oth, vis, x, Wx, tvec, out, B, passes, (hipStream_t)stream);
-  if (rc == 0) h->run.valid_rows = (int64_t)h->run.virtual_bodies(B, passes) * kJ;
-  return rc;
+  EHM_CHECK_ARG(h && B > 0);
+  const size_t need = (size_t)B * h->hid * kJ;
+  if (h->cond_E_floats < need) {
+    if (h->cond_E) {
+      EHM_HIP(hipDeviceSynchronize());
+      (void)hipFree(h->cond_E);
+      h->cond_E = nullptr;
+      h->cond_E_floats = 0;
+    }
+    if (hipMalloc(&h->cond_E, need * sizeof(float)) != hipSuccess) {
+      h->cond_E = nullptr;
+      ehm_set_error("ehm_gcn_input_layer: hipMalloc of %zu bytes failed", need * sizeof(float));
+      return EHM_ENOMEM;
+    }
+    h->cond_E_floats = need;
+  }
+  const int rc = ehm_gcn_cond_table(h, h_img, h_oth, vis, B, h->cond_E, stream);
+  return rc != 0 ? rc : ehm_gcn_input_layer_cond(h, h_img, h_oth, vis, h->cond_E, x, Wx, tvec, out, B, passes, stream);
 }
 
 extern "C" int ehm_gcn_input_layer_rows(ehm_gcn* h, const float* pre, float* out, int bodies, void* stream) {
diff --git a/egohmr_amd/csrc/gcn_dev.h b/egohmr_amd/csrc/gcn_dev.h
--- a/egohmr_amd/csrc/gcn_dev.h
+++ b/egohmr_amd/csrc/gcn_dev.h
@@ -67,6 +67,8 @@
   size_t chain_err_off = 0;
   int chain = 1;
   OutDev out{};
+  float* cond_E = nullptr;
+  size_t cond_E_floats = 0;
   float* arena = nullptr;
   float* hs = nullptr;
   int64_t hs_rows = 0;
@@ -194,28 +196,60 @@
   int total_vb, ny;
   unsigned int* sticky = nullptr;
   const float* pre = nullptr;
+  const float* E = nullptr;
 };
 
+__device__ __forceinline__ void gcn_cond_table_body(const float* __restrict__ h_img, const float* __restrict__ h_oth, const uint8_t* __restrict__ vis,
+                                                    const LayerDev& L, int mask_all, int b, int n, float* __restrict__ E) {
+  typedef const float __attribute__((address_space(4))) cfloat;
+  const cfloat* Ac = (const cfloat*)(uintptr_t)L.Aoff;
+  const int N = L.N;
+  const float img0 = h_img[((size_t)b * 2) * N + n], img1 = h_img[((size_t)b * 2 + 1) * N + n];
+  const float dl0 = mask_all ? h_oth[((size_t)b * 2) * N + n] : 0.f, dl1 = mask_all ? h_oth[((size_t)b * 2 + 1) * N + n] : 0.f;
+  const f32x4* d4 = (const f32x4*)(L.Ds + (size_t)n * kJ);
+  const f32x4* m4 = (const f32x4*)(L.M1s + (size_t)n * kJ);
+  float v[kJ], mv[kJ], mj[kJ], dj[kJ];
+#pragma unroll
+  for (int q = 0; q < kJ / 4; ++q) {
+    const f32x4 d = d4[q], m = m4[q];
+#pragma unroll
+    for (int i = 0; i < 4; ++i) {
+      const int j = 4 * q + i;
+      v[j] = vis[(size_t)b * kJ + j] ? 1.f : 0.f;
+      dj[j] = d[i];
+      mj[j] = m[i];
+      mv[j] = m[i] * v[j];
+    }
+  }
+#pragma unroll
+  for (int j = 0; j < kJ; ++j) {
+    float S = 0.f, R = 0.f;
+#pragma unroll
+    for (int k = 0; k < kJ; ++k) {
+      const float a = Ac[j * kJ + k];
+      S = fmaf(a, mv[k], S);
+      R = fmaf(a, mj[k], R);
+    }
+    E[((size_t)b * kJ + j) * N + n] = fmaf(dl1, R, fmaf(img1, S, dj[j] * fmaf(v[j], img0, dl0)));
+  }
+}
+
 template <int OUT, bool X_LDS = false, bool PRE = false>
-__device__ __forceinline__ void gcn_input_body(float* T, int tid, int bx, int by, const GcnInputArgs& a, const float* xb_in) {
-  const float* __restrict__ h_img = a.h_img; const float* __restrict__ h_oth = a.h_oth; const uint8_t* __restrict__ vis = a.vis;
+__device__ __forceinline__ void gcn_input_body(float* T, int tid, int b, int vb_c, int vb_m, int by, const GcnInputArgs& a, const float* xb_in) {
+  const float* __restrict__ h_oth = a.h_oth;
   const float* __restrict__ x = a.x; const float* __restrict__ Wx = a.Wx; const float* __restrict__ tvec = a.tvec;
   const LayerDev& L = a.L;
   float* __restrict__ Y = a.Y;
-  const int B = a.B, passes = a.passes, mask_all = a.mask_all;
-  const int32_t* __restrict__ mask_items = a.mask_items;
-  (void)passes;
+  const int mask_all = a.mask_all;
   const int N = L.N;
-  const int vb = bx;
-  const int p = vb >= B ? 1 : 0, b = p ? (mask_items ? mask_items[vb - B] : vb - B) : vb;
+  const bool cond = !PRE && vb_c >= 0;
   const int n_raw = by * 256 + tid;
   const int n = n_raw < N ? n_raw : N - 1;
-  float base[2] = {0.f, 0.f}, img[2] = {0.f, 0.f}, wx[2][6] = {{0.f, 0.f, 0.f, 0.f, 0.f, 0.f}, {0.f, 0.f, 0.f, 0.f, 0.f, 0.f}};
+  float base[2] = {0.f, 0.f}, wx[2][6] = {{0.f, 0.f, 0.f, 0.f, 0.f, 0.f}, {0.f, 0.f, 0.f, 0.f, 0.f, 0.f}};
   if constexpr (!PRE)
 #pragma unroll
   for (int k = 0; k < 2; ++k) {
-    base[k] = ((p == 1 && mask_all) ? 0.f : h_oth[((size_t)b * 2 + k) * N + n]) + tvec[k * N + n];
-    img[k] = (p == 0) ? h_img[((size_t)b * 2 + k) * N + n] : 0.f;
+    base[k] = (mask_all ? 0.f : h_oth[((size_t)b * 2 + k) * N + n]) + tvec[k * N + n];
 #pragma unroll
     for (int c = 0; c < 6; ++c) wx[k][c] = Wx[(k * 6 + c) * N + n];
   }
@@ -230,7 +264,6 @@
       xr[4 * i] = v[0]; xr[4 * i + 1] = v[1]; xr[4 * i + 2] = v[2]; xr[4 * i + 3] = v[3];
     }
   }
-  const uint8_t* vb_ = PRE ? nullptr : vis + (size_t)b * kJ;
   float h0[kJ], h1[kJ];
   const float sh = L.shift[n];
   float dj[kJ], mj[kJ];
@@ -250,7 +283,7 @@
       }
     }
   }
-  const f32x2 img2 = {img[0], img[1]}, base2 = {base[0], base[1]};
+  const f32x2 base2 = {base[0], base[1]};
   f32x2 wx2[6];
 #pragma unroll
   for (int c = 0; c < 6; ++c) wx2[c] = f32x2{wx[0][c], wx[1][c]};
@@ -258,11 +291,10 @@
   for (int j = 0; j < kJ; ++j) {
     f32x2 s;
     if constexpr (PRE) {
-      const float* pr = a.pre + ((size_t)vb * kJ + j) * 2 * (size_t)N + n;
+      const float* pr = a.pre + ((size_t)vb_m * kJ + j) * 2 * (size_t)N + n;
       s = f32x2{pr[0], pr[N]};
     } else {
-    const float v = vb_[j] ? 1.f : 0.f;
-    s = __builtin_elementwise_fma(f32x2{v, v}, img2, base2);
+    s = base2;
 #pragma unroll
     for (int c = 0; c < 6; ++c) {
       const float xv = X_LDS ? xr[X_LDS ? j * 6 + c : 0] : xb[j * 6 + c];
@@ -297,19 +329,16 @@
       DA = __builtin_amdgcn_mfma_f32_32x32x16_f16(af, __builtin_bit_cast(half8, Pw), DA, 0, 0, 0);
       DB = __builtin_amdgcn_mfma_f32_32x32x16_f16(af, __builtin_bit_cast(half8, Qw), DB, 0, 0, 0);
     }
-    const bool relu = L.relu != 0;
     const int cA = 64 * wv + (lane & 31), half = lane >> 5;
 #pragma unroll
     for (int r = 0; r < 12; ++r) {
       const int j = (r & 3) + 8 * (r >> 2) + 4 * half;
-      const float va = relu ? fmaxf(DA[r], 0.f) : DA[r], vb = relu ? fmaxf(DB[r], 0.f) : DB[r];
-      T[j * 256 + cA] = fmaf(DA[r], 0.f, va);
-      T[j * 256 + cA + 32] = fmaf(DB[r], 0.f, vb);
+      T[j * 256 + cA] = DA[r];
+      T[j * 256 + cA + 32] = DB[r];
     }
   } else {
     typedef const float __attribute__((address_space(4))) cfloat;
     const cfloat* Ac = (const cfloat*)(uintptr_t)L.Aoff;
-    const bool relu = L.relu != 0;
     f32x2 sacc[kJ / 2];
 #pragma unroll
     for (int jj = 0; jj < kJ / 2; ++jj) sacc[jj] = f32x2{h0[2 * jj], h0[2 * jj + 1]};
@@ -321,24 +350,34 @@
     }
 #pragma unroll
     for (int jj = 0; jj < kJ / 2; ++jj) {
-      f32x2 o = sacc[jj];
-      if (relu) { o[0] = fmaxf(o[0], 0.f); o[1] = fmaxf(o[1], 0.f); }
-      if constexpr (OUT != 0) o = __builtin_elementwise_fma(sacc[jj], f32x2{0.f, 0.f}, o);
-      T[(2 * jj) * 256 + tid] = o[0];
-      T[(2 * jj + 1) * 256 + tid] = o[1];
-    }
-  }
-  __syncthreads();
+      T[(2 * jj) * 256 + tid] = sacc[jj][0];
+      T[(2 * jj + 1) * 256 + tid] = sacc[jj][1];
+    }
+  }
   typedef unsigned int u32x4 __attribute__((ext_vector_type(4)));
+  const bool relu = L.relu != 0;
   const int nb = by * 256;
+  f32x4 e0[3], e1[3];
 #pragma unroll
   for (int i = 0; i < 3; ++i) {
     const int u = tid + 256 * i, j = u >> 5, c8 = (u & 31) * 8;
-    if (nb + c8 >= N) continue;
-
-    const f32x4 v0 = *(const f32x4*)(T + j * 256 + c8), v1 = *(const f32x4*)(T + j * 256 + c8 + 4);
-    const float v[8] = {v0[0], v0[1], v0[2], v0[3], v1[0], v1[1], v1[2], v1[3]};
-    const size_t row = (size_t)vb * kJ + j;
+    e0[i] = f32x4{0.f, 0.f, 0.f, 0.f};
+    e1[i] = e0[i];
+    if (cond && nb + c8 < N) {
+      const float* ep = a.E + (size_t)b * kJ * N + (unsigned int)(j * N + nb + c8);
+      e0[i] = *(const f32x4*)ep;
+      e1[i] = *(const f32x4*)(ep + 4);
+    }
+  }
+  __syncthreads();
+  auto store_row = [&](int vbr, int j, int c8, const float (&pre)[8]) {
+    float v[8];
+#pragma unroll
+    for (int k = 0; k < 8; ++k) {
+      v[k] = relu ? fmaxf(pre[k], 0.f) : pre[k];
+      if (OUT != 0) v[k] = fmaf(pre[k], 0.f, v[k]);
+    }
+    const unsigned int off = (unsigned int)(j * N + nb + c8);
     if (OUT != 0) {
       if (a.sticky) {
         float vm = 0.f;
@@ -354,22 +393,40 @@
         ll[k] = (half_t)fminf(fmaxf(v[k] - (float)hh[k], -65504.f), 65504.f);
       }
       if (OUT == 1) {
-        half_t* p = (half_t*)Y + split_off<32>(row, nb + c8, N);
+        half_t* p = (half_t*)Y + (size_t)vbr * kJ * N * 2 + (unsigned int)split_off<32>(j, nb + c8, N);
         *(u32x4*)p = __builtin_bit_cast(u32x4, hh);
         *(u32x4*)(p + 32) = __builtin_bit_cast(u32x4, ll);
       } else {
-        *(u32x4*)((half_t*)Y + row * (size_t)N + nb + c8) = __builtin_bit_cast(u32x4, hh);
+        *(u32x4*)((half_t*)Y + (size_t)vbr * kJ * N + off) = __builtin_bit_cast(u32x4, hh);
       }
     } else {
-      float* p = Y + row * (size_t)N + nb + c8;
-      *(f32x4*)p = v0;
-      *(f32x4*)(p + 4) = v1;
+      float* p = Y + (size_t)vbr * kJ * N + off;
+      *(f32x4*)p = f32x4{v[0], v[1], v[2], v[3]};
+      *(f32x4*)(p + 4) = f32x4{v[4], v[5], v[6], v[7]};
+    }
+  };
+#pragma unroll
+  for (int i = 0; i < 3; ++i) {
+    const int u = tid + 256 * i, j = u >> 5, c8 = (u & 31) * 8;
+    if (nb + c8 >= N) continue;
+
+    const f32x4 v0 = *(const f32x4*)(T + j * 256 + c8), v1 = *(const f32x4*)(T + j * 256 + c8 + 4);
+    if (cond) {
+      const f32x4 c0 = v0 + e0[i], c1 = v1 + e1[i];
+      const float pre[8] = {c0[0], c0[1], c0[2], c0[3], c1[0], c1[1], c1[2], c1[3]};
+      store_row(vb_c, j, c8, pre);
+    }
+    if (vb_m >= 0) {
+      const float pre[8] = {v0[0], v0[1], v0[2], v0[3], v1[0], v1[1], v1[2], v1[3]};
+      store_row(vb_m, j, c8, pre);
     }
   }
 }
 template <int OUT>
 __device__ __forceinline__ void gcn_input_body(float* T, int bx, int by, const GcnInputArgs& a) {
-  gcn_input_body<OUT>(T, (int)threadIdx.x, bx, by, a, nullptr);
+  const bool second = bx >= a.B;
+  const int b = second ? (a.mask_items ? a.mask_items[bx - a.B] : bx - a.B) : bx;
+  gcn_input_body<OUT>(T, (int)threadIdx.x, b, second ? -1 : bx, second ? bx : -1, by, a, nullptr);
 }
 
 constexpr int OUT_ROWS_PER_BLOCK = 16;
diff --git a/egohmr_amd/csrc/internal.h b/egohmr_amd/csrc/internal.h
--- a/egohmr_amd/csrc/internal.h
+++ b/egohmr_amd/csrc/internal.h
@@ -31,10 +31,11 @@
 int ehm_smpl_num_extra(const ehm_smpl* h);
 struct GcnInputArgs;
 struct GcnRun;
-int ehm_gcn_input_args(const ehm_gcn* h, const GcnRun& r, const float* h_img, const float* h_oth, const uint8_t* vis, const float* x, const float* Wx,
-                       const float* tvec, float* out, int B, int passes, GcnInputArgs* a);
-int ehm_gcn_input_impl(const ehm_gcn* h, const GcnRun& r, const float* h_img, const float* h_oth, const uint8_t* vis, const float* x,
+int ehm_gcn_input_args(const ehm_gcn* h, const GcnRun& r, const float* h_img, const float* h_oth, const uint8_t* vis, const float* E, const float* x,
+                       const float* Wx, const float* tvec, float* out, int B, int passes, GcnInputArgs* a);
+int ehm_gcn_input_impl(const ehm_gcn* h, const GcnRun& r, const float* h_img, const float* h_oth, const uint8_t* vis, const float* E, const float* x,
                        const float* Wx, const float* tvec, float* out, int B, int passes, hipStream_t st);
+int ehm_gcn_cond_table_impl(const ehm_gcn* h, const GcnRun& r, const float* h_img, const float* h_oth, const uint8_t* vis, int B, float* E, hipStream_t st);
 int ehm_gcn_hidden_stack_impl(ehm_gcn* h, const GcnRun& r, float* const bufs[3], int64_t rows_pad, int* result_index, hipStream_t st);
 int ehm_gcn_output_dot_impl(ehm_gcn* h, const GcnRun& r, const float* X, int B, int passes, const float** hs, hipStream_t st);
 int ehm_num_cus();
diff --git a/egohmr_amd/csrc/sampler.hip b/egohmr_amd/csrc/sampler.hip
--- a/egohmr_amd/csrc/sampler.hip
+++ b/egohmr_amd/csrc/sampler.hip
@@ -139,6 +139,7 @@
 struct Workspace {
   float* X[3];
   float* x_cur;
+  float* cond_E;
   float* A;
   float* g_verts_in;
   float* g_joints;
@@ -174,6 +175,7 @@
   };
   for (int i = 0; i < 3; ++i) w.X[i] = take(w.rows_pad * hid);
   w.x_cur = take((int64_t)d->B * kPoseDim);
+  w.cond_E = take((int64_t)d->B * hid * kJ);
   w.A = take((int64_t)d->B * kJ * 12);
   const bool guided = d->num_scene_points > 0;
   if (guided) {
@@ -241,6 +243,10 @@
 
   int rc = 0;
   base.valid_rows = w.rows;
+  {
+    EhmProfScope ps(EHM_PROF_INPUT, st);
+    rc = ehm_gcn_cond_table_impl(gcn, base, h_img, h_oth, vis, B, w.cond_E, st);
+  }
   const int lowprec = base.precision == EHM_PREC_F16X3 ? d->lowprec_steps : 0;
   auto prec_of = [&](int k) { return (lowprec > 0 && k < lowprec) ? (int)EHM_PREC_F16 : base.precision; };
   const bool defer_skin = w.skin_seg > 0 && d->lbs_every_step && ehm_smpl_has_mfma_skin(smpl);
@@ -278,7 +284,7 @@
     }
     if (rc == 0 && !input_done) {
       EhmProfScope ps(EHM_PROF_INPUT, st);
-      rc = ehm_gcn_input_impl(gcn, run, h_img, h_oth, vis, w.x_cur, Wx, tvecs + (int64_t)k * 2 * hid, w.X[0], B, d->passes, st);
+      rc = ehm_gcn_input_impl(gcn, run, h_img, h_oth, vis, w.cond_E, w.x_cur, Wx, tvecs + (int64_t)k * 2 * hid, w.X[0], B, d->passes, st);
     }
     input_done = false;
     int in = 0;
@@ -304,7 +310,7 @@
       const float* eps = noise + (int64_t)(1 + k) * n;
       float* dst = last ? x_final : w.x_cur;
       GcnInputArgs nin;
-      if (rc == 0 && !last) rc = ehm_gcn_input_args(gcn, run, h_img, h_oth, vis, dst, Wx, tvecs + (int64_t)(k + 1) * 2 * hid, w.X[0], B, d->passes, &nin);
+      if (rc == 0 && !last) rc = ehm_gcn_input_args(gcn, run, h_img, h_oth, vis, w.cond_E, dst, Wx, tvecs + (int64_t)(k + 1) * 2 * hid, w.X[0], B, d->passes, &nin);
       if (rc == 0)
         rc = ehm_step_fused_impl(out_dev, feat, run.precision, vis, w.x_cur, eps, grad, dst, defer_skin ? w.loop_x0 + (int64_t)pending * n : x0_final,
                                  &c, d->ddim, d->passes, run.slots(d->passes), B, last ? nullptr : &nin, gcn_input_format(gcn, prec_of(k + 1)), st);
@@ -327,7 +333,7 @@
       GcnInputArgs nin;
       const GcnInputArgs* pnin = nullptr;
       if (!last && d->lbs_every_step && !defer_skin) {
-        rc = ehm_gcn_input_args(gcn, run, h_img, h_oth, vis, dst, Wx, tvecs + (int64_t)(k + 1) * 2 * hid, w.X[0], B, d->passes, &nin);
+        rc = ehm_gcn_input_args(gcn, run, h_img, h_oth, vis, w.cond_E, dst, Wx, tvecs + (int64_t)(k + 1) * 2 * hid, w.X[0], B, d->passes, &nin);
         pnin = &nin;
       }
       int fused = 0;
diff --git a/egohmr_amd/csrc/step.hip b/egohmr_amd/csrc/step.hip
--- a/egohmr_amd/csrc/step.hip
+++ b/egohmr_amd/csrc/step.hip
@@ -51,11 +51,11 @@
   }
   if (!a.do_input) return;
   __syncthreads();
-  const int ny = a.in.ny, np = slot >= 0 ? 2 : 1, grp = tid >> 8;
-  const int rounds = np * ((ny + G - 1) / G);
+  const int ny = a.in.ny, grp = tid >> 8, vb_m = slot >= 0 ? B + slot : -1;
+  const int rounds = (ny + G - 1) / G;
   for (int k = 0; k < rounds; ++k) {
-    const int cb = grp + G * (k / np), p = k % np;
-    if (cb < ny) gcn_input_body<OUT, true>(T + grp * kFusedT, tid & 255, p ? B + slot : b, cb, a.in, L.xn);
+    const int cb = grp + G * k;
+    if (cb < ny) gcn_input_body<OUT, true>(T + grp * kFusedT, tid & 255, b, b, vb_m, cb, a.in, L.xn);
     else __syncthreads();
     __syncthreads();
   }
diff --git a/egohmr_amd/fused.py b/egohmr_amd/fused.py
--- a/egohmr_amd/fused.py
+++ b/egohmr_amd/fused.py
@@ -72,6 +72,7 @@
         self._nl_set = None
         self._pk = self._ck = None
         self._prep = self._prep_key = None
+        self._cond_E = None
         self._joint_map = self._count_host = None
         self._beta_key = self._beta_w = None
         self._tv_cache = None
@@ -293,12 +294,23 @@
             self._ws = torch.empty(int(nbytes), dtype=torch.uint8, device=device)
         return self._ws
 
+    def _cond_table(self, st):
+        h = self.gcn()
+        srcs = (st.h_img, st.h_oth, st.vis)
+        key = (self._gcn_key, self._gcn.serial, bool(self.model.only_mask_img_cond), st.B, tuple((t.data_ptr(), t._version) for t in srcs))
+        if self._cond_E is None or self._cond_E[0] != key:
+            E = torch.empty(st.B, 24, self.model.diffusion_model.hid_dim, device=st.h_img.device)
+            _lib.api().ehm_gcn_cond_table(h, st.h_img, st.h_oth, st.vis, st.B, E, _lib.stream_ptr())
+            self._cond_E = (key, E, srcs)
+        return self._cond_E[1]
+
     @torch.no_grad()
     def denoise_once(self, st, x_t, tvec, passes):
         m, A = self.model, _lib.api()
         rows = self._apply_pass_map(st, passes)[0] * 24
         h = self.gcn()
-        fill = lambda X0: A.ehm_gcn_input_layer(h, st.h_img, st.h_oth, st.vis, x_t, self._folded.Wx, tvec, X0, st.B, passes, _lib.stream_ptr())
+        E = self._cond_table(st)
+        fill = lambda X0: A.ehm_gcn_input_layer_cond(h, st.h_img, st.h_oth, st.vis, E, x_t, self._folded.Wx, tvec, X0, st.B, passes, _lib.stream_ptr())
         return m.diffusion_model.denoiser_tail(h, fill, rows=rows, B=st.B, passes=passes, vis=st.vis, precision=m.gcn_precision, device=m.device)
 
     @torch.no_grad()
diff --git a/include/egohmr_hip.h b/include/egohmr_hip.h
--- a/include/egohmr_hip.h
+++ b/include/egohmr_hip.h
@@ -75,6 +75,9 @@
 int ehm_gcn_set_nonlocal(ehm_gcn* h, const ehm_nonlocal_params* p);
 int ehm_gcn_input_layer(ehm_gcn* h, const float* h_img, const float* h_oth, const uint8_t* vis, const float* x,
                         const float* Wx, const float* tvec, float* out, int B, int passes, void* stream);
+int ehm_gcn_cond_table(ehm_gcn* h, const float* h_img, const float* h_oth, const uint8_t* vis, int B, float* E, void* stream);
+int ehm_gcn_input_layer_cond(ehm_gcn* h, const float* h_img, const float* h_oth, const uint8_t* vis, const float* E, const float* x,
+                             const float* Wx, const float* tvec, float* out, int B, int passes, void* stream);
 int ehm_gcn_input_layer_rows(ehm_gcn* h, const float* pre, float* out, int bodies, void* stream);
 
 int ehm_gcn_hidden_layer(ehm_gcn* h, int layer, const float* X, const float* residual, float* out,
```

New measurement: 2279 bodies/s, median of 2. Within noise of the previous version (+0.1%).
